# MIT-SPARK/Khronos

Hardware: AMD Instinct MI355X
Metric: active-window frames/sec (+ Mvoxel-updates/sec) at 1280x720 RGB-D+labels, 2 cm voxels (higher is better)
Workload: dtype f32

## Files before the change

### include/khronos_amd.h

```cpp
#ifndef KHRONOS_AMD_H_
#define KHRONOS_AMD_H_

#include <stddef.h>
#include <stdint.h>

#ifdef __cplusplus
extern "C" {
#endif

#define KHR_OK 0
#define KHR_EINVAL (-1)
#define KHR_ENOMEM (-2)
#define KHR_EDEVICE (-3)
#define KHR_ENOTFOUND (-4)
#define KHR_ESTATE (-5)

#define KHR_VOX_ACTIVE 1u
#define KHR_VOX_EVER_FREE 2u
#define KHR_VOX_TO_REMOVE 4u
#define KHR_VOX_SEM_VALID 8u
#define KHR_BLK_UPDATED 1u
#define KHR_BLK_MESH_UPDATED 2u
#define KHR_BLK_TRACKING_UPDATED 4u
#define KHR_BLK_HAS_ACTIVE_DATA 8u

typedef struct khr_config {
  float voxel_size;
  int32_t voxels_per_side;
  float truncation_distance;
  int32_t with_semantics;
  int32_t with_tracking;
  int32_t num_labels;
  int32_t use_weight_dropoff;
  float weight_dropoff_epsilon;
  int32_t use_constant_weight;
  float max_weight;
  int32_t interpolation_method;
  float adaptive_max_range_difference;
  int32_t range_mode;
  int32_t semantic_mode;
  float label_confidence;
  float temporal_buffer;
  float tsdf_occupancy_threshold;
  int32_t neighbor_connectivity;
  float temporal_window;
  int32_t md_neighbor_connectivity;
  int32_t md_min_cluster_size;
  int32_t md_max_cluster_size;
  float md_min_separation_distance;
  float md_max_range;
  float md_min_z_coordinate;
  float mesh_min_weight;
  uint32_t max_blocks;
  uint32_t max_frame_pixels;
  uint32_t num_frame_slots;
  uint64_t max_mesh_vertices;
  uint32_t max_band_records;
  int32_t disable_culling;
  int32_t device;
  int32_t rank;
  int32_t world_size;
  int32_t relaxed_arithmetic;
  uint32_t max_snapshot_blocks;
  int32_t alloc_candidate;
  int32_t color_blend_weight;
  int32_t mesh_attr_source;
  float mesh_degenerate_eps;
  int32_t packed_likelihood_rows;
} khr_config;

typedef struct khr_sensor {
  int32_t width, height;
  float fx, fy, cx, cy;
  float min_range, max_range;
} khr_sensor;

typedef struct khr_frame {
  uint64_t timestamp_ns;
  double world_T_sensor[16];
  const float* depth;
  const uint8_t* color;
  const int32_t* label;
} khr_frame;

typedef struct khr_stats {
  uint64_t n_allocated_blocks;
  uint64_t n_visible_blocks;
  uint64_t n_new_blocks;
  uint64_t n_visited_voxels;
  uint64_t n_updated_voxels;
  uint64_t n_band_voxels;
  uint64_t n_tracking_updated_blocks;
  uint64_t n_seeds;
  uint64_t n_mesh_blocks;
  uint64_t n_mesh_vertices;
  uint64_t pool_exhausted;
  uint64_t cum_updated_voxels;
  uint64_t cum_band_voxels;
  uint64_t cum_visited_voxels;
  uint64_t cum_integrate_calls;
  uint64_t n_tsdf_blocks;
  uint64_t band_overflow;
  uint64_t n_tracking_processed_blocks;
  uint64_t n_fuse_items;
  uint64_t n_seed_waits;
  uint64_t n_seed_waits_late;
  uint64_t seed_wait_max_us;
  uint64_t seed_wait_hist[8];
  uint64_t seed_wait_late_us;
  uint64_t seed_wait_late_frame;
  uint64_t seed_wait_late_state;
  uint64_t n_md_device_merges;
  uint64_t n_md_host_walks;
  uint64_t n_md_prelaunched;
  uint64_t n_md_prelaunch_repeats;
} khr_stats;

typedef struct khr_cluster {
  int32_t id;
  uint64_t num_pixels_listed;
  uint32_t num_pixels_painted;
  float bbox_min[3], bbox_max[3];
  float centroid[3];
  int32_t semantic_id;
} khr_cluster;

typedef struct khr_object_detector_config {
  int32_t use_full_connectivity;
  int32_t min_cluster_size;
  int32_t max_cluster_size;
  int32_t use_3d;
  float grid_size;
  float max_range;
  const int32_t* object_labels;
  int32_t n_object_labels;
} khr_object_detector_config;

typedef struct khr_ctx khr_ctx;

int khr_create(const khr_config* cfg, khr_ctx** out);
void khr_destroy(khr_ctx* ctx);
const char* khr_last_error(void);

void khr_host_trace(const char* tag);
int khr_set_stream(khr_ctx* ctx, void* hip_stream);
int khr_sync(khr_ctx* ctx);
void khr_default_config(khr_config* cfg);
int khr_reset_map(khr_ctx* ctx, float voxel_size, float truncation_distance);
int khr_retain_slot(khr_ctx* ctx, int slot);
int khr_release_slot(khr_ctx* ctx, int slot);
int khr_depend_on(khr_ctx* ctx, khr_ctx* other);
int khr_get_config(khr_ctx* ctx, khr_config* out);

int khr_upload_frame(khr_ctx* ctx, const khr_sensor* sensor, const khr_frame* frame, int on_device);
int khr_set_frame_image(khr_ctx* ctx, int slot, int which, const int32_t* image, int on_device);
int khr_download_frame(khr_ctx* ctx, int slot, float* range, float* vertex_map, int32_t* dynamic_image);
int khr_download_frame_image(khr_ctx* ctx, int slot, int which, int32_t* image);
typedef struct khr_frame_copy khr_frame_copy;
int khr_frame_copy_create(khr_ctx* ctx, int slot, khr_frame_copy** out);
int khr_frame_copy_download(khr_frame_copy* fc, float* depth, float* range, uint8_t* color_rgb, int32_t* labels, float* vertex_map);
void khr_frame_copy_release(khr_frame_copy* fc);
int khr_copy_frame_image(khr_ctx* ctx, int slot, int which, void* device_dst);

int khr_integrate(khr_ctx* ctx, int slot, int allocate_blocks, int use_mask, int object_id);
int khr_integrate_shared(khr_ctx* ctx, khr_ctx* src, int src_slot, int allocate_blocks, int use_mask, int object_id);
int khr_integrate_shared_batch(khr_ctx* ctx, khr_ctx* src, const int* src_slots, const int* object_ids, int n_frames,
                               int allocate_blocks, int use_mask);
int khr_update_tracking(khr_ctx* ctx, uint64_t timestamp_ns);
int khr_update_tracking_phase(khr_ctx* ctx, uint64_t timestamp_ns, int phase);
#define KHR_HALO_RECORD_BYTES 528
int khr_export_halo(khr_ctx* ctx, void* records, int64_t cap_records, int on_device);
int khr_import_halo(khr_ctx* ctx, const void* records, int64_t n_records, int on_device);
int khr_detect_motion(khr_ctx* ctx, int slot);
int khr_motion_keys(khr_ctx* ctx, int slot, void* keys_out, int on_device, uint32_t* n_seed_pixels);
int khr_detect_motion_from_keys(khr_ctx* ctx, int slot, const void* keys, int on_device);
size_t khr_motion_bits_bytes(int64_t n_pixels);
int khr_motion_bits(khr_ctx* ctx, int slot, void* bits_device);
int khr_detect_motion_from_bits(khr_ctx* ctx, int slot, const void* bits_device);
int khr_dynamic_pack_bytes(khr_ctx* ctx, int slot, void* dst_device);
int khr_dynamic_unpack_bytes(khr_ctx* ctx, int slot, const void* src_device);
int khr_mirror_dynamic(khr_ctx* ctx, int src_slot, int dst_slot);
int khr_get_dynamic_clusters(khr_ctx* ctx, int slot, khr_cluster* out, int cap);
int khr_configure_object_detector(khr_ctx* ctx, const khr_object_detector_config* cfg);
int khr_detect_objects(khr_ctx* ctx, int slot);
int khr_detect_objects_launch(khr_ctx* ctx, int slot);
int khr_get_semantic_clusters(khr_ctx* ctx, int slot, khr_cluster* out, int cap);
int64_t khr_cluster_voxels(khr_ctx* ctx, int slot, int which, float voxel_size, int32_t* ids_out, int64_t* voxels_out,
                           int64_t cap);
int khr_cluster_voxels_launch(khr_ctx* ctx, int slot, int which, float voxel_size);
int64_t khr_cluster_voxels_fetch(khr_ctx* ctx, int which, int32_t* ids_out, int64_t* voxels_out, int64_t cap);
int khr_configure_object_voxel_sets(khr_ctx* ctx, float voxel_size);
typedef struct khr_pixel_ref {
  int32_t slot;
  int32_t which;
  int32_t id;
} khr_pixel_ref;
int khr_pixel_iou(khr_ctx* ctx, int slot, const khr_pixel_ref* refs, int n_refs, int max_id, uint32_t* n_points, uint32_t* inter);
int khr_forward_instances(khr_ctx* ctx, int slot, float max_range, const int32_t* background_ids, int n_background, int max_id,
                          khr_cluster* out);
int khr_generate_mesh(khr_ctx* ctx, int only_mesh_updated, int clear_flag);
#define KHR_MESH_HALO_RECORD_BYTES(vps) (4 * (4 + 3 * 6 * (vps) * (vps)))
int khr_mesh_halo_requests(khr_ctx* ctx, void* keys_out, int64_t cap, int only_mesh_updated, int on_device);
int khr_mesh_halo_export(khr_ctx* ctx, const void* requests, int64_t n_requests, void* records, int64_t cap_records,
                         int on_device);
int khr_mesh_halo_import(khr_ctx* ctx, const void* records, int64_t n_records, int on_device);
#define KHR_MESH_HALO_REQ_HEADER_WORDS(world) (8 * (world))
int khr_mesh_halo_requests_sorted(khr_ctx* ctx, void* requests_device, int64_t cap, int only_mesh_updated);
int khr_mesh_halo_plan(int world, int rank, int vps, const uint64_t* headers, uint64_t* sendcounts, uint64_t* sdispls,
                       uint64_t* recvcounts, uint64_t* rdispls);
int khr_mesh_halo_answer(khr_ctx* ctx, const void* all_requests_device, int64_t cap, const uint64_t* headers, void* records_device,
                         int64_t cap_words);
int khr_mesh_halo_adopt(khr_ctx* ctx, const void* own_requests_device, const uint64_t* own_header, const void* records_device,
                        const uint64_t* rdispls);
int khr_reset_inactive(khr_ctx* ctx, int32_t* removed, int64_t cap, int64_t* n_removed);
int khr_last_removed(khr_ctx* ctx, int32_t* removed, int64_t cap, int64_t* n_removed);
int khr_mark_all_inactive(khr_ctx* ctx);
int khr_clear_updated(khr_ctx* ctx);
int khr_allocate_blocks(khr_ctx* ctx, const int32_t* indices, int64_t n);
int khr_object_prune(khr_ctx* ctx, float min_confidence, float min_observations, int64_t* n_pruned);

#define KHR_PF_MOTION 1u
#define KHR_PF_TRACKING 2u
#define KHR_PF_OUTPUT 4u
#define KHR_PF_OBJECTS 8u
#define KHR_PF_SNAPSHOT 32u
#define KHR_PF_INPUT_READY 16u
#define KHR_PF_INPUT_PINNED 128u
#define KHR_PF_INGESTED 64u
int khr_process_frame(khr_ctx* ctx, const khr_sensor* sensor, const khr_frame* frame, int on_device, uint32_t flags,
                      int* n_clusters);
int khr_ingest_ahead(khr_ctx* ctx, const khr_sensor* sensor, const khr_frame* frame);
int khr_ingest_ahead_host(khr_ctx* ctx, const khr_sensor* sensor, const khr_frame* frame);
int khr_ingest_cancel(khr_ctx* ctx);

int64_t khr_pool_exhausted(khr_ctx* ctx);
int khr_get_stats(khr_ctx* ctx, khr_stats* out);
int64_t khr_num_blocks(khr_ctx* ctx);
int64_t khr_block_indices(khr_ctx* ctx, int32_t* out, int64_t cap, int only_updated);
int khr_download_block(khr_ctx* ctx, int32_t bx, int32_t by, int32_t bz, float* distance, float* weight,
                       uint8_t* color_rgba, uint64_t* last_observed, uint64_t* last_occupied,
                       uint8_t* voxel_flags, uint32_t* sem_label, float* likelihoods, uint8_t* block_flags);
int khr_map_slice(khr_ctx* ctx, int64_t voxel_z, int64_t cap, int32_t* block_xy, float* positions, float* distance, float* weight,
                  uint64_t* last_observed, uint8_t* voxel_flags, int64_t* n_voxels);
int khr_slice_voxel_z(float height, float voxel_size, int32_t voxels_per_side, int64_t* voxel_z);
typedef struct khr_render_request {
  khr_sensor sensor;
  double world_T_sensor[16];
  float step_voxels;
  float min_weight;
} khr_render_request;
typedef struct khr_render_stats {
  uint64_t n_hit, n_blocked;
  uint64_t n_samples_total;
  uint64_t n_samples_evaluated;
} khr_render_stats;
int khr_render_view(khr_ctx* ctx, const khr_render_request* request, int on_device, float* depth, float* normal, uint8_t* color_rgba,
                    uint32_t* label, uint8_t* vflags, uint8_t* status, khr_render_stats* stats);
typedef struct khr_query_stats {
  uint64_t n_value, n_gradient, n_voxel;
} khr_query_stats;
#define KHR_QP_VALUE 1
#define KHR_QP_GRADIENT 2
#define KHR_QP_VOXEL 4
int khr_query_points(khr_ctx* ctx, int64_t n, const float* points, float min_weight, int on_device, float* distance, float* gradient,
                     float* weight, uint8_t* color_rgba, uint32_t* label, uint8_t* vflags, uint64_t* last_observed, uint8_t* status,
                     khr_query_stats* stats);
#define KHR_DF_MAX_DIM 512
#define KHR_DF_FAR (1 << 30)
// ... 177 lines not shown
```

### khronos_amd/capi.py

```python
import ctypes as C
import os

import numpy as np

_HERE = os.path.dirname(os.path.abspath(__file__))
LIB_PATH = os.path.join(_HERE, "lib", "libkhronos_amd.so")

KHR_OK, KHR_EINVAL, KHR_ENOMEM, KHR_EDEVICE, KHR_ENOTFOUND, KHR_ESTATE = 0, -1, -2, -3, -4, -5
VOX_ACTIVE, VOX_EVER_FREE, VOX_TO_REMOVE, VOX_SEM_VALID = 1, 2, 4, 8
BLK_UPDATED, BLK_MESH_UPDATED, BLK_TRACKING_UPDATED, BLK_HAS_ACTIVE_DATA = 1, 2, 4, 8


class KhrConfig(C.Structure):
    _fields_ = [
        ("voxel_size", C.c_float), ("voxels_per_side", C.c_int32), ("truncation_distance", C.c_float),
        ("with_semantics", C.c_int32), ("with_tracking", C.c_int32), ("num_labels", C.c_int32),
        ("use_weight_dropoff", C.c_int32), ("weight_dropoff_epsilon", C.c_float),
        ("use_constant_weight", C.c_int32), ("max_weight", C.c_float), ("interpolation_method", C.c_int32),
        ("adaptive_max_range_difference", C.c_float), ("range_mode", C.c_int32), ("semantic_mode", C.c_int32),
        ("label_confidence", C.c_float),
        ("temporal_buffer", C.c_float), ("tsdf_occupancy_threshold", C.c_float),
        ("neighbor_connectivity", C.c_int32), ("temporal_window", C.c_float),
        ("md_neighbor_connectivity", C.c_int32), ("md_min_cluster_size", C.c_int32),
        ("md_max_cluster_size", C.c_int32), ("md_min_separation_distance", C.c_float),
        ("md_max_range", C.c_float), ("md_min_z_coordinate", C.c_float),
        ("mesh_min_weight", C.c_float),
        ("max_blocks", C.c_uint32), ("max_frame_pixels", C.c_uint32), ("num_frame_slots", C.c_uint32),
        ("max_mesh_vertices", C.c_uint64), ("max_band_records", C.c_uint32), ("disable_culling", C.c_int32),
        ("device", C.c_int32), ("rank", C.c_int32), ("world_size", C.c_int32), ("relaxed_arithmetic", C.c_int32), ("max_snapshot_blocks", C.c_uint32),
        ("alloc_candidate", C.c_int32), ("color_blend_weight", C.c_int32), ("mesh_attr_source", C.c_int32), ("mesh_degenerate_eps", C.c_float),
        ("packed_likelihood_rows", C.c_int32),
    ]


class KhrSensor(C.Structure):
    _fields_ = [("width", C.c_int32), ("height", C.c_int32), ("fx", C.c_float), ("fy", C.c_float),
                ("cx", C.c_float), ("cy", C.c_float), ("min_range", C.c_float), ("max_range", C.c_float)]


class KhrRenderRequest(C.Structure):
    _fields_ = [("sensor", KhrSensor), ("world_T_sensor", C.c_double * 16), ("step_voxels", C.c_float), ("min_weight", C.c_float)]


class KhrRenderStats(C.Structure):
    _fields_ = [(n, C.c_uint64) for n in ("n_hit", "n_blocked", "n_samples_total", "n_samples_evaluated")]


class KhrQueryStats(C.Structure):
    _fields_ = [(n, C.c_uint64) for n in ("n_value", "n_gradient", "n_voxel")]


KHR_QP_VALUE, KHR_QP_GRADIENT, KHR_QP_VOXEL = 1, 2, 4


class KhrWeldStats(C.Structure):
    _fields_ = [("n_soup_vertices", C.c_uint64), ("n_vertices", C.c_uint64), ("n_faces", C.c_uint64), ("n_degenerate_faces", C.c_uint64)]


KHR_MERGE_ALIGNED, KHR_MERGE_RESAMPLE = 0, 1


class KhrMergeRequest(C.Structure):
    _fields_ = [("mode", C.c_int32), ("voxel_offset", C.c_int32 * 3), ("dst_T_src", C.c_double * 16), ("min_weight", C.c_float)]


class KhrMergeStats(C.Structure):
    _fields_ = [(n, C.c_uint64) for n in ("n_src_blocks", "n_candidate_blocks", "n_touched_blocks", "n_new_blocks", "n_added_voxels",
                                          "n_merged_voxels")]


class KhrDfRequest(C.Structure):
    _fields_ = [("origin", C.c_int32 * 3), ("dims", C.c_int32 * 3), ("ratio", C.c_int32), ("min_weight", C.c_float),
                ("max_distance", C.c_float), ("surface_distance", C.c_float), ("unknown_is_obstacle", C.c_int32),
                ("positive_only", C.c_int32)]


class KhrDfStats(C.Structure):
    _fields_ = [(n, C.c_uint64) for n in ("n_observed", "n_obstacle", "n_free", "n_in_range")]


KHR_DF_OBSERVED, KHR_DF_OBSTACLE, KHR_DF_IN_RANGE = 1, 2, 4
KHR_DF_MAX_DIM, KHR_DF_FAR = 512, 1 << 30


class KhrAlignRequest(C.Structure):
    _fields_ = [("n", C.c_int64), ("points", C.c_void_p), ("depth", C.c_void_p), ("sensor", KhrSensor), ("stride", C.c_int32),
                ("weights", C.c_void_p), ("world_T_source", C.c_double * 16), ("min_weight", C.c_float), ("gate", C.c_float),
                ("huber_delta", C.c_float)]


class KhrAlignOptions(C.Structure):
    _fields_ = [("max_iterations", C.c_int32), ("min_inliers", C.c_int32), ("lambda_", C.c_double), ("eps_rot", C.c_double),
                ("eps_trans", C.c_double)]


class KhrAlignResult(C.Structure):
    _fields_ = [("iterations", C.c_int32), ("converged", C.c_int32), ("n_inlier_first", C.c_uint64), ("n_inlier_last", C.c_uint64),
                ("rmse_first", C.c_double), ("rmse_last", C.c_double), ("H", C.c_double * 21), ("b", C.c_double * 6)]


KHR_ALIGN_WORDS, KHR_ALIGN_MAX_SOURCES = 32, 1 << 20


class KhrFrame(C.Structure):
    _fields_ = [("timestamp_ns", C.c_uint64), ("world_T_sensor", C.c_double * 16), ("depth", C.c_void_p),
                ("color", C.c_void_p), ("label", C.c_void_p)]


class KhrConvertedFrame(C.Structure):
    _fields_ = [("timestamp_ns", C.c_uint64), ("world_T_sensor", C.c_double * 16), ("range", C.c_void_p), ("depth", C.c_void_p),
                ("rgba", C.c_void_p), ("label", C.c_void_p), ("tile_max", C.c_void_p)]


class KhrCluster(C.Structure):
    _fields_ = [("id", C.c_int32), ("num_pixels_listed", C.c_uint64), ("num_pixels_painted", C.c_uint32),
                ("bbox_min", C.c_float * 3), ("bbox_max", C.c_float * 3), ("centroid", C.c_float * 3),
                ("semantic_id", C.c_int32)]


class KhrObjectDetectorConfig(C.Structure):
    _fields_ = [("use_full_connectivity", C.c_int32), ("min_cluster_size", C.c_int32), ("max_cluster_size", C.c_int32),
                ("use_3d", C.c_int32), ("grid_size", C.c_float), ("max_range", C.c_float),
                ("object_labels", C.POINTER(C.c_int32)), ("n_object_labels", C.c_int32)]


CKPT_SECTIONS = ("indices", "distance", "weight", "color", "last_observed", "last_occupied", "flags", "sem_label", "block_flags",
                 "likelihoods")


class KhrCheckpointHeader(C.Structure):
    _fields_ = [("magic", C.c_uint32), ("version", C.c_uint32), ("voxel_size", C.c_float), ("voxels_per_side", C.c_int32),
                ("truncation_distance", C.c_float), ("with_semantics", C.c_int32), ("with_tracking", C.c_int32),
                ("num_labels", C.c_int32), ("semantic_mode", C.c_int32), ("header_bytes", C.c_uint32),
                ("num_blocks", C.c_uint64), ("total_bytes", C.c_uint64), ("offset", C.c_uint64 * len(CKPT_SECTIONS))]


class KhrStats(C.Structure):
    _fields_ = [(n, C.c_uint64) for n in (
        "n_allocated_blocks", "n_visible_blocks", "n_new_blocks", "n_visited_voxels", "n_updated_voxels",
        "n_band_voxels", "n_tracking_updated_blocks", "n_seeds", "n_mesh_blocks", "n_mesh_vertices",
        "pool_exhausted", "cum_updated_voxels", "cum_band_voxels", "cum_visited_voxels", "cum_integrate_calls", "n_tsdf_blocks", "band_overflow",
        "n_tracking_processed_blocks", "n_fuse_items", "n_seed_waits", "n_seed_waits_late", "seed_wait_max_us")] + [
        ("seed_wait_hist", C.c_uint64 * 8)] + [(n, C.c_uint64) for n in (
        "seed_wait_late_us", "seed_wait_late_frame", "seed_wait_late_state", "n_md_device_merges", "n_md_host_walks",
        "n_md_prelaunched", "n_md_prelaunch_repeats")]


EXPORTS = [
    "khr_create", "khr_destroy", "khr_last_error", "khr_host_trace", "khr_set_stream", "khr_sync", "khr_default_config",
    "khr_upload_frame", "khr_set_frame_image", "khr_download_frame", "khr_frame_copy_create", "khr_frame_copy_download", "khr_frame_copy_release", "khr_integrate", "khr_update_tracking",
    "khr_detect_motion", "khr_generate_mesh", "khr_reset_inactive", "khr_mark_all_inactive", "khr_clear_updated",
    "khr_allocate_blocks", "khr_object_prune", "khr_get_stats", "khr_num_blocks", "khr_block_indices",
    "khr_download_block", "khr_mesh_num_vertices", "khr_download_mesh", "khr_fetch_mesh", "khr_fetch_mesh_into", "khr_timing_enable", "khr_timing_reset",
    "khr_timing_get", "khr_debug_read", "khr_tick_ingest", "khr_tick_integrate", "khr_tick_live_bound", "khr_tick_seed_counts", "khr_converted_bytes", "khr_export_converted",
    "khr_converted_views", "khr_tick_adopt", "khr_copy_frame_image", "khr_rv_detect_changes", "khr_last_removed", "khr_process_frame", "khr_ingest_ahead", "khr_ingest_ahead_host", "khr_ingest_cancel", "khr_integrate_shared", "khr_integrate_shared_batch", "khr_pixel_iou", "khr_forward_instances", "khr_update_tracking_phase",
    "khr_export_halo", "khr_import_halo", "khr_get_dynamic_clusters", "khr_motion_keys", "khr_motion_bits_bytes", "khr_motion_bits", "khr_detect_motion_from_bits",
    "khr_dynamic_pack_bytes", "khr_dynamic_unpack_bytes",
    "khr_detect_motion_from_keys", "khr_download_updated", "khr_mesh_halo_requests", "khr_mesh_halo_export",
    "khr_mesh_halo_requests_sorted", "khr_mesh_halo_plan", "khr_mesh_halo_answer", "khr_mesh_halo_adopt",
    "khr_mesh_halo_import", "khr_configure_object_detector", "khr_detect_objects", "khr_get_semantic_clusters",
    "khr_cluster_voxels", "khr_download_frame_image", "khr_detect_objects_launch", "khr_pool_exhausted", "khr_map_digest",
    "khr_rv_create", "khr_rv_destroy", "khr_rv_clear", "khr_rv_add_rays", "khr_rv_num_rays", "khr_rv_num_pairs", "khr_rv_check",
    "khr_snapshot_updated", "khr_take_snapshot", "khr_snapshot_num_blocks", "khr_snapshot_download", "khr_snapshot_download_extra", "khr_snapshot_download_begin", "khr_snapshot_download_end", "khr_snapshot_poll", "khr_fetch_mesh_launch", "khr_reserve_mesh_staging", "khr_reserve_snapshots", "khr_mirror_dynamic", "khr_snapshot_release",
    "khr_rv_check_stamps", "khr_get_config", "khr_cluster_voxels_launch", "khr_cluster_voxels_fetch", "khr_reset_map", "khr_depend_on", "khr_retain_slot", "khr_release_slot",
    "khr_map_slice", "khr_slice_voxel_z", "khr_render_view", "khr_query_points",
    "khr_align_linearize", "khr_align_frame", "khr_distance_field",
    "khr_checkpoint_size", "khr_checkpoint_save", "khr_checkpoint_load", "khr_checkpoint_inspect",
    "khr_debug_live_resources", "khr_configure_object_voxel_sets",
    "khr_weld_mesh", "khr_weld_mesh_into", "khr_merge_map",
]

_lib = None


class KhronosAmdError(RuntimeError):
    pass


def load_library():
    global _lib
    if _lib is not None:
        return _lib
    if not os.path.exists(LIB_PATH):
        raise KhronosAmdError(
            "HIP extension %s is missing: run `python -c 'import __graft_entry__ as g; g.build()'`. "
            "The khronos_amd fusion path has no CPU fallback." % LIB_PATH)
    lib = C.CDLL(LIB_PATH)
    vp, i32, i64, u64 = C.c_void_p, C.c_int, C.c_int64, C.c_uint64
    lib.khr_create.argtypes = [C.POINTER(KhrConfig), C.POINTER(vp)]
    lib.khr_create.restype = i32
    lib.khr_destroy.argtypes = [vp]
    lib.khr_destroy.restype = None
    lib.khr_last_error.restype = C.c_char_p
    lib.khr_host_trace.argtypes = [C.c_char_p]
    lib.khr_host_trace.restype = None
    lib.khr_set_stream.argtypes = [vp, vp]
    lib.khr_sync.argtypes = [vp]
    lib.khr_default_config.argtypes = [C.POINTER(KhrConfig)]
    lib.khr_default_config.restype = None
    lib.khr_upload_frame.argtypes = [vp, C.POINTER(KhrSensor), C.POINTER(KhrFrame), i32]
    lib.khr_set_frame_image.argtypes = [vp, i32, i32, vp, i32]
    lib.khr_download_frame.argtypes = [vp, i32, vp, vp, vp]
    lib.khr_integrate.argtypes = [vp, i32, i32, i32, i32]
    lib.khr_integrate_shared.argtypes = [vp, vp, i32, i32, i32, i32]
    lib.khr_integrate_shared_batch.argtypes = [vp, vp, vp, vp, i32, i32, i32]
    lib.khr_update_tracking.argtypes = [vp, u64]
    lib.khr_update_tracking_phase.argtypes = [vp, u64, i32]
    lib.khr_export_halo.argtypes = [vp, vp, i64, i32]
    lib.khr_import_halo.argtypes = [vp, vp, i64, i32]
    lib.khr_detect_motion.argtypes = [vp, i32]
    lib.khr_motion_keys.argtypes = [vp, i32, vp, i32, C.POINTER(C.c_uint32)]
    lib.khr_detect_motion_from_keys.argtypes = [vp, i32, vp, i32]
    lib.khr_get_dynamic_clusters.argtypes = [vp, i32, C.POINTER(KhrCluster), i32]
    lib.khr_configure_object_detector.argtypes = [vp, C.POINTER(KhrObjectDetectorConfig)]
    lib.khr_detect_objects.argtypes = [vp, i32]
    lib.khr_pixel_iou.argtypes = [vp, i32, vp, i32, i32, vp, vp]
    lib.khr_forward_instances.argtypes = [vp, i32, C.c_float, vp, i32, i32, C.POINTER(KhrCluster)]
    lib.khr_download_frame_image.argtypes = [vp, i32, i32, vp]
    lib.khr_rv_create.argtypes = [C.c_float, C.c_float, C.c_float, i32, C.POINTER(vp)]
    lib.khr_rv_destroy.argtypes = [vp]
    lib.khr_rv_destroy.restype = None
    lib.khr_rv_clear.argtypes = [vp]
    lib.khr_rv_add_rays.argtypes = [vp, C.c_int64, vp, vp, vp]
    lib.khr_rv_num_rays.argtypes = [vp]
    lib.khr_rv_num_rays.restype = C.c_int64
    lib.khr_rv_num_pairs.argtypes = [vp]
    lib.khr_rv_num_pairs.restype = C.c_int64
    lib.khr_rv_check.argtypes = [vp, C.c_int64, vp, vp, vp, vp, vp, C.POINTER(C.c_uint64), C.POINTER(C.c_uint64)]
    lib.khr_rv_check_stamps.argtypes = [vp, vp, vp]
    lib.khr_rv_detect_changes.argtypes = [vp, C.c_float, C.c_int64, i32, C.c_float, C.c_float, vp, i32, vp, vp, vp]
    lib.khr_get_config.argtypes = [vp, vp]
    lib.khr_reset_map.argtypes = [vp, C.c_float, C.c_float]
    lib.khr_depend_on.argtypes = [vp, vp]
    lib.khr_retain_slot.argtypes = [vp, i32]
    lib.khr_release_slot.argtypes = [vp, i32]
    lib.khr_cluster_voxels_launch.argtypes = [vp, i32, i32, C.c_float]
    lib.khr_cluster_voxels_fetch.argtypes = [vp, i32, vp, vp, C.c_int64]
    lib.khr_cluster_voxels_fetch.restype = C.c_int64
    lib.khr_configure_object_voxel_sets.argtypes = [vp, C.c_float]
    lib.khr_get_semantic_clusters.argtypes = [vp, i32, C.POINTER(KhrCluster), i32]
    lib.khr_cluster_voxels.argtypes = [vp, i32, i32, C.c_float, vp, vp, C.c_int64]
    lib.khr_cluster_voxels.restype = C.c_int64
    lib.khr_generate_mesh.argtypes = [vp, i32, i32]
    lib.khr_reset_inactive.argtypes = [vp, vp, i64, C.POINTER(i64)]
    lib.khr_mark_all_inactive.argtypes = [vp]
    lib.khr_clear_updated.argtypes = [vp]
    lib.khr_allocate_blocks.argtypes = [vp, vp, i64]
    lib.khr_object_prune.argtypes = [vp, C.c_float, C.c_float, C.POINTER(i64)]
    lib.khr_get_stats.argtypes = [vp, C.POINTER(KhrStats)]
    lib.khr_num_blocks.argtypes = [vp]
    lib.khr_num_blocks.restype = i64
    lib.khr_block_indices.argtypes = [vp, vp, i64, i32]
    lib.khr_block_indices.restype = i64
    lib.khr_download_block.argtypes = [vp, C.c_int32, C.c_int32, C.c_int32] + [vp] * 9
    lib.khr_map_slice.argtypes = [vp, i64, i64] + [vp] * 7
    lib.khr_slice_voxel_z.argtypes = [C.c_float, C.c_float, C.c_int32, vp]
    lib.khr_render_view.argtypes = [vp, C.POINTER(KhrRenderRequest), i32] + [vp] * 6 + [C.POINTER(KhrRenderStats)]
    lib.khr_query_points.argtypes = [vp, i64, vp, C.c_float, i32] + [vp] * 8 + [C.POINTER(KhrQueryStats)]
    lib.khr_distance_field.argtypes = [vp, C.POINTER(KhrDfRequest), i32, vp, vp, vp, C.POINTER(KhrDfStats)]
    lib.khr_align_linearize.argtypes = [vp, C.POINTER(KhrAlignRequest), i32, vp]
    lib.khr_align_frame.argtypes = [vp, C.POINTER(KhrAlignRequest), i32, C.POINTER(KhrAlignOptions), vp, C.POINTER(KhrAlignResult)]
    lib.khr_checkpoint_size.argtypes = [vp, C.POINTER(u64), C.POINTER(i64)]
    lib.khr_checkpoint_save.argtypes = [vp, vp, u64, C.POINTER(u64)]
    lib.khr_checkpoint_load.argtypes = [vp, vp, u64, C.POINTER(i64)]
    lib.khr_checkpoint_inspect.argtypes = [vp, u64, C.POINTER(KhrCheckpointHeader)]
    lib.khr_mesh_halo_requests.argtypes = [vp, vp, i64, i32, i32]
    lib.khr_mesh_halo_export.argtypes = [vp, vp, i64, vp, i64, i32]
    lib.khr_mesh_halo_import.argtypes = [vp, vp, i64, i32]
    lib.khr_mesh_halo_requests_sorted.argtypes = [vp, vp, i64, i32]
    lib.khr_mesh_halo_plan.argtypes = [i32, i32, i32, vp, vp, vp, vp, vp]
    lib.khr_mesh_halo_answer.argtypes = [vp, vp, i64, vp, vp, i64]
    lib.khr_mesh_halo_adopt.argtypes = [vp, vp, vp, vp, vp]
    lib.khr_download_updated.argtypes = [vp] + [vp] * 7 + [i64]
    lib.khr_download_updated.restype = i64
    lib.khr_snapshot_updated.argtypes = [vp, C.c_uint32, i64, C.POINTER(vp)]
    lib.khr_take_snapshot.argtypes = [vp, C.POINTER(vp)]
    lib.khr_snapshot_num_blocks.argtypes = [vp]
    lib.khr_snapshot_num_blocks.restype = i64
    lib.khr_snapshot_download.argtypes = [vp] + [vp] * 7 + [i64]
    lib.khr_snapshot_download.restype = i64
    lib.khr_snapshot_download_begin.argtypes = [vp] + [vp] * 7 + [i64]
    lib.khr_snapshot_download_end.argtypes = [vp]
    lib.khr_snapshot_download_end.restype = i64
    lib.khr_snapshot_download_extra.argtypes = [vp, vp, vp, vp, i64]
    lib.khr_snapshot_download_extra.restype = i64
    lib.khr_snapshot_release.argtypes = [vp]
    lib.khr_snapshot_release.restype = None
    lib.khr_mesh_num_vertices.argtypes = [vp]
    lib.khr_mesh_num_vertices.restype = i64
    lib.khr_download_mesh.argtypes = [vp, vp, vp, vp, vp, vp, i64]
    lib.khr_download_mesh.restype = i64
    lib.khr_fetch_mesh.argtypes = [vp, vp]
    lib.khr_fetch_mesh.restype = i64
    lib.khr_fetch_mesh_into.argtypes = [vp, vp, vp, vp, vp, vp]
    lib.khr_weld_mesh.argtypes = [vp, C.c_float, C.POINTER(KhrWeldStats)]
    lib.khr_weld_mesh_into.argtypes = [vp, i32] + [vp] * 7
    lib.khr_merge_map.argtypes = [vp, vp, C.POINTER(KhrMergeRequest), C.POINTER(KhrMergeStats)]
    lib.khr_debug_read.argtypes = [vp, vp, i64]
# ... 1028 lines not shown
```

### khronos_amd/csrc/khr_kernels_aux.h

```cpp
#pragma once
#include <cstring>
#include "khr_md_host.h"
#include "khr_device.h"

namespace khr {

#include "mc_table.inc"
__device__ int8_t g_mc_tri[256][16];
__device__ uint8_t g_mc_ntri[256];

constexpr uint64_t kSeedBit = kSeedFlag;

__global__ __launch_bounds__(256) void k_motion_pixels(DevMap m, DevParams p, DevFrame f, float md_max_range,
                                                      float min_z_world, uint64_t* __restrict__ keys, int ignore_epoch,
                                                      uint32_t* __restrict__ begin_band_count) {
  if (begin_band_count && blockIdx.x == 0) beginIntegrate(m, p.nvox, begin_band_count);
  const int i = blockIdx.x * blockDim.x + threadIdx.x;
  const bool in = i < f.W * f.H;
  uint64_t key = ~0ull;
  if (in)
    key = motionPixelKey(m, p, f.range[i], f.depth[i], i % f.W, i / f.W, f.fx, f.fy, f.cx, f.cy, f.Rw, f.tw, md_max_range,
                         min_z_world, ignore_epoch);
  if (in) keys[i] = key;
  const bool seed = (key != ~0ull) && (key & kSeedBit);
  const int any = __syncthreads_count(seed ? 1 : 0);
  if (any && threadIdx.x == 0) atomicAdd(&m.counters[C_N_SEEDS], static_cast<uint32_t>(any));
}

__global__ __launch_bounds__(1024) void k_publish(const uint32_t* __restrict__ src, volatile uint32_t* __restrict__ dst_host,
                                                 uint32_t rec_words, uint32_t max_recs, volatile uint32_t* __restrict__ ticket_host,
                                                 uint32_t ticket, uint32_t* __restrict__ counters_to_zero) {
  const uint32_t n_words = 4u + min(src[0], max_recs) * rec_words;
  for (uint32_t i = threadIdx.x; i < n_words; i += blockDim.x) dst_host[i] = src[i];
  __threadfence_system();
  __syncthreads();
  if (threadIdx.x < 4) counters_to_zero[threadIdx.x] = 0u;
  if (threadIdx.x == 0) {
    *ticket_host = ticket;
    __threadfence_system();
  }
}

__global__ void k_publish_seed(DevMap m, volatile uint32_t* host_seed, uint32_t ticket) {
  if (blockIdx.x == 0 && threadIdx.x == 0) publishSeedCount(m, host_seed, ticket);
}

__global__ __launch_bounds__(256) void k_md_keys_export(const uint64_t* __restrict__ keys, int n, uint64_t* __restrict__ out) {
  const int i = blockIdx.x * blockDim.x + threadIdx.x;
  if (i < n) out[i] = keys[i] == ~0ull ? 0ull : keys[i];
}
__global__ __launch_bounds__(256) void k_md_keys_import(const uint64_t* __restrict__ in, int n, uint64_t* __restrict__ keys,
                                                       uint32_t* __restrict__ n_seed_px) {
  const int i = blockIdx.x * blockDim.x + threadIdx.x;
  uint64_t k = ~0ull;
  if (i < n) {
    k = in[i] == 0ull ? ~0ull : in[i];
    keys[i] = k;
  }
  const unsigned long long b = __ballot(k != ~0ull && (k & kSeedBit));
  if (b && laneId() == static_cast<uint32_t>(__ffsll(static_cast<long long>(b)) - 1))
    atomicAdd(n_seed_px, static_cast<uint32_t>(__popcll(b)));
}

__global__ __launch_bounds__(256) void k_md_bits_export(const uint64_t* __restrict__ keys, int n, unsigned long long* __restrict__ bits) {
  const int i = blockIdx.x * blockDim.x + threadIdx.x;
  const uint64_t k = i < n ? keys[i] : ~0ull;
  const unsigned long long ex = __ballot(k != ~0ull), sd = __ballot(k != ~0ull && (k & kSeedBit));
  if (laneId() == 0 && (i & ~63) < n) {
    bits[2 * (i >> 6)] = ex;
    bits[2 * (i >> 6) + 1] = sd;
  }
}
__global__ __launch_bounds__(256) void k_md_keys_from_bits(DevParams p, DevFrame f, float md_max_range, float min_z_world,
                                                          const unsigned long long* __restrict__ bits, uint64_t* __restrict__ keys,
                                                          uint32_t* __restrict__ n_seed_px) {
  const int i = blockIdx.x * blockDim.x + threadIdx.x;
  const int n = f.W * f.H;
  uint64_t k = ~0ull;
  if (i < n) {
    const unsigned long long ex = bits[2 * (i >> 6)], sd = bits[2 * (i >> 6) + 1];
    if ((ex >> (i & 63)) & 1ull) {
      uint64_t bkey;
      int lin;
      k = motionPixelVoxel(p, f.range[i], f.depth[i], i % f.W, i / f.W, f.fx, f.fy, f.cx, f.cy, f.Rw, f.tw, md_max_range, min_z_world, &bkey, &lin);
      if (k != ~0ull && ((sd >> (i & 63)) & 1ull)) k |= kSeedBit;
    }
    keys[i] = k;
  }
  const unsigned long long b = __ballot(k != ~0ull && (k & kSeedBit));
  if (b && laneId() == static_cast<uint32_t>(__ffsll(static_cast<long long>(b)) - 1))
    atomicAdd(n_seed_px, static_cast<uint32_t>(__popcll(b)));
}
__global__ __launch_bounds__(256) void k_dyn_pack_u8(const int32_t* __restrict__ img, int n4, uint32_t* __restrict__ out) {
  const int i = blockIdx.x * blockDim.x + threadIdx.x;
  if (i >= n4) return;
  const int4 v = reinterpret_cast<const int4*>(img)[i];
  out[i] = (static_cast<uint32_t>(v.x) & 0xffu) | ((static_cast<uint32_t>(v.y) & 0xffu) << 8) | ((static_cast<uint32_t>(v.z) & 0xffu) << 16) |
           ((static_cast<uint32_t>(v.w) & 0xffu) << 24);
}
__global__ __launch_bounds__(256) void k_dyn_unpack_u8(const uint32_t* __restrict__ in, int n4, int32_t* __restrict__ img) {
  const int i = blockIdx.x * blockDim.x + threadIdx.x;
  if (i >= n4) return;
  const uint32_t w = in[i];
  reinterpret_cast<int4*>(img)[i] = make_int4(static_cast<int>(w & 0xffu), static_cast<int>((w >> 8) & 0xffu), static_cast<int>((w >> 16) & 0xffu),
                                              static_cast<int>(w >> 24));
}

struct VoxTable {
  uint64_t* keys;
  uint32_t* counts;
  uint32_t* ids;
  uint32_t mask;
};

__device__ inline int voxFind(const VoxTable& t, uint64_t key) {
  uint32_t h = hashKey(key) & t.mask;
  for (uint32_t probes = 0; probes <= t.mask; ++probes) {
    const uint64_t k = t.keys[h];
    if (k == key) return static_cast<int>(h);
    if (k == kEmptyKey) return -1;
    h = (h + 1) & t.mask;
  }
  return -1;
}

__device__ inline uint32_t voxInsert(const VoxTable& t, uint64_t key) {
  uint32_t h = hashKey(key) & t.mask;
  for (uint32_t probes = 0; probes <= t.mask; ++probes) {
    const unsigned long long prev = atomicCAS(reinterpret_cast<unsigned long long*>(&t.keys[h]),
                                              static_cast<unsigned long long>(kEmptyKey), static_cast<unsigned long long>(key));
    if (prev == kEmptyKey || prev == key) return h;
    h = (h + 1) & t.mask;
  }
  return kInvalidSlot;
}

__constant__ int8_t c_md_nbr26[26][3] = {
    {-1, 0, 0}, {1, 0, 0}, {0, -1, 0}, {0, 1, 0}, {0, 0, -1}, {0, 0, 1},
    {-1, -1, 0}, {-1, 1, 0}, {1, -1, 0}, {1, 1, 0}, {-1, 0, -1}, {-1, 0, 1}, {1, 0, -1}, {1, 0, 1},
    {0, -1, -1}, {0, -1, 1}, {0, 1, -1}, {0, 1, 1},
    {-1, -1, -1}, {-1, -1, 1}, {-1, 1, -1}, {-1, 1, 1}, {1, -1, -1}, {1, -1, 1}, {1, 1, -1}, {1, 1, 1}};

__device__ inline uint64_t neighbourKey(uint64_t key, int k) {
  int x, y, z;
  unpackKey(key, &x, &y, &z);
  return packKey(x + c_md_nbr26[k][0], y + c_md_nbr26[k][1], z + c_md_nbr26[k][2]);
}

__device__ inline void voxInsertCounted(const VoxTable& t, bool has, uint64_t key, uint32_t* overflow = nullptr) {
  const uint32_t lane = laneId();
  const uint32_t klo = static_cast<uint32_t>(key), khi = static_cast<uint32_t>(key >> 32);
  const uint32_t plo = __shfl_up(klo, 1), phi = __shfl_up(khi, 1);
  const unsigned long long hm = __ballot(has);
  const bool prev_has = lane > 0u && ((hm >> (lane - 1u)) & 1ull);
  const bool start = has && !(prev_has && plo == klo && phi == khi);
  const unsigned long long cont = hm & ~__ballot(start);
  if (start) {
    const unsigned long long above = lane == 63u ? 0ull : (~cont >> (lane + 1u));
    const uint32_t len = 1u + (lane == 63u ? 0u : static_cast<uint32_t>(__ffsll(static_cast<long long>(above | (1ull << (63u - lane)))) - 1));
    const uint32_t h = voxInsert(t, key);
    if (h != kInvalidSlot) atomicAdd(&t.counts[h], len);
    else if (overflow) atomicOr(overflow, 1u);
  }
}

__global__ __launch_bounds__(256) void k_md_clear(uint64_t* __restrict__ keys, uint32_t* __restrict__ counts, uint32_t tsize,
                                                 uint32_t* __restrict__ n4, int32_t* __restrict__ aabb) {
  const uint32_t stride = gridDim.x * blockDim.x;
  const uint32_t t0 = blockIdx.x * blockDim.x + threadIdx.x;
  ulonglong2* k2 = reinterpret_cast<ulonglong2*>(keys);
  for (uint32_t i = t0; i < 3u * (tsize / 2); i += stride) k2[i] = make_ulonglong2(~0ull, ~0ull);
  uint4* c4 = reinterpret_cast<uint4*>(counts);
  for (uint32_t i = t0; i < 2u * (tsize / 4); i += stride) c4[i] = make_uint4(0u, 0u, 0u, 0u);
  if (t0 < 4) n4[t0] = 0u;
  if (t0 < 6) aabb[t0] = t0 < 3 ? INT32_MAX : INT32_MIN;
  if (t0 == 7) aabb[7] = 0;
}

__global__ __launch_bounds__(256) void k_md_seed_insert(const uint64_t* __restrict__ keys, int n, VoxTable seeds,
                                                       uint32_t* __restrict__ overflow) {
  const int i = blockIdx.x * blockDim.x + threadIdx.x;
  const uint64_t k = i < n ? keys[i] : ~0ull;
  voxInsertCounted(seeds, k != ~0ull && (k & kSeedBit), k & ~kSeedBit, overflow);
}

__global__ __launch_bounds__(256) void k_md_near_insert(const uint64_t* __restrict__ seed_keys,
                                                       const uint32_t* __restrict__ n_seeds, uint32_t cap, int nn,
                                                       VoxTable near, uint32_t* __restrict__ overflow, int32_t* __restrict__ aabb) {
  const uint32_t ns = min(*n_seeds, cap);
  const bool direct = static_cast<float>(nn) * static_cast<float>(ns) > 0.7f * (static_cast<float>(near.mask) + 1.f);
  if (blockIdx.x == 0 && threadIdx.x == 0) aabb[6] = direct ? 1 : 0;
  int lo[3] = {INT32_MAX, INT32_MAX, INT32_MAX}, hi[3] = {INT32_MIN, INT32_MIN, INT32_MIN};
  for (uint32_t i = blockIdx.x * blockDim.x + threadIdx.x; i < ns * nn; i += gridDim.x * blockDim.x) {
    const uint64_t sk = seed_keys[i / nn];
    if (!direct && voxInsert(near, neighbourKey(sk, static_cast<int>(i % nn))) == kInvalidSlot) atomicOr(overflow, 1u);
    if (i % nn == 0) {
      int v[3];
      unpackKey(sk, &v[0], &v[1], &v[2]);
#pragma unroll
      for (int d = 0; d < 3; ++d) { lo[d] = min(lo[d], v[d]); hi[d] = max(hi[d], v[d]); }
    }
  }
  __shared__ int s_box[6][4];
#pragma unroll
  for (int d = 0; d < 3; ++d) {
#pragma unroll
    for (int o = 32; o > 0; o >>= 1) {
      lo[d] = min(lo[d], __shfl_xor(lo[d], o));
      hi[d] = max(hi[d], __shfl_xor(hi[d], o));
    }
  }
  if ((threadIdx.x & 63) == 0) {
#pragma unroll
    for (int d = 0; d < 3; ++d) { s_box[d][threadIdx.x >> 6] = lo[d]; s_box[3 + d][threadIdx.x >> 6] = hi[d]; }
  }
  __syncthreads();
  if (threadIdx.x < 6) {
    const int d = threadIdx.x;
    int v = s_box[d][0];
    for (int w = 1; w < 4; ++w) v = d < 3 ? min(v, s_box[d][w]) : max(v, s_box[d][w]);
    if (d < 3) { if (v != INT32_MAX) atomicMin(&aabb[d], v); }
    else if (v != INT32_MIN) atomicMax(&aabb[d], v);
  }
}

__global__ __launch_bounds__(256) void k_md_boundary_insert(const uint64_t* __restrict__ keys, int n, VoxTable near,
                                                           VoxTable bnd, VoxTable seeds, int nn, int direct,
                                                           const int32_t* __restrict__ aabb, uint32_t* __restrict__ overflow) {
  const int i = blockIdx.x * blockDim.x + threadIdx.x;
  const uint64_t k = i < n ? keys[i] : ~0ull;
  bool cand = k != ~0ull && !(k & kSeedBit);
  direct = direct || aabb[6];
  if (cand) {
    int x, y, z;
    unpackKey(k, &x, &y, &z);
    cand = x >= aabb[0] - 1 && y >= aabb[1] - 1 && z >= aabb[2] - 1 && x <= aabb[3] + 1 && y <= aabb[4] + 1 && z <= aabb[5] + 1;
  }
  if (cand) {
    if (!direct) {
      cand = voxFind(near, k) >= 0;
    } else {
      cand = false;
      for (int j = 0; j < nn && !cand; ++j) cand = voxFind(seeds, neighbourKey(k, j)) >= 0;
    }
  }
  voxInsertCounted(bnd, cand, k, overflow);
}

__global__ __launch_bounds__(256) void k_md_compact(VoxTable t, uint64_t* __restrict__ list_keys,
                                                   uint32_t* __restrict__ list_counts, uint32_t* __restrict__ n_out,
                                                   uint32_t cap, int32_t* __restrict__ zero_per_entry,
                                                   int32_t* __restrict__ zero_per_entry2 = nullptr,
                                                   unsigned long long* __restrict__ zero64 = nullptr) {
  __shared__ uint32_t s_cnt[4], s_base;
  const uint32_t h = blockIdx.x * blockDim.x + threadIdx.x;
  const bool used = h <= t.mask && t.keys[h] != kEmptyKey;
  const unsigned long long b = __ballot(used);
  if ((threadIdx.x & 63) == 0) s_cnt[threadIdx.x >> 6] = static_cast<uint32_t>(__popcll(b));
  __syncthreads();
  if (threadIdx.x == 0) {
    const uint32_t tot = s_cnt[0] + s_cnt[1] + s_cnt[2] + s_cnt[3];
    s_base = tot ? atomicAdd(n_out, tot) : 0u;
  }
  __syncthreads();
  if (used) {
    uint32_t id = s_base + static_cast<uint32_t>(__popcll(b & ((1ull << laneId()) - 1ull)));
    for (uint32_t w = 0; w < (threadIdx.x >> 6); ++w) id += s_cnt[w];
    if (id < cap) {
      list_keys[id] = t.keys[h];
      list_counts[id] = t.counts[h];
      t.ids[h] = id;
      if (zero_per_entry) zero_per_entry[id] = 0;
      if (zero_per_entry2) zero_per_entry2[id] = 0;
      if (zero64) zero64[id] = 0ull;
    }
  }
}

__global__ __launch_bounds__(256) void k_md_adjacency(const uint64_t* __restrict__ seed_keys,
                                                     const uint32_t* __restrict__ n_seeds, VoxTable seeds, VoxTable bnd,
                                                     int nn, uint32_t cap, uint32_t* __restrict__ adj,
                                                     uint32_t* __restrict__ edges, uint32_t edge_cap, uint32_t* __restrict__ n_edges) {
  __shared__ uint32_t s_cnt[4], s_base;
  const uint32_t ns = min(*n_seeds, cap);
  const uint32_t total = ns * nn;
  const uint32_t rounds = (total + gridDim.x * blockDim.x - 1) / (gridDim.x * blockDim.x);
  for (uint32_t r = 0; r < rounds; ++r) {
    const uint32_t i = (r * gridDim.x + blockIdx.x) * blockDim.x + threadIdx.x;
    uint32_t out = 0xffffffffu, s = 0;
    if (i < total) {
      s = i / nn;
      const uint32_t j = i % nn;
      const uint64_t nk = neighbourKey(seed_keys[s], static_cast<int>(j));
      const int hs = voxFind(seeds, nk);
      if (hs >= 0) {
        out = 0x80000000u | seeds.ids[hs];
      } else {
        const int hb = voxFind(bnd, nk);
        if (hb >= 0) out = bnd.ids[hb];
      }
      adj[i] = out;
    }
    const bool is_edge = out != 0xffffffffu && (out & 0x80000000u) && (out & 0x7fffffffu) < s && s < 65536u;
    const unsigned long long b = __ballot(is_edge);
    if ((threadIdx.x & 63) == 0) s_cnt[threadIdx.x >> 6] = static_cast<uint32_t>(__popcll(b));
    __syncthreads();
    if (threadIdx.x == 0) {
      const uint32_t tot = s_cnt[0] + s_cnt[1] + s_cnt[2] + s_cnt[3];
      s_base = tot ? atomicAdd(n_edges, tot) : 0u;
    }
    __syncthreads();
    if (is_edge) {
      uint32_t pos = s_base + static_cast<uint32_t>(__popcll(b & ((1ull << laneId()) - 1ull)));
      for (uint32_t w = 0; w < (threadIdx.x >> 6); ++w) pos += s_cnt[w];
      if (pos < edge_cap) edges[pos] = (s << 16) | (out & 0x7fffffffu);
    }
    __syncthreads();
  }
}

static_assert(sizeof(CompAcc) == 48, "CompAcc travels to the host as 12 words (k_publish)");
__device__ inline unsigned long long canonKey(uint64_t packed) {
  int x, y, z;
  unpackKey(packed, &x, &y, &z);
  return (static_cast<unsigned long long>(x + (1 << 20)) << 42) | (static_cast<unsigned long long>(y + (1 << 20)) << 21) |
         static_cast<unsigned long long>(z + (1 << 20));
}

constexpr uint32_t kCompLds = 12288;
// ... 136 lines not shown
    uint64_t bk[26];
#pragma unroll
    for (int j = 0; j < 26; ++j) {
      const bool is_b = av[j] != 0xffffffffu && !(av[j] & 0x80000000u);
      bc[j] = is_b ? bnd_counts[av[j]] : 0u;
      bk[j] = is_b ? bnd_keys[av[j]] : k;
    }
#pragma unroll
    for (int j = 0; j < 26; ++j) {
      px += bc[j];
      unpackKey(bk[j], &v[0], &v[1], &v[2]);
#pragma unroll
      for (int d = 0; d < 3; ++d) { lo[d] = min(lo[d], v[d]); hi[d] = max(hi[d], v[d]); }
    }
  }
  unsigned long long todo = __ballot(on);
  while (todo) {
    const int leader = __ffsll(static_cast<long long>(todo)) - 1;
    const uint32_t lr = __shfl(r, leader);
    const bool mine = on && r == lr;
    const unsigned long long grp = __ballot(mine);
    todo &= ~grp;
    unsigned long long p2 = mine ? px : 0ull, k2 = mine ? key : ~0ull;
    int l2[3], h2[3];
#pragma unroll
    for (int d = 0; d < 3; ++d) { l2[d] = mine ? lo[d] : INT32_MAX; h2[d] = mine ? hi[d] : INT32_MIN; }
#pragma unroll
    for (int o = 32; o > 0; o >>= 1) {
      const unsigned long long po = (static_cast<unsigned long long>(__shfl_xor(static_cast<uint32_t>(p2 >> 32), o)) << 32) |
                                    __shfl_xor(static_cast<uint32_t>(p2), o);
      const unsigned long long ko = (static_cast<unsigned long long>(__shfl_xor(static_cast<uint32_t>(k2 >> 32), o)) << 32) |
                                    __shfl_xor(static_cast<uint32_t>(k2), o);
      p2 += po;
      k2 = ko < k2 ? ko : k2;
#pragma unroll
      for (int d = 0; d < 3; ++d) { l2[d] = min(l2[d], __shfl_xor(l2[d], o)); h2[d] = max(h2[d], __shfl_xor(h2[d], o)); }
    }
    if (static_cast<int>(laneId()) == leader) {
      CompAcc* a = acc + lr;
      atomicAdd(&a->n_pixels, p2);
      atomicMin(&a->min_key, k2);
#pragma unroll
      for (int d = 0; d < 3; ++d) { atomicMin(&a->lo[d], l2[d]); atomicMax(&a->hi[d], h2[d]); }
    }
  }
}

__global__ __launch_bounds__(256) void k_md_comp_roots(const uint32_t* __restrict__ n_seeds, uint32_t cap, const uint32_t* __restrict__ parent,
                                                      const CompAcc* __restrict__ acc, uint32_t* __restrict__ root_idx,
                                                      uint32_t* __restrict__ n_roots, CompAcc* __restrict__ out, uint32_t out_cap) {
  const uint32_t ns = min(*n_seeds, cap);
  const uint32_t s = blockIdx.x * blockDim.x + threadIdx.x;
  const bool is_root = s < ns && parent[s] == s;
  const uint32_t idx = waveAggInc(n_roots, is_root);
  if (is_root) {
    root_idx[s] = idx;
    if (idx < out_cap) {
      CompAcc a = acc[s];
      a.root = 0u;
      a.pad = 0u;
      out[idx] = a;
    }
  }
}

__device__ inline unsigned long long compBit(const uint32_t* __restrict__ parent, const uint32_t* __restrict__ root_idx, uint32_t seed_id) {
  const uint32_t ri = root_idx[parent[seed_id]];
  return ri < 64u ? (1ull << ri) : 0ull;
}
__device__ inline unsigned long long segmentedOr(unsigned long long bits, uint32_t seg, bool* head) {
  const uint32_t lane = laneId();
  const uint32_t prev = __shfl_up(seg, 1);
  *head = lane == 0u || prev != seg;
#pragma unroll
  for (int o = 1; o < 32; o <<= 1) {
    const unsigned long long ob = (static_cast<unsigned long long>(__shfl_down(static_cast<uint32_t>(bits >> 32), o)) << 32) |
                                  __shfl_down(static_cast<uint32_t>(bits), o);
    const uint32_t os = __shfl_down(seg, o);
    if (lane + static_cast<uint32_t>(o) < 64u && os == seg) bits |= ob;
  }
  return bits;
}
__global__ __launch_bounds__(256) void k_md_bnd_comps(const uint64_t* __restrict__ bnd_keys, const uint32_t* __restrict__ n4, uint32_t cap, int nn,
                                                     VoxTable seeds, const uint32_t* __restrict__ parent, const uint32_t* __restrict__ root_idx,
                                                     unsigned long long* __restrict__ bnd_mask) {
  const uint32_t nb = min(n4[1], cap), R = n4[2];
  if (R < 2u || R > 64u) return;
  const uint32_t total = nb * static_cast<uint32_t>(nn), step = gridDim.x * blockDim.x;
  for (uint32_t i0 = blockIdx.x * blockDim.x; i0 < total; i0 += step) {
    const uint32_t i = i0 + threadIdx.x;
    const bool valid = i < total;
    const uint32_t b = valid ? i / nn : 0xffffffffu, j = valid ? i % nn : 0u;
    unsigned long long bit = 0ull;
    if (valid) {
      const int hs = voxFind(seeds, neighbourKey(bnd_keys[b], static_cast<int>(j)));
      if (hs >= 0) bit = compBit(parent, root_idx, seeds.ids[hs]);
    }
    bool head;
    bit = segmentedOr(bit, b, &head);
    if (valid && head && bit) atomicOr(&bnd_mask[b], bit);
  }
}
__global__ __launch_bounds__(256) void k_md_comp_overlap(const uint64_t* __restrict__ seed_keys, const uint64_t* __restrict__ bnd_keys,
                                                        const uint32_t* __restrict__ n4, uint32_t cap, int radius, VoxTable seeds, VoxTable bnd,
                                                        const uint32_t* __restrict__ parent, const uint32_t* __restrict__ root_idx,
                                                        const unsigned long long* __restrict__ bnd_mask, CompAcc* __restrict__ out) {
  const uint32_t ns = min(n4[0], cap), nb = min(n4[1], cap), R = n4[2];
  if (R < 2u || R > 64u) return;
  const uint32_t per = radius > 0 ? 27u : 1u;
  const uint32_t total = (ns + nb) * per, step = gridDim.x * blockDim.x;
  for (uint32_t i0 = blockIdx.x * blockDim.x; i0 < total; i0 += step) {
    const uint32_t i = i0 + threadIdx.x;
    const bool valid = i < total;
    const uint32_t v = valid ? i / per : 0xffffffffu, k = valid ? (per == 1u ? 26u : i % per) : 0u;
    unsigned long long bits = 0ull, mine = 0ull;
    if (valid) {
      const bool is_seed = v < ns;
      const uint64_t key = is_seed ? seed_keys[v] : bnd_keys[v - ns];
      mine = is_seed ? compBit(parent, root_idx, v) : bnd_mask[v - ns];
      if (k == 26u) {
        bits = mine;
      } else {
        const uint64_t nk = neighbourKey(key, static_cast<int>(k));
        const int hs = voxFind(seeds, nk);
        if (hs >= 0) {
          bits = compBit(parent, root_idx, seeds.ids[hs]);
        } else {
          const int hb = voxFind(bnd, nk);
          if (hb >= 0 && bnd.ids[hb] < cap) bits = bnd_mask[bnd.ids[hb]];
        }
      }
    }
    bool head;
    const unsigned long long acc = segmentedOr(bits, v, &head);
    if (valid && head && (acc & ~mine)) {
      unsigned long long todo = mine;
      while (todo) {
        const int c = __ffsll(static_cast<long long>(todo)) - 1;
        todo &= todo - 1ull;
        atomicOr(reinterpret_cast<unsigned long long*>(&out[c].root), acc | mine);
      }
    }
    if (valid && head && (mine & (mine - 1ull))) {
      unsigned long long todo = mine;
      while (todo) {
        const int c = __ffsll(static_cast<long long>(todo)) - 1;
        todo &= todo - 1ull;
        atomicOr(reinterpret_cast<unsigned long long*>(&out[c].root), mine);
      }
    }
  }
}

constexpr int kCompInline = 64;
struct CompFinals {
  int32_t id[kCompInline];
};
__global__ __launch_bounds__(256) void k_md_comp_finals(const uint32_t* __restrict__ adj, const uint32_t* __restrict__ n_seeds, uint32_t cap,
                                                       int nn, const uint32_t* __restrict__ parent, const uint32_t* __restrict__ root_idx,
                                                       const int32_t* __restrict__ comp_final, CompFinals inl, int32_t* __restrict__ seed_final,
                                                       int32_t* __restrict__ bnd_final, int32_t* __restrict__ bnd_deg) {
  const uint32_t ns = min(*n_seeds, cap);
  for (uint32_t i = blockIdx.x * blockDim.x + threadIdx.x; i < ns * nn; i += gridDim.x * blockDim.x) {
    const uint32_t s = i / nn, j = i % nn;
    const uint32_t ri = root_idx[parent[s]];
    const int32_t f = comp_final ? comp_final[ri] : inl.id[ri];
    if (j == 0) seed_final[s] = f;
    const uint32_t a = adj[i];
    if (f && a != 0xffffffffu && !(a & 0x80000000u)) {
      atomicMax(&bnd_final[a], f);
      atomicAdd(&bnd_deg[a], 1);
    }
  }
}

struct ClusterAcc {
  uint32_t n_pixels;
  int32_t bmin[3], bmax[3];
  float sum[3];
  uint32_t n_listed;
  float wsum[3];
};
__host__ __device__ inline void clusterAccReset(ClusterAcc& a) {
  a.n_pixels = 0;
  a.n_listed = 0;
  for (int d = 0; d < 3; ++d) { a.bmin[d] = INT32_MAX; a.bmax[d] = INT32_MIN; a.sum[d] = 0.f; a.wsum[d] = 0.f; }
}
__device__ inline int32_t floatToOrdered(float f) {
  const int32_t i = __float_as_int(f);
  return i >= 0 ? i : i ^ 0x7fffffff;
}
__host__ __device__ inline float orderedToFloat(int32_t i) {
  const int32_t j = i >= 0 ? i : i ^ 0x7fffffff;
  float f;
#if defined(__HIP_DEVICE_COMPILE__)
  f = __int_as_float(j);
#else
  std::memcpy(&f, &j, sizeof(f));
#endif
  return f;
}

__global__ __launch_bounds__(256) void k_md_paint(const uint64_t* __restrict__ keys, int n, VoxTable seeds, VoxTable bnd,
                                                 const int32_t* __restrict__ seed_final,
                                                 const int32_t* __restrict__ bnd_final, int32_t* __restrict__ dyn,
                                                 const int32_t* __restrict__ bnd_deg, uint8_t* __restrict__ dyn_weight) {
  const int i = blockIdx.x * blockDim.x + threadIdx.x;
  if (i >= n) return;
  const uint64_t k = keys[i];
  if (k == ~0ull) return;
  int id = 0, w = 1;
  if (k & kSeedBit) {
    const int h = voxFind(seeds, k & ~kSeedBit);
    if (h >= 0) id = seed_final[seeds.ids[h]];
  } else {
    const int h = voxFind(bnd, k);
    if (h >= 0) {
      id = bnd_final[bnd.ids[h]];
      w = bnd_deg[bnd.ids[h]];
    }
  }
  if (id) {
    dyn[i] = id;
    dyn_weight[i] = static_cast<uint8_t>(min(max(w, 1), 255));
  }
}

constexpr int kAccTile = 32, kAccSlots = 8;
__global__ __launch_bounds__(1024) void k_cluster_summary(DevFrame f, const int32_t* __restrict__ img,
                                                         ClusterAcc* __restrict__ acc, const uint8_t* __restrict__ weight) {
  __shared__ int s_id[kAccSlots];
  __shared__ ClusterAcc s_acc[kAccSlots];
  if (threadIdx.x < kAccSlots) {
    s_id[threadIdx.x] = 0;
    ClusterAcc a;
    clusterAccReset(a);
    s_acc[threadIdx.x] = a;
  }
  __syncthreads();
  const int tiles_x = (f.W + kAccTile - 1) / kAccTile;
  const int u = (blockIdx.x % tiles_x) * kAccTile + (threadIdx.x & 31), v = (blockIdx.x / tiles_x) * kAccTile + (threadIdx.x >> 5);
  int id = 0;
  float pw[3] = {0.f, 0.f, 0.f};
  float wt = 1.f;
  if (u < f.W && v < f.H) {
    const int i = v * f.W + u;
    id = img[i];
    if (id) {
      if (weight) wt = static_cast<float>(weight[i]);
      const float d = f.depth[i];
      xform(f.Rw, f.tw, ((static_cast<float>(u) - f.cx) / f.fx) * d, ((static_cast<float>(v) - f.cy) / f.fy) * d, d, pw);
    }
  }
  unsigned long long todo = __ballot(id != 0);
  while (todo) {
    const int leader = __ffsll(static_cast<long long>(todo)) - 1;
    const int cid = __shfl(id, leader);
    const bool mine = id == cid;
    const unsigned long long grp = __ballot(mine);
    todo &= ~grp;
    float mn[3], mx[3], sm[3], ws[3];
    float wn = mine ? wt : 0.f;
#pragma unroll
    for (int c = 0; c < 3; ++c) {
      mn[c] = mine ? pw[c] : 3.0e38f;
      mx[c] = mine ? pw[c] : -3.0e38f;
      sm[c] = mine ? pw[c] : 0.f;
      ws[c] = mine ? wt * pw[c] : 0.f;
    }
#pragma unroll
    for (int o = 32; o > 0; o >>= 1) {
      wn += __shfl_xor(wn, o);
#pragma unroll
      for (int c = 0; c < 3; ++c) {
        mn[c] = fminf(mn[c], __shfl_xor(mn[c], o));
        mx[c] = fmaxf(mx[c], __shfl_xor(mx[c], o));
        sm[c] += __shfl_xor(sm[c], o);
        ws[c] += __shfl_xor(ws[c], o);
      }
    }
    if (static_cast<int>(laneId()) == leader) {
      ClusterAcc* a = acc + cid;
      for (int k = 0; k < kAccSlots; ++k) {
        const int h = (cid + k) & (kAccSlots - 1);
        const int prev = atomicCAS(&s_id[h], 0, cid);
        if (prev == 0 || prev == cid) {
          a = &s_acc[h];
          break;
        }
      }
      atomicAdd(&a->n_pixels, static_cast<uint32_t>(__popcll(grp)));
      atomicAdd(&a->n_listed, static_cast<uint32_t>(wn));
#pragma unroll
      for (int c = 0; c < 3; ++c) {
        atomicMin(&a->bmin[c], floatToOrdered(mn[c]));
        atomicMax(&a->bmax[c], floatToOrdered(mx[c]));
        atomicAdd(&a->sum[c], sm[c]);
        atomicAdd(&a->wsum[c], ws[c]);
      }
    }
  }
  __syncthreads();
  if (threadIdx.x < kAccSlots && s_id[threadIdx.x]) {
    const ClusterAcc& l = s_acc[threadIdx.x];
    ClusterAcc* a = acc + s_id[threadIdx.x];
    atomicAdd(&a->n_pixels, l.n_pixels);
    atomicAdd(&a->n_listed, l.n_listed);
#pragma unroll
    for (int c = 0; c < 3; ++c) {
      atomicMin(&a->bmin[c], l.bmin[c]);
      atomicMax(&a->bmax[c], l.bmax[c]);
      atomicAdd(&a->sum[c], l.sum[c]);
      atomicAdd(&a->wsum[c], l.wsum[c]);
    }
  }
}

__global__ __launch_bounds__(256) void k_publish_cluster_acc(ClusterAcc* __restrict__ acc, volatile uint32_t* __restrict__ dst_host,
                                                            uint32_t n_ids, volatile uint32_t* __restrict__ ticket_host, uint32_t ticket) {
  constexpr uint32_t W = sizeof(ClusterAcc) / 4;
  const uint32_t* src = reinterpret_cast<const uint32_t*>(acc);
  for (uint32_t i = threadIdx.x; i < n_ids * W; i += blockDim.x) dst_host[i] = src[i];
  __threadfence_system();
  __syncthreads();
  for (uint32_t k = threadIdx.x; k < n_ids; k += blockDim.x) {
    ClusterAcc a;
    clusterAccReset(a);
    acc[k] = a;
  }
  if (threadIdx.x == 0) {
    *ticket_host = ticket;
    __threadfence_system();
  }
}

template <int VPS>
struct MeshHalo {
  static constexpr int PL = VPS * VPS;
  static constexpr int kPlaneWords = PL * 6;
  static constexpr int kWords = 4 + 3 * kPlaneWords;
  __host__ __device__ static int planeOf(int sel) { return (sel & 1) ? 0 : ((sel & 2) ? 1 : 2); }
  __host__ __device__ static int indexOf(int sel, int x, int y, int z) {
    return (sel & 1) ? (y + VPS * z) : ((sel & 2) ? (x + VPS * z) : (x + VPS * y));
  }
  __host__ __device__ static const uint32_t* plane(const uint32_t* rec, int pl) { return rec + 4 + pl * kPlaneWords; }
  __host__ __device__ static float dist(const uint32_t* rec, int pl, int i) {
    const uint32_t v = plane(rec, pl)[i];
    float f;
#if defined(__HIP_DEVICE_COMPILE__)
    f = __uint_as_float(v);
#else
    std::memcpy(&f, &v, 4);
#endif
    return f;
  }
  __host__ __device__ static float weight(const uint32_t* rec, int pl, int i) {
    const uint32_t v = plane(rec, pl)[PL + i];
    float f;
#if defined(__HIP_DEVICE_COMPILE__)
// ... 965 lines not shown
```

### khronos_amd/csrc/khr_md_host.h

```cpp
#pragma once
#include <algorithm>
#include <cmath>
#include <cstdint>
#include <numeric>
#include <utility>
#include <vector>

namespace khr {

struct CompAcc {
  unsigned long long n_pixels;
  unsigned long long min_key;
  int32_t lo[3], hi[3];
  uint32_t root, pad;
};

namespace mdh {

struct Vox { int64_t v[3]; };
inline Vox voxelOf(uint64_t key) {
  return Vox{{static_cast<int64_t>(key & 0x1fffffu) - (1 << 20), static_cast<int64_t>((key >> 21) & 0x1fffffu) - (1 << 20),
              static_cast<int64_t>((key >> 42) & 0x1fffffu) - (1 << 20)}};
}
inline bool closerThan(int64_t n2, float sep) { return static_cast<float>(static_cast<int64_t>(std::sqrt(static_cast<double>(n2)))) < sep; }
template <class A, class B>
inline bool boxesCloserThan(const A& a, const B& b, float sep) {
  int64_t gap2 = 0;
  for (int d = 0; d < 3; ++d) {
    const int64_t gp = std::max<int64_t>(0, std::max(static_cast<int64_t>(a.lo[d]) - b.hi[d], static_cast<int64_t>(b.lo[d]) - a.hi[d]));
    gap2 += gp * gp;
  }
  return closerThan(gap2, sep);
}

inline std::vector<uint32_t> clusterOrder(const CompAcc* comp, uint32_t R) {
  std::vector<uint32_t> order(R);
  std::iota(order.begin(), order.end(), 0u);
  std::sort(order.begin(), order.end(), [&](uint32_t a, uint32_t b) { return comp[a].min_key < comp[b].min_key; });
  return order;
}

inline bool mayMerge(const CompAcc* comp, uint32_t R, float sep) {
  for (uint32_t i = 0; i < R; ++i)
    for (uint32_t j = i + 1; j < R; ++j)
      if (boxesCloserThan(comp[i], comp[j], sep)) return true;
  return false;
}

struct Groups {
  std::vector<uint32_t> rep;
  explicit Groups(uint32_t n) : rep(n) { std::iota(rep.begin(), rep.end(), 0u); }
  uint32_t find(uint32_t x) {
    while (rep[x] != x) x = rep[x] = rep[rep[x]];
    return x;
  }
  void unite(uint32_t a, uint32_t b) {
    a = find(a), b = find(b);
    if (a != b) rep[std::max(a, b)] = std::min(a, b);
  }
  std::vector<uint32_t> labels() {
    for (uint32_t i = 0; i < rep.size(); ++i) rep[i] = find(i);
    return rep;
  }
};

inline std::vector<uint32_t> groupsFromRows(const CompAcc* comp, uint32_t R) {
  Groups g(R);
  for (uint32_t i = 0; i < R && i < 64; ++i) {
    unsigned long long row = ((static_cast<unsigned long long>(comp[i].pad) << 32) | comp[i].root) & ~(1ull << i);
    for (; row; row &= row - 1ull) {
      const uint32_t j = static_cast<uint32_t>(__builtin_ctzll(row));
      if (j < R) g.unite(i, j);
    }
  }
  return g.labels();
}

using Kept = std::vector<std::pair<int, uint64_t>>;
template <class Px>
inline Kept numberClusters(const uint32_t* order, const uint32_t* group, uint32_t R, Px px, int min_size, int max_size, std::vector<int32_t>* id_out) {
  Kept kept;
  id_out->assign(R, 0);
  std::vector<uint64_t> gpx(R, 0);
  std::vector<int32_t> gid(R, -1);
  for (uint32_t r = 0; r < R; ++r) gpx[group[r]] += px(r);
  int id = 1;
  for (uint32_t k = 0; k < R; ++k) {
    const uint32_t r = order[k], g = group[r];
    if (gid[g] < 0) {
      const int size = static_cast<int>(gpx[g]);
      gid[g] = size < min_size || size > max_size ? 0 : id;
      if (gid[g]) kept.emplace_back(id, gpx[g]);
      if (gid[g] && id < 255) ++id;
    }
    (*id_out)[r] = gid[g];
  }
  return kept;
}

struct WalkLists {
  const uint64_t *seed_keys, *bnd_keys;
  const uint32_t *seed_counts, *bnd_counts, *adj;
  uint32_t S, B;
  int nn;
};

inline Kept walkClusters(const WalkLists& l, float sep, int min_size, int max_size, int32_t* seed_final, int32_t* bnd_final, int32_t* bnd_deg) {
  const uint32_t S = l.S, B = l.B;
  const int nn = l.nn;
  std::vector<uint32_t> order(S);
  std::vector<Vox> sg(S);
  std::iota(order.begin(), order.end(), 0u);
  for (uint32_t i = 0; i < S; ++i) sg[i] = voxelOf(l.seed_keys[i]);
  std::sort(order.begin(), order.end(),
            [&](uint32_t a, uint32_t b) { return std::lexicographical_compare(sg[a].v, sg[a].v + 3, sg[b].v, sg[b].v + 3); });
  struct Cluster {
    uint64_t n_pixels = 0;
    std::vector<uint32_t> seeds, bnds;
    std::vector<Vox> vox;
    int64_t lo[3], hi[3];
  };
  std::vector<Cluster> clusters;
  std::vector<uint8_t> closed(S, 0);
  std::vector<uint32_t> stack;
  for (uint32_t s0 : order) {
    if (closed[s0]) continue;
    stack.assign(1, s0);
    Cluster cl;
    while (!stack.empty()) {
      const uint32_t r = stack.back();
      stack.pop_back();
      if (closed[r]) continue;
      closed[r] = 1;
      cl.n_pixels += l.seed_counts[r];
      cl.seeds.push_back(r);
      for (int k = 0; k < nn; ++k) {
        const uint32_t a = l.adj[static_cast<size_t>(r) * nn + k];
        if (a == 0xffffffffu) continue;
        if (a & 0x80000000u) {
          stack.push_back(a & 0x7fffffffu);
        } else {
          cl.n_pixels += l.bnd_counts[a];
          cl.bnds.push_back(a);
        }
      }
    }
    std::sort(cl.bnds.begin(), cl.bnds.end());
    cl.bnds.erase(std::unique(cl.bnds.begin(), cl.bnds.end()), cl.bnds.end());
    for (int d = 0; d < 3; ++d) { cl.lo[d] = INT64_MAX; cl.hi[d] = INT64_MIN; }
    for (uint32_t r : cl.seeds) cl.vox.push_back(sg[r]);
    for (uint32_t r : cl.bnds) cl.vox.push_back(voxelOf(l.bnd_keys[r]));
    for (const Vox& g : cl.vox)
      for (int d = 0; d < 3; ++d) { cl.lo[d] = std::min(cl.lo[d], g.v[d]); cl.hi[d] = std::max(cl.hi[d], g.v[d]); }
    clusters.push_back(std::move(cl));
  }
  const uint32_t nc = static_cast<uint32_t>(clusters.size());
  auto overlap = [&](const Cluster& a, const Cluster& b) {
    if (!boxesCloserThan(a, b, sep)) return false;
    for (const Vox& p : a.vox)
      for (const Vox& q : b.vox) {
        const int64_t dx = p.v[0] - q.v[0], dy = p.v[1] - q.v[1], dz = p.v[2] - q.v[2];
        if (closerThan(dx * dx + dy * dy + dz * dz, sep)) return true;
      }
    return false;
  };
  Groups groups(nc);
  for (uint32_t i = 0; i < nc; ++i)
    for (uint32_t j = i + 1; j < nc; ++j)
      if (overlap(clusters[i], clusters[j])) groups.unite(i, j);
  const std::vector<uint32_t> group = groups.labels();
  std::vector<uint32_t> identity(nc);
  std::vector<int32_t> ids;
  std::iota(identity.begin(), identity.end(), 0u);
  Kept kept = numberClusters(identity.data(), group.data(), nc, [&](uint32_t i) { return clusters[i].n_pixels; }, min_size, max_size, &ids);
  std::fill(seed_final, seed_final + S, 0);
  std::fill(bnd_final, bnd_final + B, 0);
  std::fill(bnd_deg, bnd_deg + B, 0);
  for (uint32_t ci = 0; ci < nc; ++ci) {
    const int32_t id = ids[ci];
    if (!id) continue;
    for (uint32_t r : clusters[ci].seeds) {
      seed_final[r] = id;
      for (int k = 0; k < nn; ++k) {
        const uint32_t a = l.adj[static_cast<size_t>(r) * nn + k];
        if (a != 0xffffffffu && !(a & 0x80000000u)) ++bnd_deg[a];
      }
    }
    for (uint32_t r : clusters[ci].bnds) bnd_final[r] = std::max(bnd_final[r], id);
  }
  return kept;
}

}
}
```

### khronos_amd/csrc/khronos_amd.hip

```cpp
#include <hip/hip_runtime.h>
#include <hip/hip_ext.h>
#include <hipcub/hipcub.hpp>

#include <algorithm>
#include <array>
#include <atomic>
#include <chrono>
#include <memory>
#include <mutex>
#include <cmath>
#include <cstdarg>
#include <cstdio>
#include <climits>
#include <cstring>
#include <cstdlib>
#include <functional>
#include <map>
#include <string>
#include <thread>
#include <tuple>
#include <unordered_map>
#include <vector>

#include "../../include/khronos_amd.h"
// ... 100 lines not shown
  Stream mc_stream;
  Stream h2d_stream;
  Event ev_aux, ev_aux_done;
  uint64_t aux_seq_issued = 0, aux_seq_done = 0, obj_seq = 0, cv_seq[3] = {0, 0, 0};
  std::vector<DevBuf<uint8_t>> allocs;
  std::vector<FrameSlot> slots;
  int next_slot = 0;
  std::unique_ptr<std::atomic<int>[]> slot_leases;
  uint32_t* d_work = nullptr;
  uint32_t* d_new = nullptr;
  uint32_t* d_ef = nullptr;
  uint32_t* d_trk_proc = nullptr;
  uint32_t* d_tick_work = nullptr;
  uint32_t* d_tick_counts = nullptr;
  uint32_t* d_tick_seeds = nullptr;
  PinnedBuf<uint32_t> h_tick;
  uint32_t tick_ticket = 0;
  std::vector<uint32_t> tick_seed_host;
  int tick_seed_n = 0, tick_seed_collected = 0;
  int tick_epoch = 0, motion_ignore_epoch = 0;
  unsigned long long* d_dbg = nullptr;
  unsigned long long* d_digest = nullptr;
  uint32_t* d_wg_stats = nullptr;
  bool fold_pending = false;
  int stream_priority = 0;
  unsigned char* d_fuse_sink = nullptr;
  DevBuf<uint32_t> d_pix_scratch;
  DevBuf<uint8_t> d_inst;
  uint4* d_work4 = nullptr;
  uint4* d_tick_work4 = nullptr;
  FuseFrame* d_tick_frames = nullptr;
  uint32_t* d_tick_mask = nullptr;
  bool tick_mask_dirty = false;
  uint32_t item_cap = 0;
  struct SnapArena {
    DevBuf<uint8_t> buf;
    PinnedBuf<uint32_t> count;
    volatile uint32_t* h_count() const { return count.get(); }
    int alloc(size_t bytes) {
      if (buf.alloc(bytes)) return fail(KHR_ENOMEM, "snapshot arena of %zu bytes", bytes);
      if (count.alloc(16)) {
        buf.reset();
        return fail(KHR_ENOMEM, "snapshot pinned words");
      }
      count[0] = count[1] = 0;
      return KHR_OK;
    }
  };
  struct SnapPool {
    std::mutex mu;
    std::vector<SnapArena> free;
    bool dead = false;
  };
  std::shared_ptr<SnapPool> snap_pool = std::make_shared<SnapPool>();
  struct FramePool {
    std::mutex mu;
    std::vector<DevBuf<uint8_t>> free;
    bool dead = false;
  };
  std::shared_ptr<FramePool> frame_pool = std::make_shared<FramePool>();
  khr_snapshot* pending_snapshot = nullptr;
  Event ev_snap_fork, ev_snap_join;
  Event ev_mc_fork, ev_mc_join;
  uint64_t explicit_blocks = 0;
  DevBuf<uint4> d_multi_list;
  DevBuf<uint32_t> d_frame_bits;
  PinnedBuf<FuseFrame> h_frames;
  DevBuf<FuseFrame> d_frames;
  Event ev_frames;
  uint32_t snap_ticket = 0;
  uint32_t wpb = 0;
  int fuse_zsplit = 2;
  DevBuf<uint64_t> d_halo_recs;
  const uint64_t* halo_view = nullptr;
  DevBuf<uint64_t> d_halo_keys;
  DevBuf<uint32_t> d_halo_vals;
  uint32_t halo_cap_total = 0, halo_mask = 0, halo_n = 0;
  DevBuf<uint32_t> d_mh_recs;
  const uint32_t* mh_view = nullptr;
  DevBuf<uint64_t> d_mh_keys;
  DevBuf<uint32_t> d_mh_vals;
  uint32_t mh_cap_total = 0, mh_mask = 0, mh_n = 0;
  uint8_t* d_mh_flag = nullptr;
  DevBuf<uint32_t> d_mh2_scratch;
  DevBuf<uint64_t> d_mh2_keys;
  DevBuf<uint32_t> d_mh2_offs;
  uint32_t mh2_ht = 0;
  bool mh_compact = false;
  PinnedBuf<uint32_t> h_pinned;
  uint32_t seed_ticket = 0;
  bool seed_publish_pending = false;
  bool seed_by_ticket = false;
  bool begun = false;
  uint32_t fetch_ticket = 0;
  bool fetch_pending = false;
  uint32_t* d_fetch_done = nullptr;
  std::vector<uint32_t> fm_order;
  size_t fm_total = 0;
  uint64_t map_gen = 1, counters_gen = 0;
  int last_frame_slot = -1;
  PinnedBuf<void> h_stage;
  PinnedBuf<uint32_t> h_totals;
  PinnedBuf<void> h_up;
  Event ev_ingest;
  Event ev_up;
  struct AheadEntry { int slot; int ev; bool host; };
  std::vector<AheadEntry> ahead_q;
  Event ev_ahead[2];
  Event ev_ahead_h2d[2];
  int ahead_ev_next = 0;
  Event ev_h2d;
  bool h2d_pending = false;
  uint64_t h2d_bytes = 0;
  int ef_parity = 0, ef_cur = 0;
  Event ev_seed;
  uint32_t last_removed = 0;
  khr_ctx* dep_src = nullptr;
  Event ev_dep, ev_dep_aux;
  uint64_t last_track_stamp = 0;
  bool removed_pending = false;
  int4* d_removed = nullptr;
  PinnedBuf<int4> h_removed_early;
  uint32_t* d_removed_early_n = nullptr;
  uint32_t removed_early_ticket = 0;
  bool removed_early = false;
  int* d_idx_staging = nullptr;
  uint64_t* d_keys = nullptr;
  uint32_t* d_pix = nullptr;
  void* d_cub_temp = nullptr;
  uint64_t* d_md_keys = nullptr;
  uint32_t *d_md_counts = nullptr, *d_md_ids = nullptr, *d_md_adj = nullptr;
  uint32_t* d_md_n = nullptr;
  uint64_t *d_md_seed_keys = nullptr, *d_md_bnd_keys = nullptr;
  uint32_t *d_md_seed_counts = nullptr, *d_md_bnd_counts = nullptr;
  int32_t *d_md_seed_final = nullptr, *d_md_bnd_final = nullptr;
  int32_t* d_md_bnd_deg = nullptr;
  unsigned long long* d_md_bnd_mask = nullptr;
  uint64_t n_seed_waits = 0, n_seed_waits_late = 0, seed_wait_max_us = 0, seed_wait_hist[8] = {0, 0, 0, 0, 0, 0, 0, 0};
  uint64_t seed_wait_late_us = 0, seed_wait_late_frame = 0, seed_wait_late_state = 0;
  bool last_ingest_on_aux = false;
  uint64_t n_md_device_merges = 0, n_md_host_walks = 0;
  ClusterAcc* d_md_acc = nullptr;
  uint32_t *d_md_parent = nullptr, *d_md_rootidx = nullptr;
  CompAcc* d_md_comp_acc = nullptr;
  int32_t* d_md_comp_final = nullptr;
  PinnedBuf<uint8_t> h_md_head;
  bool md_host_walk = false;
  uint32_t md_lds_max = kCompLds;
  uint32_t md_mask = 0, md_list_cap = 0;
  uint32_t md_head_ticket = 0;
  bool md_seed_run = false;
  uint32_t md_prev_seed_px = 0;
  uint64_t n_md_prelaunched = 0, n_md_prelaunch_repeats = 0;
  uint32_t md_last_seeds = 0;
  uint32_t* d_md_edges = nullptr;
  uint32_t* d_md_scratch4 = nullptr;
  PinnedBuf<uint32_t> h_md_walk;
  Event ev_md_walk_up;
  PinnedBuf<ClusterAcc> h_md_acc_pinned;
  uint32_t md_acc_ticket = 0;
  int md_acc_slot = -1;
  size_t cub_temp_bytes = 0;
  bool obj_configured = false;
  khr_object_detector_config obj_cfg{};
  std::vector<int32_t> obj_labels;
  DevBuf<int32_t> d_obj_labels;
  uint64_t* d_gv_keys = nullptr;
  uint32_t gv_mask = 0;
  uint32_t *d_gv_parent = nullptr, *d_gv_rootidx = nullptr, *d_gv_node = nullptr;
  uint32_t* d_gv_n = nullptr;
  ObjAcc* d_obj_acc = nullptr;
  int32_t* d_obj_final = nullptr;
  uint64_t* d_cv_list = nullptr;
  uint32_t obj_root_cap = 0;
  uint32_t* d_gv_owners = nullptr;
  uint32_t* d_gv_done = nullptr;
  bool gv_clean = false;
  bool gv_counters_clean[4] = {false, false, false, false};
  PinnedBuf<uint8_t> h_obj_head;
  Event ev_obj;
  int obj_pending_slot = -1;
  uint32_t* d_cv_n[3] = {nullptr, nullptr, nullptr};
  uint64_t* d_cv_keys[3] = {nullptr, nullptr, nullptr};
  PinnedBuf<uint8_t> h_cv[3];
  Event ev_cv[3];
  int cv_pending_slot[2] = {-1, -1};
  uint32_t obj_ticket = 0, cv_ticket[3] = {0, 0, 0};
  int3 cv_origin[3]{};
  int cv_set_obj = 1;
  float obj_cv_size = 0.f;
  int obj_cv_slot = -1;
  MeshBuffers mesh[2]{};
  int mesh_cur = 0;
  uint32_t *d_mesh_count = nullptr, *d_mesh_offset = nullptr;
  uint8_t* d_regen = nullptr;
  uint32_t* d_mesh_old_off = nullptr;
  uint32_t* d_mesh_nwork = nullptr;
  uint64_t mesh_total = 0;
  bool mesh_stale = false;
  std::vector<uint32_t> h_counters;
  khr_stats stats{};
  bool host_index_valid = false;
  std::map<std::array<int32_t, 3>, uint32_t> host_index;
  std::vector<uint32_t> host_flags;
  DevBuf<uint64_t> d_slice_keys;
  DevBuf<uint32_t> d_slice_count;
  DevBuf<uint8_t> d_slice_stage;
  PinnedBuf<uint8_t> h_slice_stage;
  uint32_t slice_cap = 0, slice_hint = 0;
  DevBuf<unsigned long long> d_render_stats;
  DevBuf<uint8_t> d_render_stage;
  PinnedBuf<uint8_t> h_render_stage;
  DevBuf<unsigned long long> d_query_stats;
  DevBuf<uint8_t> d_query_stage;
  PinnedBuf<uint8_t> h_query_stage;
  DevBuf<int32_t> d_df_outer, d_df_inner;
  DevBuf<unsigned long long> d_df_stats;
  DevBuf<uint8_t> d_df_stage;
  PinnedBuf<uint8_t> h_df_stage;
  DevBuf<unsigned long long> d_align_acc;
  PinnedBuf<unsigned long long> h_align_acc;
  DevBuf<uint8_t> d_align_stage;
  PinnedBuf<uint8_t> h_align_stage;
  DevBuf<uint8_t> d_ckpt[2];
  PinnedBuf<uint8_t> h_ckpt[2];
  DevBuf<uint32_t> d_ckpt_slots[2];
  DevBuf<uint32_t> d_ckpt_err;
  Event ev_ckpt_filled[2], ev_ckpt_drained[2];
  DevBuf<uint8_t> d_weld_work, d_weld_cub, d_weld_out;
  PinnedBuf<uint32_t> h_weld;
  WeldOut weld_out{};
  khr_weld_stats weld_stats{};
  bool weld_valid = false;
  DevBuf<uint64_t> d_merge_set;
  DevBuf<int4> d_merge_cand;
  DevBuf<uint32_t> d_merge_words;
  DevBuf<uint32_t> d_merge_ctr;
  PinnedBuf<uint32_t> h_merge;
  Event ev_merge;
  uint32_t timing = 0;
  std::vector<TimingRec> pending;
  std::vector<Event> event_pool;
  double t_ms[kNumTimers] = {0};
  uint64_t t_n[kNumTimers] = {0};
};

namespace {

Event takeEvent(khr_ctx* c) {
  Event e;
  if (!c->event_pool.empty()) {
    e = std::move(c->event_pool.back());
    c->event_pool.pop_back();
  } else {
    e.ensure(hipEventDefault);
  }
  return e;
}

struct ScopedTimer {
  khr_ctx* c;
  int which;
  Event a, b;
  hipStream_t st;
  bool on = false;
  ScopedTimer(khr_ctx* ctx, int w, hipStream_t stream = nullptr)
      : c(ctx), which(w), st(stream ? stream : static_cast<hipStream_t>(ctx->stream)) {
    on = w >= 0 && ((c->timing >> w) & 1u);
    if (on) {
      a = takeEvent(c);
      b = takeEvent(c);
      hipEventRecord(a, st);
    }
  }
  ~ScopedTimer() {
    if (on) {
      hipEventRecord(b, st);
      c->pending.push_back({which, std::move(a), std::move(b)});
    }
  }
};

#define KHR_LAUNCH_TIMED_ON(which, strm, kernel, grid, block, ...)                                     \
  do {                                                                                                 \
    if ((c->timing >> (which)) & 1u) {                                                                 \
      Event ev_a = takeEvent(c), ev_b = takeEvent(c);                                                  \
      hipExtLaunchKernelGGL(kernel, grid, block, 0, strm, ev_a, ev_b, 0, __VA_ARGS__);                 \
      c->pending.push_back({(which), std::move(ev_a), std::move(ev_b)});                               \
    } else {                                                                                           \
      hipLaunchKernelGGL(kernel, grid, block, 0, strm, __VA_ARGS__);                                   \
    }                                                                                                  \
  } while (0)
#define KHR_LAUNCH_TIMED(which, kernel, grid, block, ...) KHR_LAUNCH_TIMED_ON(which, c->stream, kernel, grid, block, __VA_ARGS__)

void resolveTimers(khr_ctx* c) {
  for (auto& r : c->pending) {
    hipEventSynchronize(r.b);
    float ms = 0.f;
    hipEventElapsedTime(&ms, r.a, r.b);
    if (r.which >= 0) {
      c->t_ms[r.which] += ms;
      c->t_n[r.which] += 1;
    }
    c->event_pool.push_back(std::move(r.a));
    c->event_pool.push_back(std::move(r.b));
  }
// ... 336 lines not shown
  *out = nullptr;
  if (!(cfg->voxel_size > 0.f) || !(cfg->truncation_distance > 0.f)) return fail(KHR_EINVAL, "voxel_size / truncation_distance must be > 0");
  if (cfg->voxels_per_side != 16 && cfg->voxels_per_side != 8) return fail(KHR_EINVAL, "voxels_per_side must be 8 or 16");
  auto conn_ok = [](int c) { return c == 6 || c == 18 || c == 26; };
  if (!conn_ok(cfg->neighbor_connectivity) || !conn_ok(cfg->md_neighbor_connectivity)) return fail(KHR_EINVAL, "neighbor_connectivity must be one of {6, 18, 26}");
  if (!(cfg->temporal_buffer > 0.f) || !(cfg->temporal_window > 0.f)) return fail(KHR_EINVAL, "temporal_buffer / temporal_window must be > 0");
  if (cfg->tsdf_occupancy_threshold == 0.f) return fail(KHR_EINVAL, "tsdf_occupancy_threshold must be != 0");
  if (cfg->md_max_cluster_size < cfg->md_min_cluster_size) return fail(KHR_EINVAL, "param 'max_cluster_size' must be >= 'min_cluster_size'");
  if (!(cfg->md_max_range > 0.f)) return fail(KHR_EINVAL, "md_max_range must be > 0");
  if (cfg->with_semantics && cfg->num_labels < 1) return fail(KHR_EINVAL, "num_labels must be >= 1 with semantics");
  if (cfg->semantic_mode == 1 && cfg->with_semantics && cfg->num_labels != 2) return fail(KHR_EINVAL, "binary semantic integrator needs num_labels == 2");
  if (cfg->max_blocks < 1 || cfg->max_frame_pixels < 1 || cfg->num_frame_slots < 1) return fail(KHR_EINVAL, "capacities must be >= 1");
  if (cfg->world_size < 1 || cfg->rank < 0 || cfg->rank >= cfg->world_size) return fail(KHR_EINVAL, "bad rank / world_size");

  int ndev = 0;
  if (hipGetDeviceCount(&ndev) != hipSuccess || ndev == 0)
    return fail(KHR_EDEVICE, "no HIP device available: the khronos_amd fusion path has no CPU fallback");
  if (cfg->device < 0 || cfg->device >= ndev) return fail(KHR_EINVAL, "device %d out of range (%d devices)", cfg->device, ndev);
  HIP_TRY(hipSetDevice(cfg->device));

  std::unique_ptr<khr_ctx, void (*)(khr_ctx*)> owner(new khr_ctx(), khr_destroy);
  khr_ctx* c = owner.get();
  c->cfg = *cfg;
  c->device = cfg->device;
  {
    static const bool prio_off = std::getenv("KHR_STREAM_PRIORITY") && std::atoi(std::getenv("KHR_STREAM_PRIORITY")) == 0;
    static const int prio_window = std::getenv("KHR_WINDOW_PRIORITY") ? std::atoi(std::getenv("KHR_WINDOW_PRIORITY")) : 0;
    c->stream_priority = prio_off ? 0 : (cfg->voxels_per_side == 8 ? -1 : prio_window);
  }
  if (createStream(c, c->stream)) return fail(KHR_EDEVICE, "hipStreamCreate failed");
  if (createStream(c, c->aux_stream) || c->ev_aux.ensure() || c->ev_aux_done.ensure())
    return fail(KHR_EDEVICE, "auxiliary stream / event creation failed");
  if (c->h_pinned.alloc(16) || c->ev_seed.ensure()) return fail(KHR_EDEVICE, "pinned scratch / event creation failed");
  std::memset(c->h_pinned, 0, 64);
  if (ensureStage(c, 1u << 20) != KHR_OK ||
      c->h_up.alloc(std::max<size_t>(1u << 16, cfg->voxels_per_side == 8 ? sizeof(int32_t) * 3 * static_cast<size_t>(cfg->max_blocks) : 0)))
    return fail(KHR_ENOMEM, "pinned staging buffers");

  DevParams& p = c->p;
  deriveMetricParams(*cfg, p);
  p.vps = cfg->voxels_per_side;
  p.nvox = p.vps * p.vps * p.vps;
  p.K = cfg->with_semantics ? cfg->num_labels : 1;
  p.KS = cfg->packed_likelihood_rows ? p.K : likStride(p.K);
  p.with_semantics = cfg->with_semantics;
  p.with_tracking = cfg->with_tracking;
  p.use_dropoff = cfg->use_weight_dropoff;
  p.const_weight = cfg->use_constant_weight;
  p.interp = cfg->interpolation_method;
  p.range_mode = cfg->range_mode;
  p.sem_mode = cfg->semantic_mode;
  p.max_weight = cfg->max_weight;
  p.adaptive_diff = cfg->adaptive_max_range_difference;
  p.log_match = std::log(cfg->label_confidence);
  p.log_nomatch = cfg->num_labels > 1 ? std::log((1.f - cfg->label_confidence) / static_cast<float>(cfg->num_labels - 1)) : 0.f;
  p.temporal_buffer = static_cast<double>(cfg->temporal_buffer);
  p.temporal_window = static_cast<double>(cfg->temporal_window);
  p.nn = cfg->neighbor_connectivity;
  p.mesh_min_weight = cfg->mesh_min_weight;
  p.mesh_eps = cfg->mesh_degenerate_eps > 0.f ? cfg->mesh_degenerate_eps : 1e-6f;
  p.mesh_attr_source = cfg->mesh_attr_source;
  p.alloc_candidate = cfg->alloc_candidate;
  p.rank = cfg->rank;
  p.world = cfg->world_size;
  p.dbg = std::getenv("KHR_DEBUG") ? std::atoi(std::getenv("KHR_DEBUG")) : 0;

  DevMap& m = c->m;
  const size_t cap = cfg->max_blocks, nv = p.nvox;
  uint32_t ht = 1;
  while (ht < cap * 4) ht <<= 1;
  m.ht_mask = ht - 1;
  m.capacity = static_cast<uint32_t>(cap);
  int rc = KHR_OK;
  KHR_CHAIN(devAlloc(c, &m.ht_keys, ht, false));
  KHR_CHAIN(devAlloc(c, &m.ht_vals, ht));
  KHR_CHAIN(devAlloc(c, &m.blk_index, cap));
  KHR_CHAIN(devAlloc(c, &m.blk_flags, cap));
  KHR_CHAIN(devAlloc(c, &m.dist, cap * nv, false));
  KHR_CHAIN(devAlloc(c, &m.weight, cap * nv, false));
  KHR_CHAIN(devAlloc(c, &m.color, cap * nv, false));
  KHR_CHAIN(devAlloc(c, &m.vflags, cap * nv, false));
  KHR_CHAIN(devAlloc(c, &m.sem_label, cfg->with_semantics ? cap * nv : 1, false));
  if (rc == KHR_OK && devAlloc(c, &m.lik, cfg->with_semantics ? cap * nv * p.KS : 1, false) != KHR_OK) {
    fail(KHR_ENOMEM, "the label-likelihood layer of %zu blocks needs %.2f GB (%d floats per voxel%s); khr_config.packed_likelihood_rows = 1 "
                     "stores %d per voxel, a smaller max_blocks less of everything", static_cast<size_t>(cap),
         1e-9 * static_cast<double>(cap) * nv * p.KS * 4, p.KS, p.KS != p.K ? ": rows padded to 128-byte lines" : "", p.K);
    KHR_CHAIN(KHR_ENOMEM);
  }
  KHR_CHAIN(devAlloc(c, &m.last_obs, cfg->with_tracking ? cap * nv : 1, false));
  KHR_CHAIN(devAlloc(c, &m.last_occ, cfg->with_tracking ? cap * nv : 1, false));
  KHR_CHAIN(devAlloc(c, &m.trk_lim, cfg->with_tracking ? cap * 2 : 2));
  KHR_CHAIN(devAlloc(c, &m.freebits, cfg->with_tracking ? cap * (nv / 64) : 1, false));
  KHR_CHAIN(devAlloc(c, &m.obs, cfg->with_tracking ? cap * (nv / 64) : 1, false));
  KHR_CHAIN(devAlloc(c, &m.free_slots, cap, false));
  KHR_CHAIN(devAlloc(c, &m.counters, C_COUNT));
  KHR_CHAIN(devAlloc(c, &m.stats, S_COUNT));
  KHR_CHAIN(devAlloc(c, &m.mesh_desc, cap));
  KHR_CHAIN(devAlloc(c, &c->d_work, cap));
  KHR_CHAIN(devAlloc(c, &c->d_new, cap));
  KHR_CHAIN(devAlloc(c, &c->d_ef, cap));
  KHR_CHAIN(devAlloc(c, &c->d_trk_proc, cap));
  KHR_CHAIN(devAlloc(c, &c->d_dbg, 4096 * 4 * 12));
  KHR_CHAIN(devAlloc(c, &c->d_digest, kDigestWords));
  KHR_CHAIN(devAlloc(c, &c->d_wg_stats, 2 * kUpdateStatSlots));
  KHR_CHAIN(devAlloc(c, &c->d_fuse_sink, static_cast<size_t>(kUpdateStatSlots) * 16 * 256, false));
  KHR_CHAIN(devAlloc(c, &c->d_fetch_done, 4));
  {
    const int zs = (cfg->voxels_per_side != 8 && (cfg->world_size >= 4 || cfg->max_frame_pixels <= 640u * 480u)) ? 8 : 4;
    c->fuse_zsplit = zs;
    c->wpb = static_cast<uint32_t>((cfg->voxels_per_side * cfg->voxels_per_side / 64) * zs);
    c->item_cap = static_cast<uint32_t>(cap) * c->wpb;
  }
  KHR_CHAIN(devAlloc(c, &c->d_work4, 2 * static_cast<size_t>(c->item_cap), false));
  if (cfg->voxels_per_side == 8 && rc == KHR_OK) {
    const size_t bits_words = static_cast<size_t>(c->item_cap) * 4;
    if (c->h_frames.alloc(kMaxMultiFrames) || c->d_frames.alloc(kMaxMultiFrames) || c->ev_frames.ensure() ||
        hipEventRecord(c->ev_frames, c->stream) != hipSuccess || c->d_frame_bits.alloc(bits_words) ||
        c->d_multi_list.alloc(2 * static_cast<size_t>(c->item_cap) + 1))
      rc = fail(KHR_ENOMEM, "buffers of the multi-frame update");
    if (rc == KHR_OK && (c->h_totals.alloc(C_COUNT + 2) || c->ev_up.ensure() || hipEventRecord(c->ev_up, c->stream) != hipSuccess ||
                         c->ev_dep.ensure() || c->ev_dep_aux.ensure()))
      rc = fail(KHR_ENOMEM, "page-locked words / events of an object mini-map");
  }
  KHR_CHAIN(devAlloc(c, &m.blk_band, cap * kBandSlots));
  KHR_CHAIN(devAlloc(c, &c->d_removed, cap));
  KHR_CHAIN(devAlloc(c, &c->d_mesh_count, cap + 1));
  KHR_CHAIN(devAlloc(c, &c->d_mesh_offset, cap + 1));
  KHR_CHAIN(devAlloc(c, &c->d_regen, cap));
  KHR_CHAIN(devAlloc(c, &c->d_mesh_old_off, cap + 1));
  KHR_CHAIN(devAlloc(c, &c->d_mh_flag, cap));
  KHR_CHAIN(devAlloc(c, &c->d_mesh_nwork, 8));
  const size_t npx = cfg->max_frame_pixels;
  KHR_CHAIN(devAlloc(c, &c->d_keys, npx, false));
  KHR_CHAIN(devAlloc(c, &c->d_pix, npx, false));
  {
    uint32_t ts = 1;
    while (ts < 2 * npx) ts <<= 1;
    c->md_mask = ts - 1;
    c->md_list_cap = static_cast<uint32_t>(std::min<size_t>(npx, 1u << 20));
    KHR_CHAIN(devAlloc(c, &c->d_md_keys, 3 * static_cast<size_t>(ts), false));
    KHR_CHAIN(devAlloc(c, &c->d_md_counts, 3 * static_cast<size_t>(ts), false));
    KHR_CHAIN(devAlloc(c, &c->d_md_ids, 3 * static_cast<size_t>(ts), false));
    {
      uint8_t* head = nullptr;
      KHR_CHAIN(devAlloc(c, &head, 16 + sizeof(CompAcc) * kCompCap));
      c->d_md_n = reinterpret_cast<uint32_t*>(head);
    }
    KHR_CHAIN(devAlloc(c, &c->d_md_parent, c->md_list_cap, false));
    KHR_CHAIN(devAlloc(c, &c->d_md_rootidx, c->md_list_cap, false));
    KHR_CHAIN(devAlloc(c, &c->d_md_edges, c->md_list_cap, false));
    KHR_CHAIN(devAlloc(c, &c->d_md_comp_acc, c->md_list_cap, false));
    KHR_CHAIN(devAlloc(c, &c->d_md_comp_final, kCompCap));
    KHR_CHAIN(c->h_md_head.alloc(16 + sizeof(CompAcc) * kCompCap));
    KHR_CHAIN(devAlloc(c, &c->d_md_scratch4, 16));
    c->md_host_walk = std::getenv("KHR_MD_HOST_WALK") != nullptr;
    if (const char* e = std::getenv("KHR_MD_LDS_MAX")) c->md_lds_max = std::min<uint32_t>(kCompLds, static_cast<uint32_t>(std::atoi(e)));
    KHR_CHAIN(devAlloc(c, &c->d_md_seed_keys, c->md_list_cap, false));
    KHR_CHAIN(devAlloc(c, &c->d_md_bnd_keys, c->md_list_cap, false));
    KHR_CHAIN(devAlloc(c, &c->d_md_seed_counts, c->md_list_cap, false));
    KHR_CHAIN(devAlloc(c, &c->d_md_bnd_counts, c->md_list_cap, false));
    KHR_CHAIN(devAlloc(c, &c->d_md_seed_final, c->md_list_cap, false));
    KHR_CHAIN(devAlloc(c, &c->d_md_bnd_final, c->md_list_cap, false));
    KHR_CHAIN(devAlloc(c, &c->d_md_bnd_deg, c->md_list_cap, false));
    KHR_CHAIN(devAlloc(c, &c->d_md_bnd_mask, c->md_list_cap, false));
    KHR_CHAIN(devAlloc(c, &c->d_md_adj, static_cast<size_t>(c->md_list_cap) * 26, false));
    KHR_CHAIN(c->h_md_walk.alloc(std::min<size_t>(c->md_list_cap, 16384) * (3 + 26 + 3 + 3) + 16));
    KHR_CHAIN(devAlloc(c, &c->d_md_acc, 256, false));
    KHR_CHAIN(c->h_md_acc_pinned.alloc(256));
    {
      std::vector<ClusterAcc> init(256);
      for (auto& a : init) clusterAccReset(a);
      KHR_CHAIN(hipMemcpy(c->d_md_acc, init.data(), sizeof(ClusterAcc) * 256, hipMemcpyHostToDevice) != hipSuccess ? KHR_EDEVICE : KHR_OK);
    }
  }
  if (rc == KHR_OK) {
    size_t t3 = 0;
    hipcub::DeviceScan::ExclusiveSum(nullptr, t3, c->d_mesh_count, c->d_mesh_offset, static_cast<int>(cap + 1), c->stream);
    c->cub_temp_bytes = t3 + 256;
    uint8_t* tmp = nullptr;
    KHR_CHAIN(devAlloc(c, &tmp, c->cub_temp_bytes, false));
    c->d_cub_temp = tmp;
  }
  for (int b = 0; b < 2 && rc == KHR_OK; ++b) {
    KHR_CHAIN(devAlloc(c, &c->mesh[b].points, cfg->max_mesh_vertices * 3, false));
    KHR_CHAIN(devAlloc(c, &c->mesh[b].colors, cfg->max_mesh_vertices, false));
    KHR_CHAIN(devAlloc(c, &c->mesh[b].labels, cfg->max_mesh_vertices, false));
    KHR_CHAIN(devAlloc(c, &c->mesh[b].stamps, cfg->max_mesh_vertices, false));
  }
  c->slots.resize(cfg->num_frame_slots);
  c->slot_leases.reset(new std::atomic<int>[cfg->num_frame_slots]);
  for (uint32_t i = 0; i < cfg->num_frame_slots; ++i) c->slot_leases[i].store(0);
  for (auto& s : c->slots) {
    if (rc != KHR_OK) break;
    KHR_CHAIN(devAlloc(c, &s.depth, npx, false));
    KHR_CHAIN(devAlloc(c, &s.range, npx + 4, false));
    KHR_CHAIN(devAlloc(c, &s.rgba, npx + 4, false));
    KHR_CHAIN(devAlloc(c, &s.label, npx, false));
    KHR_CHAIN(devAlloc(c, &s.dyn, npx));
    KHR_CHAIN(devAlloc(c, &s.dynw, npx, false));
    KHR_CHAIN(devAlloc(c, &s.obj, npx));
    KHR_CHAIN(devAlloc(c, &s.rgb_staging, npx * 3, false));
    KHR_CHAIN(devAlloc(c, &s.tile_max, npx / 16 + 64, false));
  }
  if (rc != KHR_OK) return rc;
  hipError_t e = hipMemsetAsync(m.ht_keys, 0xff, sizeof(uint64_t) * ht, c->stream);
  if (e == hipSuccess) {
    std::vector<uint32_t> ident(cap);
    for (size_t i = 0; i < cap; ++i) ident[i] = static_cast<uint32_t>(i);
    e = hipMemcpyAsync(m.free_slots, ident.data(), sizeof(uint32_t) * cap, hipMemcpyHostToDevice, c->stream);
    uint32_t ctr[C_COUNT] = {0};
    ctr[C_N_FREE] = static_cast<uint32_t>(cap);
    if (e == hipSuccess) e = hipMemcpyAsync(m.counters, ctr, sizeof(ctr), hipMemcpyHostToDevice, c->stream);
    if (e == hipSuccess) e = hipMemcpyToSymbol(HIP_SYMBOL(g_mc_tri), kMcTriTable, sizeof(kMcTriTable));
    if (e == hipSuccess) e = hipMemcpyToSymbol(HIP_SYMBOL(g_mc_ntri), kMcNumTris, sizeof(kMcNumTris));
    if (e == hipSuccess) e = hipStreamSynchronize(c->stream);
  }
  if (e != hipSuccess) return fail(KHR_EDEVICE, "context initialisation failed: %s", hipGetErrorString(e));
  {
    std::lock_guard<std::mutex> lock(g_live_mu);
    g_live_ctx.push_back(c);
  }
  *out = owner.release();
  return KHR_OK;
}

void khr_destroy(khr_ctx* c) {
  if (!c) return;
  {
    std::lock_guard<std::mutex> lock(g_live_mu);
    g_live_ctx.erase(std::remove(g_live_ctx.begin(), g_live_ctx.end(), c), g_live_ctx.end());
  }
  hipSetDevice(c->device);
  for (Stream* st : {&c->stream, &c->aux_stream, &c->h2d_stream, &c->snap_stream, &c->mc_stream, &c->copy_stream})
    if (*st) hipStreamSynchronize(*st);
  resolveTimers(c);
  if (c->pending_snapshot) khr_snapshot_release(c->pending_snapshot);
  {
    std::lock_guard<std::mutex> lock(c->snap_pool->mu);
    c->snap_pool->dead = true;
    c->snap_pool->free.clear();
  }
  {
    std::lock_guard<std::mutex> lock(c->frame_pool->mu);
    c->frame_pool->dead = true;
    c->frame_pool->free.clear();
  }
  delete c;
}

int khr_set_stream(khr_ctx* c, void* hip_stream) {
  if (!c) return fail(KHR_EINVAL, "null ctx");
  HIP_TRY(hipStreamSynchronize(c->stream));
  HIP_TRY(hipStreamSynchronize(c->aux_stream));
  if (hip_stream) {
    c->stream.refer(static_cast<hipStream_t>(hip_stream));
    return KHR_OK;
  }
  return createStream(c, c->stream);
}

int khr_sync(khr_ctx* c) {
  if (!c) return fail(KHR_EINVAL, "null ctx");
  HIP_TRY(hipStreamSynchronize(c->stream));
  HIP_TRY(hipStreamSynchronize(c->aux_stream));
  return KHR_OK;
}

static int auxAfterMain(khr_ctx* c) {
  HIP_TRY(hipEventRecord(c->ev_aux, c->stream));
  HIP_TRY(hipStreamWaitEvent(c->aux_stream, c->ev_aux, 0));
  return KHR_OK;
}

static int peekSlot(const khr_ctx* c) {
  const int n_slots = static_cast<int>(c->slots.size());
  for (int k = 0; k < n_slots; ++k) {
    const int cand = (c->next_slot + k) % n_slots;
    if (c->slot_leases[cand].load(std::memory_order_acquire) == 0) return cand;
  }
  return -1;
}

static int acquireSlot(khr_ctx* c) {
  const int n_slots = static_cast<int>(c->slots.size());
  int slot = -1;
  for (int k = 0; k < n_slots && slot < 0; ++k) {
    const int cand = (c->next_slot + k) % n_slots;
    if (c->slot_leases[cand].load(std::memory_order_acquire) == 0) slot = cand;
  }
  if (slot < 0) return fail(KHR_ENOMEM, "all %d frame slots are retained (raise num_frame_slots)", n_slots);
  c->next_slot = (slot + 1) % n_slots;
  if (c->slots[slot].aux_seq > c->aux_seq_done) {
    const uint64_t upto = c->aux_seq_issued;
    if (hipStreamQuery(c->aux_stream) != hipSuccess) HIP_TRY(hipStreamSynchronize(c->aux_stream));
    c->aux_seq_done = upto;
  }
  c->slots[slot].aux_seq = 0;
  FrameSlot& fs = c->slots[slot];
  fs.x_depth = fs.x_range = nullptr, fs.x_rgba = nullptr, fs.x_label = nullptr, fs.x_tile_max = nullptr;
  return slot;
}

static bool validSlot(const khr_ctx* c, int slot) {
  return slot >= 0 && slot < static_cast<int>(c->slots.size()) && c->slots[slot].valid;
}

// ... 920 lines not shown
    if (phases & 8) {
      ScopedTimer tm(c, 3);
      hipLaunchKernelGGL(k_init_blocks, dim3(2048), dim3(256), 0, c->stream, m, c->p, c->d_new);
      const FrameSlot& s0 = c->slots[slots[base]];
      if (one_launch && c->tick_mask_dirty)
        HIP_TRY(hipMemsetAsync(c->d_tick_mask, 0, sizeof(uint32_t) * (c->item_cap / 4 + 1), c->stream));
      c->tick_mask_dirty = one_launch;
      hipLaunchKernelGGL(k_tick_cull, dim3(256, nb), dim3(256), 0, c->stream, m, c->p, t, c->d_tick_work, cap, c->d_tick_work4, c->item_cap, c->wpb,
                         c->d_tick_counts, c->cfg.disable_culling ? 0 : 1, s0.tw, s0.th, one_launch ? c->d_tick_mask : nullptr);
      c->host_index_valid = false, ++c->map_gen;
      HIP_TRY(hipGetLastError());
    }
    if ((phases & 2) && one_launch) {
      rc = tickUpdateUnion(c, slots + base, t.f, nb, use_mask, object_id);
      if (rc) return rc;
    }
    for (int k = 0; k < nb && (phases & 2) && !one_launch; ++k) {
      FrameSlot& s = c->slots[slots[base + k]];
      UpdateLists lists;
      lists.list = FuseList{c->d_tick_work4 + static_cast<size_t>(2 * k) * c->item_cap, c->d_tick_work4 + static_cast<size_t>(2 * k + 1) * c->item_cap,
                            c->item_cap, &c->d_tick_counts[2 * kMaxTick + 4 * k]};
      rc = integrateUpdate(c, s, t.f[k], 1, use_mask, object_id, false, &lists);
      if (rc) return rc;
    }
    if (phases & 2) c->motion_ignore_epoch = 0;
  }
  return KHR_OK;
}

int khr_tick_live_bound(khr_ctx* c, int64_t* out_device, int n_out, int index) {
  if (!c || !out_device || n_out < 1 || index < 0 || index >= n_out) return fail(KHR_EINVAL, "bad argument");
  HIP_TRY(hipSetDevice(c->device));
  hipLaunchKernelGGL(k_live_bound, dim3(1), dim3(64), 0, c->stream, c->m, out_device, n_out, index);
  HIP_TRY(hipGetLastError());
  return KHR_OK;
}

int khr_export_halo(khr_ctx* c, void* records, int64_t cap_records, int on_device) {
  if (!c || !records || cap_records < 1) return fail(KHR_EINVAL, "bad argument");
  if (!c->cfg.with_tracking) return fail(KHR_ESTATE, "halo records need the tracking layer");
  HIP_TRY(hipSetDevice(c->device));
  DevMap& m = c->m;
  const size_t bytes = static_cast<size_t>(cap_records) * kHaloRecWords * sizeof(uint64_t);
  uint64_t* dst = static_cast<uint64_t*>(records);
  DevTemp holder;
  uint64_t* tmp = nullptr;
  if (!on_device) {
    KHR_TRY(holder.alloc(bytes));
    dst = tmp = holder.as<uint64_t>();
  }
  HIP_TRY(hipMemsetAsync(c->d_mesh_nwork + 1, 0, sizeof(uint32_t), c->stream));
  hipLaunchKernelGGL(k_list_live, dim3(gridFor(m.capacity)), dim3(256), 0, c->stream, m, c->d_work, c->d_mesh_nwork + 1, 0u);
  int rc = dispatchVps(c, [&](auto vps) {
    hipLaunchKernelGGL((k_export_halo<decltype(vps)::value>), dim3(1024), dim3(256), 0, c->stream, m, c->d_work,
                       c->d_mesh_nwork + 1, dst, static_cast<uint32_t>(cap_records));
    return KHR_OK;
  });
  if (rc == KHR_OK && !on_device) {
    hipError_t e = hipMemcpyAsync(records, tmp, bytes, hipMemcpyDeviceToHost, c->stream);
    if (e == hipSuccess) e = hipStreamSynchronize(c->stream);
    if (e != hipSuccess) rc = fail(KHR_EDEVICE, "halo export copy failed: %s", hipGetErrorString(e));
  }
  return rc;
}

int khr_import_halo(khr_ctx* c, const void* records, int64_t n_records, int on_device) {
  if (!c || (!records && n_records > 0) || n_records < 0) return fail(KHR_EINVAL, "bad argument");
  HIP_TRY(hipSetDevice(c->device));
  if (n_records == 0) {
    c->halo_n = 0;
    return KHR_OK;
  }
  uint32_t ht = 1;
  while (ht < static_cast<uint64_t>(n_records) * 4) ht <<= 1;
  if (static_cast<uint64_t>(n_records) > c->halo_cap_total) {
    HIP_TRY(hipStreamSynchronize(c->stream));
    c->halo_cap_total = 0;
    c->d_halo_keys.reset(), c->d_halo_vals.reset();
    KHR_TRY(c->d_halo_keys.alloc(ht));
    KHR_TRY(c->d_halo_vals.alloc(ht));
    c->halo_cap_total = static_cast<uint32_t>(n_records);
  }
  if (!on_device && static_cast<size_t>(n_records) * kHaloRecWords > c->d_halo_recs.count()) {
    HIP_TRY(hipStreamSynchronize(c->stream));
    KHR_TRY(c->d_halo_recs.reserve(static_cast<size_t>(n_records) * kHaloRecWords));
  }
  c->halo_mask = ht - 1;
  if (on_device) {
    c->halo_view = static_cast<const uint64_t*>(records);
  } else {
    HIP_TRY(hipMemcpyAsync(c->d_halo_recs, records, static_cast<size_t>(n_records) * kHaloRecWords * sizeof(uint64_t),
                           hipMemcpyHostToDevice, c->stream));
    c->halo_view = c->d_halo_recs;
  }
  HIP_TRY(hipMemsetAsync(c->d_halo_keys, 0xff, sizeof(uint64_t) * (static_cast<size_t>(c->halo_mask) + 1), c->stream));
  hipLaunchKernelGGL(k_import_halo, dim3(gridFor(n_records)), dim3(256), 0, c->stream, c->halo_view,
                     static_cast<uint32_t>(n_records), c->cfg.rank, c->cfg.world_size, c->d_halo_keys, c->d_halo_vals, c->halo_mask);
  HIP_TRY(hipGetLastError());
  if (!on_device) HIP_TRY(hipStreamSynchronize(c->stream));
  c->halo_n = static_cast<uint32_t>(n_records);
  return KHR_OK;
}

static int motionLaunch(khr_ctx* c, FrameSlot& s, bool fresh_slot, bool do_begin = false) {
  const size_t n = static_cast<size_t>(s.sensor.width) * s.sensor.height;
  if (!fresh_slot) {
    if (!s.dyn_clean) HIP_TRY(hipMemsetAsync(s.dyn, 0, n * sizeof(int32_t), c->stream));
    HIP_TRY(hipMemsetAsync(&c->m.counters[C_N_SEEDS], 0, sizeof(uint32_t), c->stream));
  }
  c->stats.n_seeds = 0;
  c->h_pinned[0] = 0;
  c->seed_by_ticket = false;
  if (!c->cfg.with_tracking) return KHR_OK;
  DevMap& m = c->m;
  const DevFrame f = makeDevFrame(c, s);
  const float min_z_world = static_cast<float>(s.meta.world_T_sensor[11] + static_cast<double>(c->cfg.md_min_z_coordinate));
  {
    ScopedTimer tm(c, 4);
    ++c->seed_ticket;
    if (c->seed_ticket == 0) ++c->seed_ticket;
    hipLaunchKernelGGL(k_motion_pixels, dim3(gridFor(n)), dim3(256), 0, c->stream, m, c->p, f, c->cfg.md_max_range,
                       min_z_world, c->d_keys, c->motion_ignore_epoch, do_begin ? c->d_wg_stats : nullptr);
    if (do_begin) c->begun = true;
  }
  HIP_TRY(hipGetLastError());
  c->seed_by_ticket = true;
  c->seed_publish_pending = true;
  return KHR_OK;
}

static void seedWaitDone(khr_ctx* c, std::chrono::steady_clock::time_point t0, bool event_path) {
  const uint64_t us = static_cast<uint64_t>(std::chrono::duration_cast<std::chrono::microseconds>(std::chrono::steady_clock::now() - t0).count());
  ++c->n_seed_waits;
  c->seed_wait_max_us = std::max(c->seed_wait_max_us, us);
  static const uint64_t edge[7] = {50, 100, 200, 500, 1000, 2000, 5000};
  int b = 0;
  while (b < 7 && us >= edge[b]) ++b;
  ++c->seed_wait_hist[b];
  if (us > 500) {
    ++c->n_seed_waits_late;
    c->seed_wait_late_us = us;
    c->seed_wait_late_frame = c->n_seed_waits;
    uint64_t st = 0;
    if (hipStreamQuery(c->stream) == hipErrorNotReady) st |= 1u;
    if (c->aux_stream && hipStreamQuery(c->aux_stream) == hipErrorNotReady) st |= 2u;
    if (c->h2d_stream && hipStreamQuery(c->h2d_stream) == hipErrorNotReady) st |= 4u;
    if (c->last_ingest_on_aux) st |= 8u;
    if (event_path) st |= 16u;
    st |= static_cast<uint64_t>(c->ahead_q.size()) << 8;
    c->seed_wait_late_state = st;
  }
}

static int waitSeedCount(khr_ctx* c) {
  const auto t_wait0 = std::chrono::steady_clock::now();
  if (!c->seed_by_ticket) {
    HIP_TRY(hipEventSynchronize(c->ev_seed));
    seedWaitDone(c, t_wait0, true);
    return KHR_OK;
  }
  if (c->seed_publish_pending) {
    hipLaunchKernelGGL(k_publish_seed, dim3(1), dim3(1), 0, c->stream, c->m, c->h_pinned.dev() + 2, c->seed_ticket);
    HIP_TRY(hipGetLastError());
    c->seed_publish_pending = false;
  }
  volatile uint32_t* hp = c->h_pinned;
  uint64_t spins = 0;
  while (hp[3] != c->seed_ticket) {
    __builtin_ia32_pause();
    if ((++spins & 0xffffu) == 0) {
      const hipError_t q = hipStreamQuery(c->stream);
      if (q != hipSuccess && q != hipErrorNotReady) return fail(KHR_EDEVICE, "stream failed while waiting for the seed count: %s", hipGetErrorString(q));
      if (q == hipSuccess && hp[3] != c->seed_ticket) return fail(KHR_EDEVICE, "seed count was never published");
    }
  }
  c->h_pinned[0] = hp[2];
  seedWaitDone(c, t_wait0, false);
  return KHR_OK;
}

static int waitTicket(khr_ctx* c, int word, uint32_t ticket, const char* what, hipStream_t stream = nullptr) {
  volatile uint32_t* hp = c->h_pinned;
  uint64_t spins = 0;
  if (!stream) stream = c->stream;
  while (hp[word] != ticket) {
    __builtin_ia32_pause();
    if ((++spins & 0xffffu) == 0) {
      const hipError_t q = hipStreamQuery(stream);
      if (q != hipSuccess && q != hipErrorNotReady) return fail(KHR_EDEVICE, "stream failed while waiting for %s: %s", what, hipGetErrorString(q));
      if (q == hipSuccess && hp[word] != ticket) return fail(KHR_EDEVICE, "%s was never published", what);
    }
  }
  return KHR_OK;
}

static int clusterSummaryLaunch(khr_ctx* c, FrameSlot& s, int max_id) {
  const int tiles = ((s.sensor.width + kAccTile - 1) / kAccTile) * ((s.sensor.height + kAccTile - 1) / kAccTile);
  hipLaunchKernelGGL(k_cluster_summary, dim3(tiles), dim3(1024), 0, c->stream, makeDevFrame(c, s), s.dyn, c->d_md_acc,
                     s.dynw_valid ? static_cast<const uint8_t*>(s.dynw) : nullptr);
  if (++c->md_acc_ticket == 0) ++c->md_acc_ticket;
  hipLaunchKernelGGL(k_publish_cluster_acc, dim3(1), dim3(256), 0, c->stream, c->d_md_acc, reinterpret_cast<uint32_t*>(c->h_md_acc_pinned.dev()),
                     static_cast<uint32_t>(std::min(max_id + 1, 256)), c->h_pinned.dev() + 7, c->md_acc_ticket);
  HIP_TRY(hipGetLastError());
  c->md_acc_slot = static_cast<int>(&s - c->slots.data());
  return KHR_OK;
}

struct MdHooks {
  bool no_device_merge, no_predict, no_prelaunch;
  uint32_t table_log2, prelaunch_px;
};
static MdHooks mdHooks() {
  static const bool no_device_merge = std::getenv("KHR_MD_NO_DEVICE_MERGE") != nullptr;
  MdHooks h{};
  h.no_device_merge = no_device_merge;
  h.no_predict = std::getenv("KHR_MD_NO_PREDICT") != nullptr;
  h.no_prelaunch = std::getenv("KHR_MD_NO_PRELAUNCH") != nullptr;
  if (const char* e = std::getenv("KHR_MD_TABLE_LOG2")) h.table_log2 = static_cast<uint32_t>(std::min(30, std::max(4, std::atoi(e))));
  if (const char* e = std::getenv("KHR_MD_PRELAUNCH_PX")) h.prelaunch_px = static_cast<uint32_t>(std::max(1, std::atoi(e)));
  return h;
}

static bool mdQueuesAhead(const khr_ctx* c, const MdHooks& hooks) { return c->md_seed_run && c->seed_by_ticket && !hooks.no_prelaunch; }

static uint32_t mdMaskFor(const khr_ctx* c, const MdHooks& hooks, uint32_t seed_pixels) {
  uint32_t ts = 1u << 14;
  while (ts < 2ull * std::max<uint32_t>(seed_pixels, 1u) && ts - 1 < c->md_mask) ts <<= 1;
  if (hooks.table_log2) ts = 1u << hooks.table_log2;
  return std::min(ts - 1, c->md_mask);
}

struct MdTables { VoxTable seeds, bnd, near; };
struct MdHead { uint32_t S, B, R, overflow; };
static int mdLaunchChain(khr_ctx* c, int n, uint32_t seed_pixels, uint32_t mask, bool global_components, bool device_merge, MdTables* t) {
  const uint32_t cap = c->md_list_cap;
  const int nn = c->cfg.md_neighbor_connectivity;
  CompAcc* d_comp_out = reinterpret_cast<CompAcc*>(reinterpret_cast<uint8_t*>(c->d_md_n) + 16);
  const uint32_t seed_px = std::min<uint32_t>(seed_pixels, cap);
  const size_t tsize = static_cast<size_t>(mask) + 1;
  const VoxTable seeds = t->seeds = VoxTable{c->d_md_keys, c->d_md_counts, c->d_md_ids, mask};
  const VoxTable bnd = t->bnd = VoxTable{c->d_md_keys + tsize, c->d_md_counts + tsize, c->d_md_ids + tsize, mask};
  const VoxTable near = t->near = VoxTable{c->d_md_keys + 2 * tsize, c->d_md_counts + 2 * tsize, c->d_md_ids + 2 * tsize, mask};
  int32_t* const d_box = reinterpret_cast<int32_t*>(c->d_md_scratch4) + 8;
  hipLaunchKernelGGL(k_md_clear, dim3(1024), dim3(256), 0, c->stream, c->d_md_keys, c->d_md_counts, static_cast<uint32_t>(tsize), c->d_md_n, d_box);
  hipLaunchKernelGGL(k_md_seed_insert, dim3(gridFor(n)), dim3(256), 0, c->stream, c->d_keys, n, seeds, c->d_md_n + 3);
  hipLaunchKernelGGL(k_md_compact, dim3(gridFor(tsize)), dim3(256), 0, c->stream, seeds, c->d_md_seed_keys, c->d_md_seed_counts, c->d_md_n, cap, nullptr);
  hipLaunchKernelGGL(k_md_near_insert, dim3(256), dim3(256), 0, c->stream, c->d_md_seed_keys, c->d_md_n, cap, nn, near, c->d_md_n + 3, d_box);
  hipLaunchKernelGGL(k_md_boundary_insert, dim3(gridFor(n)), dim3(256), 0, c->stream, c->d_keys, n, near, bnd, seeds, nn, 0, d_box, c->d_md_n + 3);
  hipLaunchKernelGGL(k_md_compact, dim3(gridFor(tsize)), dim3(256), 0, c->stream, bnd, c->d_md_bnd_keys, c->d_md_bnd_counts,
                     c->d_md_n + 1, cap, c->d_md_bnd_final, c->d_md_bnd_deg, c->d_md_bnd_mask);
  uint32_t* const d_n_edges = c->d_md_scratch4 + 15;
  hipLaunchKernelGGL(k_md_adjacency, dim3(1024), dim3(256), 0, c->stream, c->d_md_seed_keys, c->d_md_n, seeds, bnd, nn, cap,
                     c->d_md_adj, c->d_md_edges, cap, d_n_edges);
  hipLaunchKernelGGL(k_md_comp_lds, dim3(1), dim3(1024), 0, c->stream, c->d_md_adj, c->d_md_n, cap, nn, c->d_md_parent, c->d_md_comp_acc,
                     c->md_lds_max, c->d_md_edges, cap, d_n_edges, (c->p.dbg & 16) ? c->d_dbg : nullptr);
  if (global_components) {
    hipLaunchKernelGGL(k_md_comp_init, dim3(64), dim3(256), 0, c->stream, c->d_md_adj, c->d_md_n, cap, nn, c->d_md_parent, c->d_md_comp_acc,
                       c->md_lds_max);
    hipLaunchKernelGGL(k_md_comp_jump, dim3(64), dim3(256), 0, c->stream, c->d_md_n, cap, c->d_md_parent, c->md_lds_max);
    hipLaunchKernelGGL(k_md_comp_union, dim3(1024), dim3(256), 0, c->stream, c->d_md_adj, c->d_md_n, cap, nn, c->d_md_parent, c->md_lds_max);
  }
  hipLaunchKernelGGL(k_md_comp_reduce, dim3(gridFor(seed_px)), dim3(256), 0, c->stream, c->d_md_seed_keys, c->d_md_seed_counts,
                     c->d_md_bnd_keys, c->d_md_bnd_counts, c->d_md_adj, c->d_md_n, cap, nn, c->d_md_parent, c->d_md_comp_acc);
  hipLaunchKernelGGL(k_md_comp_roots, dim3(gridFor(seed_px)), dim3(256), 0, c->stream, c->d_md_n, cap, c->d_md_parent, c->d_md_comp_acc,
                     c->d_md_rootidx, c->d_md_n + 2, d_comp_out, kCompCap);
  if (device_merge) {
    hipLaunchKernelGGL(k_md_bnd_comps, dim3(256), dim3(256), 0, c->stream, c->d_md_bnd_keys, c->d_md_n, cap, nn, seeds, c->d_md_parent,
                       c->d_md_rootidx, c->d_md_bnd_mask);
    hipLaunchKernelGGL(k_md_comp_overlap, dim3(512), dim3(256), 0, c->stream, c->d_md_seed_keys, c->d_md_bnd_keys, c->d_md_n, cap,
                       c->cfg.md_min_separation_distance > 1.f ? 1 : 0, seeds, bnd, c->d_md_parent, c->d_md_rootidx, c->d_md_bnd_mask, d_comp_out);
  }
  HIP_TRY(hipGetLastError());
  if (++c->md_head_ticket == 0) ++c->md_head_ticket;
  hipLaunchKernelGGL(k_publish, dim3(1), dim3(1024), 0, c->stream, c->d_md_n, reinterpret_cast<uint32_t*>(c->h_md_head.dev()),
                     static_cast<uint32_t>(sizeof(CompAcc) / 4), kCompHead, c->h_pinned.dev() + 8, c->md_head_ticket, c->d_md_scratch4);
  HIP_TRY(hipGetLastError());
  return KHR_OK;
}

static int mdRunChain(khr_ctx* c, FrameSlot& s, const MdHooks& hooks, bool device_merge, MdTables* t, MdHead* head) {
  const int n = s.sensor.width * s.sensor.height;
  bool with_global = c->md_host_walk || 2u * c->md_last_seeds > c->md_lds_max || c->md_lds_max < kCompLds;
  if (hooks.no_predict) with_global = false;
  uint32_t pre_px = 0, pre_mask = 0;
  if (mdQueuesAhead(c, hooks)) {
    pre_px = hooks.prelaunch_px ? hooks.prelaunch_px : std::min<uint32_t>(c->md_list_cap, std::max<uint32_t>(4096u, 2u * c->md_prev_seed_px));
    pre_mask = mdMaskFor(c, hooks, pre_px);
    KHR_TRY(mdLaunchChain(c, n, pre_px, pre_mask, with_global, device_merge, t));
    ++c->n_md_prelaunched;
  }
  KHR_TRY(waitSeedCount(c));
  s.clusters.clear();
  c->md_seed_run = c->h_pinned[0] != 0;
  if (c->h_pinned[0] == 0) return 0;
  c->md_prev_seed_px = c->h_pinned[0];
  s.dyn_clean = false;
  bool chain_queued = pre_px != 0 && c->h_pinned[0] <= pre_px;
  if (pre_px != 0 && !chain_queued) ++c->n_md_prelaunch_repeats;
  uint32_t mask = chain_queued ? pre_mask : mdMaskFor(c, hooks, c->h_pinned[0]);
  const uint32_t* cnt = reinterpret_cast<const uint32_t*>(c->h_md_head.get());
  for (int attempt = 0;; ++attempt) {
    if (!chain_queued) KHR_TRY(mdLaunchChain(c, n, c->h_pinned[0], mask, with_global, device_merge, t));
    chain_queued = false;
    KHR_TRY(waitTicket(c, 8, c->md_head_ticket, "the motion detector's component records"));
    const bool table_full = cnt[3] && mask < c->md_mask;
    const bool lds_short = !table_full && cnt[0] > c->md_lds_max && !with_global;
    if (attempt == 2 || !(table_full || lds_short)) break;
    if (table_full) mask = c->md_mask;
    else with_global = true;
  }
  *head = MdHead{cnt[0], cnt[1], cnt[2], cnt[3]};
  c->md_last_seeds = head->S;
  if (head->overflow) return fail(KHR_ENOMEM, "motion detector: neighbour table overflow (%u seed voxels)", head->S);
  if (head->S > c->md_list_cap || head->B > c->md_list_cap)
    return fail(KHR_ENOMEM, "motion detector: %u seed / %u boundary voxels exceed the list capacity %u", head->S, head->B, c->md_list_cap);
  return 1;
}

static int mdPaintAndList(khr_ctx* c, FrameSlot& s, const MdTables& t, const mdh::Kept& kept, int* deferred_summary) {
  const int n = s.sensor.width * s.sensor.height;
  hipLaunchKernelGGL(k_md_paint, dim3(gridFor(n)), dim3(256), 0, c->stream, c->d_keys, n, t.seeds, t.bnd, c->d_md_seed_final,
                     c->d_md_bnd_final, s.dyn, c->d_md_bnd_deg, s.dynw);
  s.dyn_clean = false, s.dynw_valid = true;
  HIP_TRY(hipGetLastError());
  if (deferred_summary) *deferred_summary = kept.back().first;
  else KHR_TRY(clusterSummaryLaunch(c, s, kept.back().first));
  s.clusters.assign(kept.size(), khr_cluster{});
  for (size_t i = 0; i < kept.size(); ++i) {
    s.clusters[i].id = kept[i].first;
    s.clusters[i].num_pixels_listed = kept[i].second;
    s.clusters[i].semantic_id = -1;
  }
  return static_cast<int>(kept.size());
}

static int mdFinishFromRecords(khr_ctx* c, FrameSlot& s, const MdTables& t, const CompAcc* comp, uint32_t R, bool merge_here, int* deferred_summary) {
  const std::vector<uint32_t> order = mdh::clusterOrder(comp, R);
  const std::vector<uint32_t> group = merge_here ? mdh::groupsFromRows(comp, R) : mdh::Groups(R).labels();
  std::vector<int32_t> ids;
  const mdh::Kept kept = mdh::numberClusters(order.data(), group.data(), R, [&](uint32_t r) { return comp[r].n_pixels; },
                                             c->cfg.md_min_cluster_size, c->cfg.md_max_cluster_size, &ids);
  if (kept.empty()) return 0;
  CompFinals inl{};
  const int32_t* fin_dev = nullptr;
  if (R <= static_cast<uint32_t>(kCompInline)) {
    std::copy(ids.begin(), ids.end(), inl.id);
  } else {
    int32_t* fin = reinterpret_cast<int32_t*>(c->h_md_head.get());
    std::copy(ids.begin(), ids.end(), fin);
    HIP_TRY(hipMemcpyAsync(c->d_md_comp_final, fin, sizeof(int32_t) * R, hipMemcpyHostToDevice, c->stream));
    fin_dev = c->d_md_comp_final;
  }
  hipLaunchKernelGGL(k_md_comp_finals, dim3(1024), dim3(256), 0, c->stream, c->d_md_adj, c->d_md_n, c->md_list_cap, c->cfg.md_neighbor_connectivity,
                     c->d_md_parent, c->d_md_rootidx, fin_dev, inl, c->d_md_seed_final, c->d_md_bnd_final, c->d_md_bnd_deg);
  return mdPaintAndList(c, s, t, kept, deferred_summary);
}

static void mdCopyWords(khr_ctx* c, const void* src, void* dst, size_t words) {
  if (words) hipLaunchKernelGGL(k_copy_words, dim3(static_cast<unsigned>((words + 255) / 256)), dim3(256), 0, c->stream,
                                static_cast<const uint32_t*>(src), static_cast<uint32_t*>(dst), static_cast<uint32_t>(words));
}

static int mdFinishByWalk(khr_ctx* c, FrameSlot& s, const MdTables& t, const MdHead& head, int* deferred_summary) {
  const size_t S = head.S, B = head.B, nn = static_cast<size_t>(c->cfg.md_neighbor_connectivity);
  const size_t o_sk = 0, o_bk = o_sk + 2 * S, o_sc = o_bk + 2 * B, o_adj = o_sc + S, o_bc = o_adj + S * nn;
  const size_t o_sf = o_bc + B, o_bf = o_sf + S, o_bd = o_bf + B, walk_words = o_bd + B + 16;
  if (c->ev_md_walk_up) HIP_TRY(hipEventSynchronize(c->ev_md_walk_up));
  if (walk_words > c->h_md_walk.count()) {
    const size_t want = std::max<size_t>(2 * walk_words, 1u << 18);
    if (c->h_md_walk.reserve(want)) return fail(KHR_ENOMEM, "page-locked block of the motion detector's host walk (%zu bytes)", want * 4);
  }
  KHR_TRY(c->ev_md_walk_up.ensure());
  uint32_t *const w = c->h_md_walk, *const w_dev = c->h_md_walk.dev();
  mdCopyWords(c, c->d_md_seed_keys, w_dev + o_sk, 2 * S);
  mdCopyWords(c, c->d_md_bnd_keys, w_dev + o_bk, 2 * B);
  mdCopyWords(c, c->d_md_seed_counts, w_dev + o_sc, S);
  mdCopyWords(c, c->d_md_adj, w_dev + o_adj, S * nn);
  mdCopyWords(c, c->d_md_bnd_counts, w_dev + o_bc, B);
  HIP_TRY(hipGetLastError());
  HIP_TRY(hipStreamSynchronize(c->stream));
  const mdh::WalkLists lists{reinterpret_cast<const uint64_t*>(w + o_sk), reinterpret_cast<const uint64_t*>(w + o_bk), w + o_sc, w + o_bc, w + o_adj,
                             head.S, head.B, static_cast<int>(nn)};
  const mdh::Kept kept = mdh::walkClusters(lists, c->cfg.md_min_separation_distance, c->cfg.md_min_cluster_size, c->cfg.md_max_cluster_size,
                                        reinterpret_cast<int32_t*>(w + o_sf), reinterpret_cast<int32_t*>(w + o_bf), reinterpret_cast<int32_t*>(w + o_bd));
  if (kept.empty()) return 0;
  mdCopyWords(c, w_dev + o_sf, c->d_md_seed_final, S);
  mdCopyWords(c, w_dev + o_bf, c->d_md_bnd_final, B);
  mdCopyWords(c, w_dev + o_bd, c->d_md_bnd_deg, B);
  HIP_TRY(hipEventRecord(c->ev_md_walk_up, c->stream));
  return mdPaintAndList(c, s, t, kept, deferred_summary);
}

static int motionFinish(khr_ctx* c, FrameSlot& s, int* deferred_summary = nullptr) {
  if (deferred_summary) *deferred_summary = -1;
  if (!c->cfg.with_tracking) return 0;
  const MdHooks hooks = mdHooks();
  const float sep = c->cfg.md_min_separation_distance;
  const bool device_merge = !hooks.no_device_merge && !c->md_host_walk && sep > 0.f && sep <= 2.f;
  MdTables t{};
  MdHead head{};
  const int rc = mdRunChain(c, s, hooks, device_merge, &t, &head);
  if (rc <= 0) return rc;
  c->stats.n_seeds = head.S;
  if (head.R <= kCompCap && !c->md_host_walk) {
    if (head.R > kCompHead) {
      HIP_TRY(hipMemcpyAsync(c->h_md_head, c->d_md_n, 16 + sizeof(CompAcc) * head.R, hipMemcpyDeviceToHost, c->stream));
      HIP_TRY(hipStreamSynchronize(c->stream));
    }
    const CompAcc* comp = reinterpret_cast<const CompAcc*>(c->h_md_head + 16);
    const bool may_merge = mdh::mayMerge(comp, head.R, sep);
    const bool merge_here = may_merge && device_merge && head.R <= 64;
    if (merge_here) ++c->n_md_device_merges;
    if (!may_merge || merge_here) return mdFinishFromRecords(c, s, t, comp, head.R, merge_here, deferred_summary);
  }
  ++c->n_md_host_walks;
  return mdFinishByWalk(c, s, t, head, deferred_summary);
}

int khr_detect_motion(khr_ctx* c, int slot) {
  if (!c || !validSlot(c, slot)) return fail(KHR_EINVAL, "bad slot");
  HIP_TRY(hipSetDevice(c->device));
  FrameSlot& s = c->slots[slot];
  int rc = motionLaunch(c, s, false);
  if (rc) return rc;
  return motionFinish(c, s);
}

int khr_motion_keys(khr_ctx* c, int slot, void* keys_out, int on_device, uint32_t* n_seed_pixels) {
  if (!c || !keys_out || !validSlot(c, slot)) return fail(KHR_EINVAL, "bad argument");
  HIP_TRY(hipSetDevice(c->device));
  FrameSlot& s = c->slots[slot];
  const int n = s.sensor.width * s.sensor.height;
  int rc = motionLaunch(c, s, false);
  if (rc) return rc;
  uint64_t* dst = static_cast<uint64_t*>(keys_out);
  DevTemp holder;
  if (!on_device) {
    KHR_TRY(holder.alloc(sizeof(uint64_t) * n));
    dst = holder.as<uint64_t>();
  }
  hipLaunchKernelGGL(k_md_keys_export, dim3(gridFor(n)), dim3(256), 0, c->stream, c->d_keys, n, dst);
  if (!on_device) {
    HIP_TRY(hipMemcpyAsync(keys_out, dst, sizeof(uint64_t) * n, hipMemcpyDeviceToHost, c->stream));
    HIP_TRY(hipStreamSynchronize(c->stream));
  }
  if (!n_seed_pixels && on_device) {
    c->seed_publish_pending = false;
    c->seed_by_ticket = false;
    return KHR_OK;
  }
  { const int rcw = waitSeedCount(c); if (rcw) return rcw; }
  if (n_seed_pixels) *n_seed_pixels = c->h_pinned[0];
  return KHR_OK;
}

int khr_detect_motion_from_keys(khr_ctx* c, int slot, const void* keys, int on_device) {
  if (!c || !keys || !validSlot(c, slot)) return fail(KHR_EINVAL, "bad argument");
  HIP_TRY(hipSetDevice(c->device));
  FrameSlot& s = c->slots[slot];
  const int n = s.sensor.width * s.sensor.height;
  const uint64_t* src = static_cast<const uint64_t*>(keys);
  DevTemp holder;
  if (!on_device) {
    KHR_TRY(holder.alloc(sizeof(uint64_t) * n));
    HIP_TRY(hipMemcpyAsync(holder.get(), keys, sizeof(uint64_t) * n, hipMemcpyHostToDevice, c->stream));
    src = holder.as<uint64_t>();
  }
  if (!s.dyn_clean) HIP_TRY(hipMemsetAsync(s.dyn, 0, sizeof(int32_t) * n, c->stream));
  s.dyn_clean = true, s.dynw_valid = false;
  HIP_TRY(hipMemsetAsync(&c->m.counters[C_N_SEEDS], 0, sizeof(uint32_t), c->stream));
  hipLaunchKernelGGL(k_md_keys_import, dim3(gridFor(n)), dim3(256), 0, c->stream, src, n, c->d_keys, &c->m.counters[C_N_SEEDS]);
  HIP_TRY(hipMemcpyAsync(&c->h_pinned[0], &c->m.counters[C_N_SEEDS], sizeof(uint32_t), hipMemcpyDeviceToHost, c->stream));
  HIP_TRY(hipEventRecord(c->ev_seed, c->stream));
  c->seed_by_ticket = false;
  return motionFinish(c, s);
}

size_t khr_motion_bits_bytes(int64_t n_pixels) { return n_pixels > 0 ? 16u * static_cast<size_t>((n_pixels + 63) / 64) : 0u; }

int khr_motion_bits(khr_ctx* c, int slot, void* bits_device) {
  if (!c || !bits_device || !validSlot(c, slot)) return fail(KHR_EINVAL, "bad argument");
  HIP_TRY(hipSetDevice(c->device));
  FrameSlot& s = c->slots[slot];
  const int n = s.sensor.width * s.sensor.height;
  int rc = motionLaunch(c, s, false);
  if (rc) return rc;
  hipLaunchKernelGGL(k_md_bits_export, dim3(gridFor((static_cast<size_t>(n) + 63) / 64 * 64)), dim3(256), 0, c->stream, c->d_keys, n,
                     static_cast<unsigned long long*>(bits_device));
  HIP_TRY(hipGetLastError());
  c->seed_publish_pending = false;
  c->seed_by_ticket = false;
  return KHR_OK;
}

int khr_detect_motion_from_bits(khr_ctx* c, int slot, const void* bits_device) {
  if (!c || !bits_device || !validSlot(c, slot)) return fail(KHR_EINVAL, "bad argument");
  HIP_TRY(hipSetDevice(c->device));
  FrameSlot& s = c->slots[slot];
  const int n = s.sensor.width * s.sensor.height;
  if (!s.dyn_clean) HIP_TRY(hipMemsetAsync(s.dyn, 0, sizeof(int32_t) * n, c->stream));
  s.dyn_clean = true, s.dynw_valid = false;
  HIP_TRY(hipMemsetAsync(&c->m.counters[C_N_SEEDS], 0, sizeof(uint32_t), c->stream));
  const float min_z_world = static_cast<float>(s.meta.world_T_sensor[11] + static_cast<double>(c->cfg.md_min_z_coordinate));
  hipLaunchKernelGGL(k_md_keys_from_bits, dim3(gridFor(n)), dim3(256), 0, c->stream, c->p, makeDevFrame(c, s), c->cfg.md_max_range, min_z_world,
                     static_cast<const unsigned long long*>(bits_device), c->d_keys, &c->m.counters[C_N_SEEDS]);
  HIP_TRY(hipMemcpyAsync(&c->h_pinned[0], &c->m.counters[C_N_SEEDS], sizeof(uint32_t), hipMemcpyDeviceToHost, c->stream));
  HIP_TRY(hipEventRecord(c->ev_seed, c->stream));
  c->seed_by_ticket = false;
  return motionFinish(c, s);
}

int khr_dynamic_pack_bytes(khr_ctx* c, int slot, void* dst_device) {
  if (!c || !dst_device || !validSlot(c, slot)) return fail(KHR_EINVAL, "bad argument");
  HIP_TRY(hipSetDevice(c->device));
  FrameSlot& s = c->slots[slot];
  const int n4 = (s.sensor.width * s.sensor.height + 3) / 4;
  hipLaunchKernelGGL(k_dyn_pack_u8, dim3(gridFor(n4)), dim3(256), 0, c->stream, s.dyn, n4, static_cast<uint32_t*>(dst_device));
  HIP_TRY(hipGetLastError());
  return KHR_OK;
}

int khr_dynamic_unpack_bytes(khr_ctx* c, int slot, const void* src_device) {
  if (!c || !src_device || !validSlot(c, slot)) return fail(KHR_EINVAL, "bad argument");
  HIP_TRY(hipSetDevice(c->device));
  FrameSlot& s = c->slots[slot];
  const int n4 = (s.sensor.width * s.sensor.height + 3) / 4;
  hipLaunchKernelGGL(k_dyn_unpack_u8, dim3(gridFor(n4)), dim3(256), 0, c->stream, static_cast<const uint32_t*>(src_device), n4, s.dyn);
  HIP_TRY(hipGetLastError());
  s.dyn_clean = false;
  s.dynw_valid = false;
  return KHR_OK;
}

int khr_mirror_dynamic(khr_ctx* c, int src, int dst) {
  if (!c) return fail(KHR_EINVAL, "null ctx");
  if (!validSlot(c, src) || !validSlot(c, dst)) return fail(KHR_EINVAL, "bad slot");
  if (src == dst) return KHR_OK;
  FrameSlot& a = c->slots[src];
  FrameSlot& b = c->slots[dst];
  if (a.sensor.width != b.sensor.width || a.sensor.height != b.sensor.height) return fail(KHR_EINVAL, "the slots hold frames of different sizes");
  HIP_TRY(hipSetDevice(c->device));
  if (!(a.dyn_clean && b.dyn_clean)) {
    HIP_TRY(hipMemcpyAsync(b.dyn, a.dyn, sizeof(int32_t) * static_cast<size_t>(a.sensor.width) * a.sensor.height, hipMemcpyDeviceToDevice, c->stream));
    if (a.dynw_valid)
      HIP_TRY(hipMemcpyAsync(b.dynw, a.dynw, static_cast<size_t>(a.sensor.width) * a.sensor.height, hipMemcpyDeviceToDevice, c->stream));
  }
  b.dyn_clean = a.dyn_clean;
  b.dynw_valid = a.dynw_valid;
  b.clusters = a.clusters;
  return KHR_OK;
}

int khr_get_dynamic_clusters(khr_ctx* c, int slot, khr_cluster* out, int cap) {
  if (!c || cap < 0 || (!out && cap > 0)) return fail(KHR_EINVAL, "bad argument");
  if (!validSlot(c, slot)) return fail(KHR_EINVAL, "bad slot");
  const int n = static_cast<int>(c->slots[slot].clusters.size());
// ... 918 lines not shown

static int ingestAhead(khr_ctx* c, const khr_sensor* sensor, const khr_frame* frame, int on_device) {
  if (!c || !sensor || !frame) return fail(KHR_EINVAL, "null argument");
  if (c->ahead_q.size() >= kMaxAhead)
    return fail(KHR_ESTATE, "%zu frames handed over by khr_ingest_ahead are still waiting for khr_process_frame (khr_ingest_cancel drops them)", c->ahead_q.size());
  const int next = peekSlot(c);
  if (!c->cfg.with_tracking || c->slots.size() < 3 + c->ahead_q.size() || next < 0 || next == c->last_frame_slot) return KHR_ENOTFOUND;
  HIP_TRY(hipSetDevice(c->device));
  if (!pointerIs(frame->depth, on_device) || !pointerIs(frame->color, on_device) || !pointerIs(frame->label, on_device))
    return fail(KHR_EINVAL, on_device ? "khr_ingest_ahead: the frame's buffers must be device memory" : "khr_ingest_ahead_host: the frame's buffers must be page-locked host memory (hipHostMalloc / hipHostRegister)");
  const int evi = c->ahead_ev_next;
  for (const auto& e : c->ahead_q)
    if (e.ev == evi) return fail(KHR_ESTATE, "look-ahead event ring out of step");
  hipStream_t conv_stream = c->aux_stream;
  if (!on_device) {
    if (!c->h2d_stream) KHR_TRY(createStream(c, c->h2d_stream));
    conv_stream = c->h2d_stream;
  }
  IngestOpts opts;
  opts.stream = conv_stream;
  opts.pinned = !on_device;
  opts.h2d_event = &c->ev_ahead_h2d[evi];
  const int slot = uploadFrame(c, sensor, frame, on_device, opts);
  if (slot < 0) return slot;
  auto undo = [&](int rc) {
    c->slots[slot].valid = false;
    if (!on_device && c->ev_ahead_h2d[evi]) hipEventSynchronize(c->ev_ahead_h2d[evi]);
    return rc;
  };
  if (c->ev_ahead[evi].ensure()) return undo(fail(KHR_EDEVICE, "hipEventCreate failed"));
  if (hipEventRecord(c->ev_ahead[evi], conv_stream) != hipSuccess) return undo(fail(KHR_EDEVICE, "hipEventRecord failed"));
  if (on_device) c->slots[slot].aux_seq = ++c->aux_seq_issued;
  if (on_device && c->obj_configured && c->obj_pending_slot < 0 && c->ahead_q.empty()) {
    const int rco = objectsLaunch(c, slot);
    if (rco) {
      if (c->obj_pending_slot == slot) c->obj_pending_slot = -1;
      return undo(rco);
    }
  }
  c->slot_leases[slot].fetch_add(1, std::memory_order_acq_rel);
  c->ahead_q.push_back({slot, evi, !on_device});
  c->ahead_ev_next ^= 1;
  return slot;
}

int khr_ingest_ahead(khr_ctx* c, const khr_sensor* sensor, const khr_frame* frame) { return ingestAhead(c, sensor, frame, 1); }
int khr_ingest_ahead_host(khr_ctx* c, const khr_sensor* sensor, const khr_frame* frame) { return ingestAhead(c, sensor, frame, 0); }
int khr_ingest_cancel(khr_ctx* c) {
  if (!c) return fail(KHR_EINVAL, "null ctx");
  if (c->ahead_q.empty()) return KHR_ENOTFOUND;
  cancelAhead(c);
  return KHR_OK;
}

static int snapshotUpdated(khr_ctx* c, hipStream_t st, uint32_t fields, int64_t cap_blocks, khr_snapshot** out);

int khr_process_frame(khr_ctx* c, const khr_sensor* sensor, const khr_frame* frame, int on_device, uint32_t flags,
                      int* n_clusters) {
  if (!c) return fail(KHR_EINVAL, "null ctx");
  HT("pf_enter");
  if (n_clusters) *n_clusters = 0;
  const bool motion = (flags & KHR_PF_MOTION) != 0;
  const bool objects = (flags & KHR_PF_OBJECTS) != 0;
  const bool ahead = (flags & KHR_PF_INGESTED) != 0;
  if (ahead && (c->ahead_q.empty() || !frame || !motion || !(flags & KHR_PF_INPUT_READY) ||
                c->slots[c->ahead_q.front().slot].meta.timestamp_ns != frame->timestamp_ns)) {
    cancelAhead(c);
    return fail(KHR_ESTATE, "KHR_PF_INGESTED: the oldest frame handed over by khr_ingest_ahead does not carry this stamp (or flags are missing); the handed-over frames were dropped");
  }
  if (!ahead && !c->ahead_q.empty()) return fail(KHR_ESTATE, "the frames handed over by khr_ingest_ahead have to be processed first (khr_ingest_cancel drops them)");
  const bool pinned_in = !on_device && (flags & KHR_PF_INPUT_PINNED) != 0;
  if (pinned_in && !ahead && frame && (!pointerIs(frame->depth, 0) || !pointerIs(frame->color, 0) || !pointerIs(frame->label, 0)))
    return fail(KHR_EINVAL, "KHR_PF_INPUT_PINNED: the frame's buffers must be page-locked host memory (hipHostMalloc / hipHostRegister)");
  struct Leave {
    khr_ctx* c;
    bool ok = false;
    ~Leave() {
      if (!ok && c->fold_pending) {
        hipLaunchKernelGGL(k_fuse_fold, dim3((c->m.capacity + 255) / 256), dim3(256), 0, c->stream, c->m.blk_flags, c->m.blk_band,
                           &c->m.counters[C_MAX_SLOT], static_cast<const uint32_t*>(nullptr));
        c->fold_pending = false;
      }
      if (c->h2d_pending) {
        hipEventSynchronize(c->ev_h2d);
        c->h2d_pending = false;
      }
      if (own_h2d) hipEventSynchronize(own_h2d);
    }
    hipEvent_t own_h2d = nullptr;
  } leave{c};
  const bool early = ahead || ((flags & KHR_PF_INPUT_READY) && (on_device || pinned_in) && motion && c->cfg.with_tracking &&
                               c->slots.size() >= (pinned_in ? 3u : 2u) && peekSlot(c) != c->last_frame_slot);
  int slot;
  int ahead_ev = 0;
  if (ahead) {
    const khr_ctx::AheadEntry e = c->ahead_q.front();
    c->ahead_q.erase(c->ahead_q.begin());
    slot = e.slot;
    ahead_ev = e.ev;
    if (e.host) leave.own_h2d = c->ev_ahead_h2d[e.ev];
    c->slot_leases[slot].fetch_sub(1, std::memory_order_acq_rel);
  } else {
    c->last_ingest_on_aux = early;
    IngestOpts opts;
    opts.stream = early ? static_cast<hipStream_t>(c->aux_stream) : nullptr;
    opts.pinned = pinned_in;
    opts.begin = !early;
    slot = uploadFrame(c, sensor, frame, on_device, opts);
    if (slot < 0) return slot;
  }
  c->last_frame_slot = slot;
  FrameSlot& s = c->slots[slot];
  const DevFrame f = makeDevFrame(c, s);
  int rc = KHR_OK;
  if (ahead) {
    c->begun = false;
    HIP_TRY(hipStreamWaitEvent(c->stream, c->ev_ahead[ahead_ev], 0));
  } else if (early) {
    c->begun = false;
    s.aux_seq = ++c->aux_seq_issued;
    HIP_TRY(hipEventRecord(c->ev_aux_done, c->aux_stream));
    HIP_TRY(hipStreamWaitEvent(c->stream, c->ev_aux_done, 0));
  }
  if (objects && !c->obj_configured) return fail(KHR_ESTATE, "KHR_PF_OBJECTS needs khr_configure_object_detector");
  if (objects && !early) {
    KHR_TRY(c->ev_ingest.ensure());
    HIP_TRY(hipEventRecord(c->ev_ingest, c->stream));
  }
  if (motion && (rc = motionLaunch(c, s, true, early))) return rc;
  if ((rc = integrateAlloc(c, s, f, 1))) return rc;
  HT("pf_alloc_launched");
  if (objects) {
    if (!(ahead && c->obj_pending_slot == slot)) {
      if (!early) HIP_TRY(hipStreamWaitEvent(c->aux_stream, c->ev_ingest, 0));
      if (ahead) HIP_TRY(hipStreamWaitEvent(c->aux_stream, c->ev_ahead[ahead_ev], 0));
      if ((rc = objectsLaunch(c, slot))) return rc;
    }
    HT("pf_objects_launched");
  }
  bool speculated = false;
  size_t spec_timer = static_cast<size_t>(-1), spec_end = 0;
  const bool tracking = (flags & KHR_PF_TRACKING) && c->cfg.with_tracking;
  const bool defer_fold = tracking;
  if (motion && c->cfg.with_tracking && !mdQueuesAhead(c, mdHooks())) {
    const size_t n_pending = c->pending.size();
    rc = integrateUpdate(c, s, f, 1, 0, -1, defer_fold, nullptr, &c->m.counters[C_N_SEEDS]);
    if (rc) return rc;
    if (c->pending.size() > n_pending) spec_timer = n_pending;
    spec_end = c->pending.size();
    speculated = true;
  }
  bool have_seeds = false;
  int summary_pending = -1;
  if (motion) {
    const int nc = motionFinish(c, s, &summary_pending);
    if (nc < 0) return nc;
    if (n_clusters) *n_clusters = nc;
    have_seeds = c->cfg.with_tracking && c->h_pinned[0] != 0;
  }
  HT("pf_motion_done");
  if (speculated && have_seeds && spec_timer != static_cast<size_t>(-1))
    for (size_t i = spec_timer; i < spec_end && i < c->pending.size(); ++i) c->pending[i].which = -1;
  if (!speculated || have_seeds) {
    rc = integrateUpdate(c, s, f, 1, motion ? 1 : 0, -1, defer_fold);
    if (rc) return rc;
  }
  if (summary_pending >= 0 && (rc = clusterSummaryLaunch(c, s, summary_pending))) return rc;
  const bool mc_fork = (flags & KHR_PF_OUTPUT) && tracking;
  if (mc_fork) {
    if (!c->mc_stream) KHR_TRY(createStream(c, c->mc_stream));
    KHR_TRY(c->ev_mc_fork.ensure());
    KHR_TRY(c->ev_mc_join.ensure());
  }
  if (tracking) {
    HIP_TRY(hipSetDevice(c->device));
    if ((rc = trackingPhase(c, frame->timestamp_ns, 3, mc_fork ? static_cast<hipEvent_t>(c->ev_mc_fork) : nullptr))) return rc;
  }
  const bool early_list = (flags & KHR_PF_OUTPUT) && c->cfg.with_tracking;
  if (mc_fork) {
    HIP_TRY(hipStreamWaitEvent(c->mc_stream, c->ev_mc_fork, 0));
    if ((rc = generateMesh(c, c->mc_stream, 1, 1))) return rc;
    HIP_TRY(hipEventRecord(c->ev_mc_join, c->mc_stream));
  }
  HT("pf_update_launched");
  if (flags & KHR_PF_OUTPUT) {
    const bool snap = (flags & KHR_PF_SNAPSHOT) != 0;
    if (snap) {
      if (c->pending_snapshot) khr_snapshot_release(c->pending_snapshot);
      c->pending_snapshot = nullptr;
      if (!c->snap_stream) KHR_TRY(createStream(c, c->snap_stream));
      KHR_TRY(c->ev_snap_fork.ensure());
      KHR_TRY(c->ev_snap_join.ensure());
      HIP_TRY(hipEventRecord(c->ev_snap_fork, c->stream));
      HIP_TRY(hipStreamWaitEvent(c->snap_stream, c->ev_snap_fork, 0));
      const int64_t snap_cap = c->cfg.max_snapshot_blocks ? c->cfg.max_snapshot_blocks : 8192;
      if ((rc = snapshotUpdated(c, c->snap_stream, KHR_SNAP_ALL, snap_cap, &c->pending_snapshot))) return rc;
      HIP_TRY(hipEventRecord(c->ev_snap_join, c->snap_stream));
    }
    if (early_list && (rc = removedPublishLaunch(c))) return rc;
    if (mc_fork) HIP_TRY(hipStreamWaitEvent(c->stream, c->ev_mc_join, 0));
    else if ((rc = generateMesh(c, c->stream, 1, 1))) return rc;
    if (snap) HIP_TRY(hipStreamWaitEvent(c->stream, c->ev_snap_join, 0));
    if (c->cfg.with_tracking) {
      if ((rc = resetInactiveLaunch(c, early_list, BLK_UPDATED))) return rc;
    } else if ((rc = khr_clear_updated(c))) {
      return rc;
    }
    c->removed_early = early_list;
    HT("pf_output_launched");
  }
  if (objects) {
    const int ns = objectsFinish(c, slot);
    if (ns < 0) return ns;
  }
  HT("pf_exit");
  leave.ok = true;
  return slot;
}

int khr_mark_all_inactive(khr_ctx* c) {
  if (!c) return fail(KHR_EINVAL, "null ctx");
  hipLaunchKernelGGL(k_block_flag_op, dim3(gridFor(c->m.capacity)), dim3(256), 0, c->stream, c->m, ~BLK_HAS_ACTIVE, BLK_TRACK_DIRTY);
  HIP_TRY(hipGetLastError());
  c->host_index_valid = false, ++c->map_gen;
  return KHR_OK;
}

int khr_clear_updated(khr_ctx* c) {
  if (!c) return fail(KHR_EINVAL, "null ctx");
  hipLaunchKernelGGL(k_block_flag_op, dim3(gridFor(c->m.capacity)), dim3(256), 0, c->stream, c->m, ~BLK_UPDATED, 0u);
  HIP_TRY(hipGetLastError());
  c->host_index_valid = false, ++c->map_gen;
  return KHR_OK;
}

int khr_allocate_blocks(khr_ctx* c, const int32_t* indices, int64_t n) {
  if (!c || (!indices && n > 0)) return fail(KHR_EINVAL, "null argument");
  if (n <= 0) return KHR_OK;
  HIP_TRY(hipSetDevice(c->device));
  std::vector<std::array<int32_t, 3>> v(n);
  for (int64_t i = 0; i < n; ++i) v[i] = {indices[3 * i], indices[3 * i + 1], indices[3 * i + 2]};
  std::sort(v.begin(), v.end());
  v.erase(std::unique(v.begin(), v.end()), v.end());
  const size_t bytes = sizeof(int32_t) * 3 * v.size();
  HT("ab_enter");
  if (c->ev_up) HIP_TRY(hipEventSynchronize(c->ev_up));
  KHR_TRY(c->ev_up.ensure());
  HT("ab_prev_upload_consumed");
  if (bytes > c->h_up.count()) {
    HIP_TRY(hipStreamSynchronize(c->stream));
    const size_t want = std::max<size_t>(2 * bytes, 1u << 16);
    if (c->h_up.reserve(want)) return fail(KHR_ENOMEM, "block index staging of %zu bytes", want);
  }
  std::memcpy(c->h_up, v.data(), bytes);
  HIP_TRY(hipMemsetAsync(&c->m.counters[C_N_NEW], 0, sizeof(uint32_t), c->stream));
  c->explicit_blocks += v.size();
  hipLaunchKernelGGL(k_alloc_list, dim3(gridFor(v.size())), dim3(256), 0, c->stream, c->m, static_cast<const int*>(c->h_up.dev()),
                     static_cast<int>(v.size()), c->d_new);
  HIP_TRY(hipEventRecord(c->ev_up, c->stream));
  hipLaunchKernelGGL(k_init_blocks, dim3(2048), dim3(256), 0, c->stream, c->m, c->p, c->d_new);
  HIP_TRY(hipGetLastError());
  c->host_index_valid = false, ++c->map_gen;
  return KHR_OK;
}

int khr_object_prune(khr_ctx* c, float min_confidence, float min_observations, int64_t* n_pruned) {
  if (!c) return fail(KHR_EINVAL, "null ctx");
  if (!c->cfg.with_semantics || c->p.K < 2) return fail(KHR_ESTATE, "object pruning needs a binary semantic layer");
  HIP_TRY(hipMemsetAsync(&c->m.stats[S_PRUNED], 0, sizeof(unsigned long long), c->stream));
  int rc = dispatchVps(c, [&](auto vps) {
    hipLaunchKernelGGL((k_object_prune<decltype(vps)::value>), dim3(kStreamGrid), dim3(256), 0, c->stream, c->m, c->p,
                       min_confidence, min_observations);
    return KHR_OK;
  });
  if (rc) return rc;
  if (n_pruned) {
    unsigned long long np = 0;
    HIP_TRY(hipMemcpyAsync(&np, &c->m.stats[S_PRUNED], sizeof(np), hipMemcpyDeviceToHost, c->stream));
    HIP_TRY(hipStreamSynchronize(c->stream));
    *n_pruned = static_cast<int64_t>(np);
  }
  return KHR_OK;
}

static int refreshMeshTotals(khr_ctx* c);

int64_t khr_pool_exhausted(khr_ctx* c) {
  if (!c) return fail(KHR_EINVAL, "null ctx");
  const int rc = readCounters(c);
  if (rc) return rc;
  return static_cast<int64_t>(c->h_counters[C_POOL_EXHAUSTED]);
}

int khr_get_stats(khr_ctx* c, khr_stats* out) {
  if (!c || !out) return fail(KHR_EINVAL, "null argument");
  int rc = readCounters(c);
  if (rc) return rc;
  unsigned long long st[S_COUNT];
  HIP_TRY(hipMemcpy(st, c->m.stats, sizeof(st), hipMemcpyDeviceToHost));
  rc = ensureHostIndex(c);
  if (rc) return rc;
  rc = refreshMeshTotals(c);
  if (rc) return rc;
  khr_stats s = c->stats;
  s.n_allocated_blocks = c->host_index.size();
  s.n_visible_blocks = c->h_counters[C_N_VISIBLE];
  s.n_new_blocks = c->h_counters[C_N_NEW];
  s.n_visited_voxels = static_cast<uint64_t>(c->h_counters[C_N_VISIBLE]) * c->p.nvox;
  std::vector<uint32_t> wgs(2 * kUpdateStatSlots);
  HIP_TRY(hipMemcpy(wgs.data(), c->d_wg_stats, sizeof(uint32_t) * wgs.size(), hipMemcpyDeviceToHost));
  uint64_t cur_upd = 0, cur_band = 0;
  for (int i = 0; i < kUpdateStatSlots; ++i) {
    cur_upd += wgs[2 * i];
    cur_band += wgs[2 * i + 1];
  }
  s.n_updated_voxels = cur_upd;
  s.n_band_voxels = cur_band;
  s.n_tracking_updated_blocks = c->h_counters[c->ef_cur ? C_N_EF2 : C_N_EF_A];
  s.pool_exhausted = c->h_counters[C_POOL_EXHAUSTED];
  s.n_tsdf_blocks = c->h_counters[C_N_TSDF];
  s.n_fuse_items = static_cast<uint64_t>(c->h_counters[C_N_ITEMS0]) + c->h_counters[C_N_ITEMS1] + c->h_counters[C_N_ITEMS2] +
                   c->h_counters[C_N_ITEMS3];
  s.n_seed_waits = c->n_seed_waits;
  s.n_seed_waits_late = c->n_seed_waits_late;
  s.seed_wait_max_us = c->seed_wait_max_us;
  for (int i = 0; i < 8; ++i) s.seed_wait_hist[i] = c->seed_wait_hist[i];
  s.seed_wait_late_us = c->seed_wait_late_us;
  s.seed_wait_late_frame = c->seed_wait_late_frame;
  s.seed_wait_late_state = c->seed_wait_late_state;
  s.n_md_device_merges = c->n_md_device_merges;
  s.n_md_host_walks = c->n_md_host_walks;
  s.n_md_prelaunched = c->n_md_prelaunched;
  s.n_md_prelaunch_repeats = c->n_md_prelaunch_repeats;
  s.band_overflow = 0;
  s.n_tracking_processed_blocks = c->h_counters[c->ef_cur ? C_N_PROC2 : C_N_PROC];
  s.cum_updated_voxels = st[S_CUM_UPD] + cur_upd;
  s.cum_band_voxels = st[S_CUM_BAND] + cur_band;
  s.cum_visited_voxels = st[S_CUM_VISITED] + s.n_visited_voxels;
  s.cum_integrate_calls = st[S_CUM_CALLS];
  *out = s;
  return KHR_OK;
}

int64_t khr_num_blocks(khr_ctx* c) {
  if (!c) return fail(KHR_EINVAL, "null ctx");
  int rc = ensureHostIndex(c);
  if (rc) return rc;
  return static_cast<int64_t>(c->host_index.size());
}

int64_t khr_block_indices(khr_ctx* c, int32_t* out, int64_t cap, int only_updated) {
  if (!c) return fail(KHR_EINVAL, "null ctx");
  int rc = ensureHostIndex(c);
  if (rc) return rc;
  int64_t n = 0;
  for (auto& kv : c->host_index) {
    if (only_updated && !(c->host_flags[kv.second] & BLK_UPDATED)) continue;
    if (out && n < cap) {
      out[3 * n] = kv.first[0];
      out[3 * n + 1] = kv.first[1];
      out[3 * n + 2] = kv.first[2];
    }
    ++n;
  }
  return n;
}

int khr_download_block(khr_ctx* c, int32_t bx, int32_t by, int32_t bz, float* distance, float* weight,
                       uint8_t* color_rgba, uint64_t* last_observed, uint64_t* last_occupied, uint8_t* voxel_flags,
                       uint32_t* sem_label, float* likelihoods, uint8_t* block_flags) {
  if (!c) return fail(KHR_EINVAL, "null ctx");
  int rc = ensureHostIndex(c);
  if (rc) return rc;
  auto it = c->host_index.find({bx, by, bz});
  if (it == c->host_index.end()) return fail(KHR_ENOTFOUND, "block (%d,%d,%d) not allocated", bx, by, bz);
  const size_t slot = it->second, nv = c->p.nvox;
  const DevMap& m = c->m;
  auto D = [&](void* dst, const void* src, size_t bytes) { return hipMemcpyAsync(dst, src, bytes, hipMemcpyDeviceToHost, c->stream); };
  if (distance) HIP_TRY(D(distance, m.dist + slot * nv, nv * 4));
  if (weight) HIP_TRY(D(weight, m.weight + slot * nv, nv * 4));
  if (color_rgba) HIP_TRY(D(color_rgba, m.color + slot * nv, nv * 4));
  std::vector<uint8_t> raw_flags;
  if (voxel_flags || (last_occupied && c->cfg.with_tracking)) {
    raw_flags.resize(nv);
    HIP_TRY(D(raw_flags.data(), m.vflags + slot * nv, nv));
  }
  std::vector<uint64_t> obs_words;
  if (last_observed) {
    if (c->cfg.with_tracking) {
      HIP_TRY(D(last_observed, m.last_obs + slot * nv, nv * 8));
      obs_words.resize(2 * (nv / 64));
      HIP_TRY(D(obs_words.data(), m.obs + slot * (nv / 64), (nv / 64) * 16));
    } else std::memset(last_observed, 0, nv * 8);
  }
  if (last_occupied) {
    if (c->cfg.with_tracking) HIP_TRY(D(last_occupied, m.last_occ + slot * nv, nv * 8));
    else std::memset(last_occupied, 0, nv * 8);
  }
  if (sem_label) {
    if (c->cfg.with_semantics) HIP_TRY(D(sem_label, m.sem_label + slot * nv, nv * 4));
    else std::memset(sem_label, 0, nv * 4);
  }
  std::vector<float> lik_vm;
  if (likelihoods && c->cfg.with_semantics) {
    lik_vm.resize(nv * c->p.KS);
    HIP_TRY(D(lik_vm.data(), m.lik + slot * nv * c->p.KS, nv * c->p.KS * 4));
  }
  uint32_t bf = 0;
  if (block_flags) HIP_TRY(D(&bf, m.blk_flags + slot, 4));
  HIP_TRY(hipStreamSynchronize(c->stream));
  if (block_flags) *block_flags = static_cast<uint8_t>(bf & 0xfu);
  for (size_t w = 0; w < obs_words.size() / 2; ++w)
    for (int b = 0; b < 64; ++b)
      if ((obs_words[2 * w] >> b) & 1ull) last_observed[64 * w + b] = obs_words[2 * w + 1];
  if (last_occupied && c->cfg.with_tracking)
    for (size_t i = 0; i < nv; ++i)
      if (raw_flags[i] & VOX_OCC) last_occupied[i] = c->last_track_stamp;
  if (voxel_flags)
    for (size_t i = 0; i < nv; ++i) voxel_flags[i] = raw_flags[i] & VOX_PUBLIC_MASK;
  if (likelihoods && c->cfg.with_semantics)
    for (size_t i = 0; i < nv; ++i)
      for (int k = 0; k < c->p.K; ++k) likelihoods[static_cast<size_t>(k) * nv + i] = lik_vm[i * c->p.KS + k];
  if (likelihoods && c->cfg.with_semantics) {
    std::vector<uint8_t> fl(nv);
    const uint8_t* f = voxel_flags;
    if (!f) {
      HIP_TRY(hipMemcpy(fl.data(), m.vflags + slot * nv, nv, hipMemcpyDeviceToHost));
      f = fl.data();
    }
    for (size_t i = 0; i < nv; ++i)
      if (!(f[i] & VOX_SEM_VALID))
        for (int k = 0; k < c->p.K; ++k) likelihoods[static_cast<size_t>(k) * nv + i] = 0.f;
  }
  return KHR_OK;
}

int khr_slice_voxel_z(float height, float voxel_size, int32_t voxels_per_side, int64_t* voxel_z) {
  if (!voxel_z || !(voxel_size > 0.f) || voxels_per_side < 1 || !std::isfinite(height)) return fail(KHR_EINVAL, "bad argument");
  const float bs = voxel_size * static_cast<float>(voxels_per_side), bs_inv = 1.f / bs, vs_inv = 1.f / voxel_size;
  const float fb = std::floor(height * bs_inv);
  if (!(std::fabs(fb) < 1e15f)) return fail(KHR_EINVAL, "slice height %g is out of range", static_cast<double>(height));
  const int64_t bz = static_cast<int64_t>(fb);
  const float origin = static_cast<float>(bz) * bs;
  const int64_t v = static_cast<int64_t>(std::floor((height - origin) * vs_inv));
  *voxel_z = bz * voxels_per_side + v;
  return KHR_OK;
}

struct SliceLayout {
  size_t xy, pos, dist, weight, obs, flags, bytes;
  SliceLayout(size_t cap, size_t np) {
    auto al = [](size_t b) { return (b + 255) / 256 * 256; };
    xy = 256;
    pos = xy + al(cap * 8);
    dist = pos + al(cap * np * 12);
    weight = dist + al(cap * np * 4);
    obs = weight + al(cap * np * 4);
    flags = obs + al(cap * np * 8);
    bytes = flags + al(cap * np);
  }
};

static int ensureSortKeys(khr_ctx* c) {
  if (c->d_slice_keys) return KHR_OK;
  const uint32_t sort_len = slicePadded(c->m.capacity);
  if (c->d_slice_keys.alloc(sort_len) || c->d_slice_count.alloc(1)) {
    c->d_slice_keys.reset();
    return fail(KHR_ENOMEM, "sort keys (%u words)", sort_len);
  }
  return KHR_OK;
}
static int sortKeys(khr_ctx* c) {
  const uint32_t sort_len = slicePadded(c->m.capacity);
  hipLaunchKernelGGL(k_slice_sort_tile, dim3(std::max(1u, sort_len / kSliceSortTile)), dim3(kSliceSortThreads), 0, c->stream,
                     c->d_slice_keys, c->d_slice_count, 0u);
  HIP_TRY(hipGetLastError());
  for (uint32_t k = 2 * kSliceSortTile; k <= sort_len; k <<= 1) {
    for (uint32_t j = k / 2; j >= kSliceSortTile; j >>= 1) {
      hipLaunchKernelGGL(k_slice_sort_step, dim3(std::min(gridFor(sort_len / 2), 1024)), dim3(256), 0, c->stream, c->d_slice_keys,
                         c->d_slice_count, k, j);
      HIP_TRY(hipGetLastError());
    }
    hipLaunchKernelGGL(k_slice_sort_tile, dim3(sort_len / kSliceSortTile), dim3(kSliceSortThreads), 0, c->stream, c->d_slice_keys,
                       c->d_slice_count, k);
    HIP_TRY(hipGetLastError());
  }
// ... 1846 lines not shown
```

Baseline: 4158.

## Finish motion-detector cluster numbering on device and queue gated tail work

Adds a single-block kernel that checks the component records, merges nearby components and numbers clusters on the GPU, then publishes the result to pinned host memory. The comp_finals and paint kernels, plus a speculative integrate, are queued behind it and gated by a device verdict word. The host no longer waits for the records, numbers them on the CPU and only then launches the tail. When the verdict says the host must handle the case, the gated kernels exit early and the queued integrate timers are discarded, at the cost of more complex control flow and some extra kernel launches.

Result: no change. 4164 (median of 3 runs) (+0.2%).

```diff
diff --git a/include/khronos_amd.h b/include/khronos_amd.h
--- a/include/khronos_amd.h
+++ b/include/khronos_amd.h
@@ -114,6 +114,7 @@
   uint64_t n_md_host_walks;
   uint64_t n_md_prelaunched;
   uint64_t n_md_prelaunch_repeats;
+  uint64_t n_md_device_finishes;
 } khr_stats;
 
 typedef struct khr_cluster {
diff --git a/khronos_amd/capi.py b/khronos_amd/capi.py
--- a/khronos_amd/capi.py
+++ b/khronos_amd/capi.py
@@ -143,7 +143,7 @@
         "n_tracking_processed_blocks", "n_fuse_items", "n_seed_waits", "n_seed_waits_late", "seed_wait_max_us")] + [
         ("seed_wait_hist", C.c_uint64 * 8)] + [(n, C.c_uint64) for n in (
         "seed_wait_late_us", "seed_wait_late_frame", "seed_wait_late_state", "n_md_device_merges", "n_md_host_walks",
-        "n_md_prelaunched", "n_md_prelaunch_repeats")]
+        "n_md_prelaunched", "n_md_prelaunch_repeats", "n_md_device_finishes")]
 
 
 EXPORTS = [
diff --git a/khronos_amd/csrc/khr_kernels_aux.h b/khronos_amd/csrc/khr_kernels_aux.h
--- a/khronos_amd/csrc/khr_kernels_aux.h
+++ b/khronos_amd/csrc/khr_kernels_aux.h
@@ -165,7 +165,8 @@
 }
 
 __global__ __launch_bounds__(256) void k_md_clear(uint64_t* __restrict__ keys, uint32_t* __restrict__ counts, uint32_t tsize,
-                                                 uint32_t* __restrict__ n4, int32_t* __restrict__ aabb) {
+                                                 uint32_t* __restrict__ n4, int32_t* __restrict__ aabb, uint32_t* __restrict__ verdict,
+                                                 const volatile uint32_t* __restrict__ seed_px_host) {
   const uint32_t stride = gridDim.x * blockDim.x;
   const uint32_t t0 = blockIdx.x * blockDim.x + threadIdx.x;
   ulonglong2* k2 = reinterpret_cast<ulonglong2*>(keys);
@@ -175,6 +176,8 @@
   if (t0 < 4) n4[t0] = 0u;
   if (t0 < 6) aabb[t0] = t0 < 3 ? INT32_MAX : INT32_MIN;
   if (t0 == 7) aabb[7] = 0;
+  if (t0 == 8) *verdict = mdh::kMdPending;
+  if (t0 == 64) verdict[sizeof(mdh::MdFinish) / 4] = *seed_px_host;
 }
 
 __global__ __launch_bounds__(256) void k_md_seed_insert(const uint64_t* __restrict__ keys, int n, VoxTable seeds,
@@ -617,6 +620,80 @@
   }
 }
 
+struct NumberArgs {
+  uint32_t force;
+  uint32_t device_merge, global_components, pre_px, mask, full_mask, list_cap, lds_max;
+  float sep;
+  int min_size, max_size;
+};
+__global__ __launch_bounds__(256) void k_md_number_publish(const uint32_t* __restrict__ src, NumberArgs a, int32_t* __restrict__ comp_final,
+                                                          uint32_t* __restrict__ fin, volatile uint32_t* __restrict__ dst_host,
+                                                          volatile uint32_t* __restrict__ fin_host, volatile uint32_t* __restrict__ ticket_host,
+                                                          uint32_t ticket, uint32_t* __restrict__ counters_to_zero) {
+  constexpr uint32_t N = mdh::kNumberMax, kRecWords = sizeof(CompAcc) / 4, kFinWords = sizeof(mdh::MdFinish) / 4;
+  __shared__ CompAcc comp[N];
+  __shared__ mdh::NumberWork w;
+  __shared__ mdh::MdFinish out;
+  __shared__ int32_t ids[N];
+  const uint32_t S = src[0], B = src[1], R = src[2], overflow = src[3];
+  const uint32_t seed_px = fin[kFinWords];
+  uint32_t verdict = a.force;
+  if (!verdict) {
+    if (overflow) verdict = a.mask < a.full_mask ? mdh::kMdHostTableFull : mdh::kMdHostOverflow;
+    else if (S > a.list_cap || B > a.list_cap) verdict = mdh::kMdHostListCap;
+    else if (seed_px > a.pre_px) verdict = mdh::kMdHostPrePx;
+    else if (S > a.lds_max && !a.global_components) verdict = mdh::kMdHostLdsShort;
+    else if (R > N) verdict = mdh::kMdHostManyComps;
+  }
+  const uint32_t n_recs = min(R, N);
+  if (threadIdx.x < 4) dst_host[threadIdx.x] = src[threadIdx.x];
+  for (uint32_t i = threadIdx.x; i < n_recs * kRecWords; i += blockDim.x) {
+    const uint32_t word = src[4 + i];
+    reinterpret_cast<uint32_t*>(comp)[i] = word;
+    dst_host[4 + i] = word;
+  }
+  __syncthreads();
+  int near = 0;
+  if (!verdict) {
+    for (uint32_t p = threadIdx.x; p < n_recs * N; p += blockDim.x) {
+      const uint32_t i = p / N, j = p % N;
+      if (i < j && j < n_recs && mdh::pairMayMerge(comp, i, j, a.sep)) near = 1;
+    }
+    if (threadIdx.x < n_recs) w.order[mdh::clusterRank(comp, n_recs, threadIdx.x)] = threadIdx.x;
+  }
+  const bool may_merge = __syncthreads_or(near) != 0;
+  if (!verdict && may_merge && !a.device_merge) verdict = mdh::kMdHostMergeOff;
+  if (threadIdx.x == 0) {
+    uint32_t n_kept = 0;
+    if (!verdict) {
+      if (may_merge) mdh::groupsFromRowsN(comp, n_recs, w.group);
+      else for (uint32_t r = 0; r < n_recs; ++r) w.group[r] = r;
+      n_kept = mdh::numberClustersN(w.order, w.group, n_recs, [&](uint32_t r) { return comp[r].n_pixels; }, a.min_size, a.max_size, w.gpx, w.gid,
+                                    ids, out.kept_id, out.kept_px);
+    }
+    out.verdict = verdict;
+    out.n_kept = n_kept;
+    out.max_id = n_kept ? out.kept_id[n_kept - 1] : 0u;
+    out.merged = !verdict && may_merge ? 1u : 0u;
+  }
+  __syncthreads();
+  if (!verdict && threadIdx.x < n_recs) comp_final[threadIdx.x] = ids[threadIdx.x];
+  const uint32_t n_kept = out.n_kept;
+  for (uint32_t i = threadIdx.x; i < kFinWords; i += blockDim.x)
+    if (i < 4u + n_kept || (i >= 4u + N && i < 4u + N + 2u * n_kept)) {
+      const uint32_t word = reinterpret_cast<const uint32_t*>(&out)[i];
+      fin[i] = word;
+      fin_host[i] = word;
+    }
+  __threadfence_system();
+  __syncthreads();
+  if (threadIdx.x < 4) counters_to_zero[threadIdx.x] = 0u;
+  if (threadIdx.x == 0) {
+    *ticket_host = ticket;
+    __threadfence_system();
+  }
+}
+
 constexpr int kCompInline = 64;
 struct CompFinals {
   int32_t id[kCompInline];
@@ -624,7 +701,9 @@
 __global__ __launch_bounds__(256) void k_md_comp_finals(const uint32_t* __restrict__ adj, const uint32_t* __restrict__ n_seeds, uint32_t cap,
                                                        int nn, const uint32_t* __restrict__ parent, const uint32_t* __restrict__ root_idx,
                                                        const int32_t* __restrict__ comp_final, CompFinals inl, int32_t* __restrict__ seed_final,
-                                                       int32_t* __restrict__ bnd_final, int32_t* __restrict__ bnd_deg) {
+                                                       int32_t* __restrict__ bnd_final, int32_t* __restrict__ bnd_deg,
+                                                       const uint32_t* __restrict__ fin_gate) {
+  if (fin_gate != nullptr && (fin_gate[0] != 0u || fin_gate[1] == 0u)) return;
   const uint32_t ns = min(*n_seeds, cap);
   for (uint32_t i = blockIdx.x * blockDim.x + threadIdx.x; i < ns * nn; i += gridDim.x * blockDim.x) {
     const uint32_t s = i / nn, j = i % nn;
@@ -669,7 +748,9 @@
 __global__ __launch_bounds__(256) void k_md_paint(const uint64_t* __restrict__ keys, int n, VoxTable seeds, VoxTable bnd,
                                                  const int32_t* __restrict__ seed_final,
                                                  const int32_t* __restrict__ bnd_final, int32_t* __restrict__ dyn,
-                                                 const int32_t* __restrict__ bnd_deg, uint8_t* __restrict__ dyn_weight) {
+                                                 const int32_t* __restrict__ bnd_deg, uint8_t* __restrict__ dyn_weight,
+                                                 const uint32_t* __restrict__ fin_gate) {
+  if (fin_gate != nullptr && (fin_gate[0] != 0u || fin_gate[1] == 0u)) return;
   const int i = blockIdx.x * blockDim.x + threadIdx.x;
   if (i >= n) return;
   const uint64_t k = keys[i];
diff --git a/khronos_amd/csrc/khr_md_host.h b/khronos_amd/csrc/khr_md_host.h
--- a/khronos_amd/csrc/khr_md_host.h
+++ b/khronos_amd/csrc/khr_md_host.h
@@ -6,6 +6,12 @@
 #include <utility>
 #include <vector>
 
+#if defined(__HIPCC__)
+#define KHR_MD_HD __host__ __device__
+#else
+#define KHR_MD_HD
+#endif
+
 namespace khr {
 
 struct CompAcc {
@@ -22,79 +28,147 @@
   return Vox{{static_cast<int64_t>(key & 0x1fffffu) - (1 << 20), static_cast<int64_t>((key >> 21) & 0x1fffffu) - (1 << 20),
               static_cast<int64_t>((key >> 42) & 0x1fffffu) - (1 << 20)}};
 }
-inline bool closerThan(int64_t n2, float sep) { return static_cast<float>(static_cast<int64_t>(std::sqrt(static_cast<double>(n2)))) < sep; }
+KHR_MD_HD inline bool closerThan(int64_t n2, float sep) { return static_cast<float>(static_cast<int64_t>(std::sqrt(static_cast<double>(n2)))) < sep; }
 template <class A, class B>
-inline bool boxesCloserThan(const A& a, const B& b, float sep) {
+KHR_MD_HD inline bool boxesCloserThan(const A& a, const B& b, float sep) {
   int64_t gap2 = 0;
   for (int d = 0; d < 3; ++d) {
-    const int64_t gp = std::max<int64_t>(0, std::max(static_cast<int64_t>(a.lo[d]) - b.hi[d], static_cast<int64_t>(b.lo[d]) - a.hi[d]));
+    const int64_t ab = static_cast<int64_t>(a.lo[d]) - b.hi[d], ba = static_cast<int64_t>(b.lo[d]) - a.hi[d];
+    const int64_t far = ab > ba ? ab : ba, gp = far > 0 ? far : 0;
     gap2 += gp * gp;
   }
   return closerThan(gap2, sep);
 }
 
-inline std::vector<uint32_t> clusterOrder(const CompAcc* comp, uint32_t R) {
-  std::vector<uint32_t> order(R);
-  std::iota(order.begin(), order.end(), 0u);
-  std::sort(order.begin(), order.end(), [&](uint32_t a, uint32_t b) { return comp[a].min_key < comp[b].min_key; });
-  return order;
-}
-
-inline bool mayMerge(const CompAcc* comp, uint32_t R, float sep) {
+constexpr uint32_t kNumberMax = 64;
+
+KHR_MD_HD inline uint32_t clusterRank(const CompAcc* comp, uint32_t R, uint32_t i) {
+  const unsigned long long ki = comp[i].min_key;
+  uint32_t rank = 0;
+  for (uint32_t j = 0; j < R; ++j) rank += (comp[j].min_key < ki || (comp[j].min_key == ki && j < i)) ? 1u : 0u;
+  return rank;
+}
+KHR_MD_HD inline void clusterOrderN(const CompAcc* comp, uint32_t R, uint32_t* order) {
+  for (uint32_t i = 0; i < R; ++i) order[clusterRank(comp, R, i)] = i;
+}
+
+KHR_MD_HD inline bool pairMayMerge(const CompAcc* comp, uint32_t i, uint32_t j, float sep) { return boxesCloserThan(comp[i], comp[j], sep); }
+KHR_MD_HD inline bool mayMergeN(const CompAcc* comp, uint32_t R, float sep) {
   for (uint32_t i = 0; i < R; ++i)
     for (uint32_t j = i + 1; j < R; ++j)
-      if (boxesCloserThan(comp[i], comp[j], sep)) return true;
+      if (pairMayMerge(comp, i, j, sep)) return true;
   return false;
 }
 
-struct Groups {
-  std::vector<uint32_t> rep;
-  explicit Groups(uint32_t n) : rep(n) { std::iota(rep.begin(), rep.end(), 0u); }
-  uint32_t find(uint32_t x) {
-    while (rep[x] != x) x = rep[x] = rep[rep[x]];
-    return x;
-  }
-  void unite(uint32_t a, uint32_t b) {
-    a = find(a), b = find(b);
-    if (a != b) rep[std::max(a, b)] = std::min(a, b);
-  }
-  std::vector<uint32_t> labels() {
-    for (uint32_t i = 0; i < rep.size(); ++i) rep[i] = find(i);
-    return rep;
-  }
-};
-
-inline std::vector<uint32_t> groupsFromRows(const CompAcc* comp, uint32_t R) {
-  Groups g(R);
+KHR_MD_HD inline uint32_t groupFind(uint32_t* rep, uint32_t x) {
+  while (rep[x] != x) x = rep[x] = rep[rep[x]];
+  return x;
+}
+KHR_MD_HD inline void groupUnite(uint32_t* rep, uint32_t a, uint32_t b) {
+  a = groupFind(rep, a), b = groupFind(rep, b);
+  if (a != b) rep[a > b ? a : b] = a > b ? b : a;
+}
+KHR_MD_HD inline unsigned long long overlapRow(const CompAcc& a) { return (static_cast<unsigned long long>(a.pad) << 32) | a.root; }
+
+KHR_MD_HD inline void groupsFromRowsN(const CompAcc* comp, uint32_t R, uint32_t* group) {
+  for (uint32_t i = 0; i < R; ++i) group[i] = i;
   for (uint32_t i = 0; i < R && i < 64; ++i) {
-    unsigned long long row = ((static_cast<unsigned long long>(comp[i].pad) << 32) | comp[i].root) & ~(1ull << i);
+    unsigned long long row = overlapRow(comp[i]) & ~(1ull << i);
     for (; row; row &= row - 1ull) {
       const uint32_t j = static_cast<uint32_t>(__builtin_ctzll(row));
-      if (j < R) g.unite(i, j);
-    }
-  }
-  return g.labels();
-}
-
-using Kept = std::vector<std::pair<int, uint64_t>>;
+      if (j < R) groupUnite(group, i, j);
+    }
+  }
+  for (uint32_t i = 0; i < R; ++i) group[i] = groupFind(group, i);
+}
+
 template <class Px>
-inline Kept numberClusters(const uint32_t* order, const uint32_t* group, uint32_t R, Px px, int min_size, int max_size, std::vector<int32_t>* id_out) {
-  Kept kept;
-  id_out->assign(R, 0);
-  std::vector<uint64_t> gpx(R, 0);
-  std::vector<int32_t> gid(R, -1);
+KHR_MD_HD inline uint32_t numberClustersN(const uint32_t* order, const uint32_t* group, uint32_t R, Px px, int min_size, int max_size,
+                                          unsigned long long* gpx, int32_t* gid, int32_t* id_out, uint32_t* kept_id, unsigned long long* kept_px) {
+  for (uint32_t r = 0; r < R; ++r) { gpx[r] = 0; gid[r] = -1; }
   for (uint32_t r = 0; r < R; ++r) gpx[group[r]] += px(r);
+  uint32_t n_kept = 0;
   int id = 1;
   for (uint32_t k = 0; k < R; ++k) {
     const uint32_t r = order[k], g = group[r];
     if (gid[g] < 0) {
       const int size = static_cast<int>(gpx[g]);
       gid[g] = size < min_size || size > max_size ? 0 : id;
-      if (gid[g]) kept.emplace_back(id, gpx[g]);
-      if (gid[g] && id < 255) ++id;
-    }
-    (*id_out)[r] = gid[g];
-  }
+      if (gid[g]) {
+        kept_id[n_kept] = static_cast<uint32_t>(id);
+        kept_px[n_kept++] = gpx[g];
+        if (id < 255) ++id;
+      }
+    }
+    id_out[r] = gid[g];
+  }
+  return n_kept;
+}
+
+enum MdVerdict : uint32_t {
+  kMdFinal = 0,
+  kMdHostForced = 1,
+  kMdHostWalk = 2,
+  kMdHostManyComps = 3,
+  kMdHostMergeOff = 4,
+  kMdHostOverflow = 5,
+  kMdHostListCap = 6,
+  kMdHostPrePx = 7,
+  kMdHostTableFull = 8,
+  kMdHostLdsShort = 9,
+  kMdPending = 0xffffffffu,
+};
+struct MdFinish {
+  uint32_t verdict, n_kept, max_id, merged;
+  uint32_t kept_id[kNumberMax];
+  unsigned long long kept_px[kNumberMax];
+};
+struct NumberWork {
+  uint32_t order[kNumberMax], group[kNumberMax];
+  int32_t gid[kNumberMax];
+  unsigned long long gpx[kNumberMax];
+};
+
+inline std::vector<uint32_t> clusterOrder(const CompAcc* comp, uint32_t R) {
+  std::vector<uint32_t> order(R);
+  if (R <= kNumberMax) {
+    clusterOrderN(comp, R, order.data());
+    return order;
+  }
+  std::iota(order.begin(), order.end(), 0u);
+  std::sort(order.begin(), order.end(), [&](uint32_t a, uint32_t b) { return comp[a].min_key < comp[b].min_key; });
+  return order;
+}
+
+inline bool mayMerge(const CompAcc* comp, uint32_t R, float sep) { return mayMergeN(comp, R, sep); }
+
+struct Groups {
+  std::vector<uint32_t> rep;
+  explicit Groups(uint32_t n) : rep(n) { std::iota(rep.begin(), rep.end(), 0u); }
+  uint32_t find(uint32_t x) { return groupFind(rep.data(), x); }
+  void unite(uint32_t a, uint32_t b) { groupUnite(rep.data(), a, b); }
+  std::vector<uint32_t> labels() {
+    for (uint32_t i = 0; i < rep.size(); ++i) rep[i] = find(i);
+    return rep;
+  }
+};
+
+inline std::vector<uint32_t> groupsFromRows(const CompAcc* comp, uint32_t R) {
+  std::vector<uint32_t> group(R);
+  groupsFromRowsN(comp, R, group.data());
+  return group;
+}
+
+using Kept = std::vector<std::pair<int, uint64_t>>;
+template <class Px>
+inline Kept numberClusters(const uint32_t* order, const uint32_t* group, uint32_t R, Px px, int min_size, int max_size, std::vector<int32_t>* id_out) {
+  id_out->assign(R, 0);
+  std::vector<unsigned long long> gpx(R), kept_px(R);
+  std::vector<int32_t> gid(R);
+  std::vector<uint32_t> kept_id(R);
+  const uint32_t n = numberClustersN(order, group, R, px, min_size, max_size, gpx.data(), gid.data(), id_out->data(), kept_id.data(), kept_px.data());
+  Kept kept(n);
+  for (uint32_t i = 0; i < n; ++i) kept[i] = {static_cast<int>(kept_id[i]), static_cast<uint64_t>(kept_px[i])};
   return kept;
 }
 
diff --git a/khronos_amd/csrc/khronos_amd.hip b/khronos_amd/csrc/khronos_amd.hip
--- a/khronos_amd/csrc/khronos_amd.hip
+++ b/khronos_amd/csrc/khronos_amd.hip
@@ -276,6 +276,9 @@
   bool md_seed_run = false;
   uint32_t md_prev_seed_px = 0;
   uint64_t n_md_prelaunched = 0, n_md_prelaunch_repeats = 0;
+  uint64_t n_md_device_finishes = 0;
+  uint32_t* d_md_fin = nullptr;
+  PinnedBuf<uint32_t> h_md_fin;
   uint32_t md_last_seeds = 0;
   uint32_t* d_md_edges = nullptr;
   uint32_t* d_md_scratch4 = nullptr;
@@ -918,6 +921,8 @@
     KHR_CHAIN(devAlloc(c, &c->d_md_comp_acc, c->md_list_cap, false));
     KHR_CHAIN(devAlloc(c, &c->d_md_comp_final, kCompCap));
     KHR_CHAIN(c->h_md_head.alloc(16 + sizeof(CompAcc) * kCompCap));
+    KHR_CHAIN(devAlloc(c, &c->d_md_fin, sizeof(mdh::MdFinish) / 4 + 4));
+    KHR_CHAIN(c->h_md_fin.alloc(sizeof(mdh::MdFinish) / 4));
     KHR_CHAIN(devAlloc(c, &c->d_md_scratch4, 16));
     c->md_host_walk = std::getenv("KHR_MD_HOST_WALK") != nullptr;
     if (const char* e = std::getenv("KHR_MD_LDS_MAX")) c->md_lds_max = std::min<uint32_t>(kCompLds, static_cast<uint32_t>(std::atoi(e)));
@@ -2144,6 +2149,15 @@
   }
 }
 
+static int seedPublishNow(khr_ctx* c) {
+  if (c->seed_by_ticket && c->seed_publish_pending) {
+    hipLaunchKernelGGL(k_publish_seed, dim3(1), dim3(1), 0, c->stream, c->m, c->h_pinned.dev() + 2, c->seed_ticket);
+    HIP_TRY(hipGetLastError());
+    c->seed_publish_pending = false;
+  }
+  return KHR_OK;
+}
+
 static int waitSeedCount(khr_ctx* c) {
   const auto t_wait0 = std::chrono::steady_clock::now();
   if (!c->seed_by_ticket) {
@@ -2151,11 +2165,7 @@
     seedWaitDone(c, t_wait0, true);
     return KHR_OK;
   }
-  if (c->seed_publish_pending) {
-    hipLaunchKernelGGL(k_publish_seed, dim3(1), dim3(1), 0, c->stream, c->m, c->h_pinned.dev() + 2, c->seed_ticket);
-    HIP_TRY(hipGetLastError());
-    c->seed_publish_pending = false;
-  }
+  KHR_TRY(seedPublishNow(c));
   volatile uint32_t* hp = c->h_pinned;
   uint64_t spins = 0;
   while (hp[3] != c->seed_ticket) {
@@ -2199,7 +2209,7 @@
 }
 
 struct MdHooks {
-  bool no_device_merge, no_predict, no_prelaunch;
+  bool no_device_merge, no_predict, no_prelaunch, no_device_finish;
   uint32_t table_log2, prelaunch_px;
 };
 static MdHooks mdHooks() {
@@ -2208,6 +2218,7 @@
   h.no_device_merge = no_device_merge;
   h.no_predict = std::getenv("KHR_MD_NO_PREDICT") != nullptr;
   h.no_prelaunch = std::getenv("KHR_MD_NO_PRELAUNCH") != nullptr;
+  h.no_device_finish = std::getenv("KHR_MD_NO_DEVICE_FINISH") != nullptr;
   if (const char* e = std::getenv("KHR_MD_TABLE_LOG2")) h.table_log2 = static_cast<uint32_t>(std::min(30, std::max(4, std::atoi(e))));
   if (const char* e = std::getenv("KHR_MD_PRELAUNCH_PX")) h.prelaunch_px = static_cast<uint32_t>(std::max(1, std::atoi(e)));
   return h;
@@ -2224,7 +2235,13 @@
 
 struct MdTables { VoxTable seeds, bnd, near; };
 struct MdHead { uint32_t S, B, R, overflow; };
-static int mdLaunchChain(khr_ctx* c, int n, uint32_t seed_pixels, uint32_t mask, bool global_components, bool device_merge, MdTables* t) {
+struct MdTail {
+  std::function<int()> queue_behind;
+  bool queued = false;
+  bool device_finished = false;
+};
+static int mdLaunchChain(khr_ctx* c, int n, uint32_t seed_pixels, uint32_t mask, bool global_components, bool device_merge, MdTables* t,
+                         const MdHooks& hooks, FrameSlot* tail) {
   const uint32_t cap = c->md_list_cap;
   const int nn = c->cfg.md_neighbor_connectivity;
   CompAcc* d_comp_out = reinterpret_cast<CompAcc*>(reinterpret_cast<uint8_t*>(c->d_md_n) + 16);
@@ -2234,7 +2251,8 @@
   const VoxTable bnd = t->bnd = VoxTable{c->d_md_keys + tsize, c->d_md_counts + tsize, c->d_md_ids + tsize, mask};
   const VoxTable near = t->near = VoxTable{c->d_md_keys + 2 * tsize, c->d_md_counts + 2 * tsize, c->d_md_ids + 2 * tsize, mask};
   int32_t* const d_box = reinterpret_cast<int32_t*>(c->d_md_scratch4) + 8;
-  hipLaunchKernelGGL(k_md_clear, dim3(1024), dim3(256), 0, c->stream, c->d_md_keys, c->d_md_counts, static_cast<uint32_t>(tsize), c->d_md_n, d_box);
+  hipLaunchKernelGGL(k_md_clear, dim3(1024), dim3(256), 0, c->stream, c->d_md_keys, c->d_md_counts, static_cast<uint32_t>(tsize), c->d_md_n, d_box, c->d_md_fin,
+                     c->h_pinned.dev() + (c->seed_by_ticket ? 2 : 0));
   hipLaunchKernelGGL(k_md_seed_insert, dim3(gridFor(n)), dim3(256), 0, c->stream, c->d_keys, n, seeds, c->d_md_n + 3);
   hipLaunchKernelGGL(k_md_compact, dim3(gridFor(tsize)), dim3(256), 0, c->stream, seeds, c->d_md_seed_keys, c->d_md_seed_counts, c->d_md_n, cap, nullptr);
   hipLaunchKernelGGL(k_md_near_insert, dim3(256), dim3(256), 0, c->stream, c->d_md_seed_keys, c->d_md_n, cap, nn, near, c->d_md_n + 3, d_box);
@@ -2264,13 +2282,27 @@
   }
   HIP_TRY(hipGetLastError());
   if (++c->md_head_ticket == 0) ++c->md_head_ticket;
-  hipLaunchKernelGGL(k_publish, dim3(1), dim3(1024), 0, c->stream, c->d_md_n, reinterpret_cast<uint32_t*>(c->h_md_head.dev()),
-                     static_cast<uint32_t>(sizeof(CompAcc) / 4), kCompHead, c->h_pinned.dev() + 8, c->md_head_ticket, c->d_md_scratch4);
+  NumberArgs na{};
+  na.force = !tail || hooks.no_device_finish ? mdh::kMdHostForced : c->md_host_walk ? mdh::kMdHostWalk : mdh::kMdFinal;
+  na.device_merge = device_merge ? 1u : 0u;
+  na.global_components = global_components ? 1u : 0u;
+  na.pre_px = seed_pixels, na.mask = mask, na.full_mask = c->md_mask, na.list_cap = cap, na.lds_max = c->md_lds_max;
+  na.sep = c->cfg.md_min_separation_distance;
+  na.min_size = c->cfg.md_min_cluster_size, na.max_size = c->cfg.md_max_cluster_size;
+  static_assert(kCompHead == mdh::kNumberMax && kCompInline == static_cast<int>(mdh::kNumberMax), "the records that travel with the head are the ones the device numbers");
+  hipLaunchKernelGGL(k_md_number_publish, dim3(1), dim3(256), 0, c->stream, c->d_md_n, na, c->d_md_comp_final, c->d_md_fin,
+                     reinterpret_cast<uint32_t*>(c->h_md_head.dev()), c->h_md_fin.dev(), c->h_pinned.dev() + 8, c->md_head_ticket, c->d_md_scratch4);
+  if (tail) {
+    hipLaunchKernelGGL(k_md_comp_finals, dim3(1024), dim3(256), 0, c->stream, c->d_md_adj, c->d_md_n, cap, nn, c->d_md_parent, c->d_md_rootidx,
+                       c->d_md_comp_final, CompFinals{}, c->d_md_seed_final, c->d_md_bnd_final, c->d_md_bnd_deg, c->d_md_fin);
+    hipLaunchKernelGGL(k_md_paint, dim3(gridFor(n)), dim3(256), 0, c->stream, c->d_keys, n, seeds, bnd, c->d_md_seed_final, c->d_md_bnd_final,
+                       tail->dyn, c->d_md_bnd_deg, tail->dynw, c->d_md_fin);
+  }
   HIP_TRY(hipGetLastError());
   return KHR_OK;
 }
 
-static int mdRunChain(khr_ctx* c, FrameSlot& s, const MdHooks& hooks, bool device_merge, MdTables* t, MdHead* head) {
+static int mdRunChain(khr_ctx* c, FrameSlot& s, const MdHooks& hooks, bool device_merge, MdTables* t, MdHead* head, MdTail* tail) {
   const int n = s.sensor.width * s.sensor.height;
   bool with_global = c->md_host_walk || 2u * c->md_last_seeds > c->md_lds_max || c->md_lds_max < kCompLds;
   if (hooks.no_predict) with_global = false;
@@ -2278,13 +2310,20 @@
   if (mdQueuesAhead(c, hooks)) {
     pre_px = hooks.prelaunch_px ? hooks.prelaunch_px : std::min<uint32_t>(c->md_list_cap, std::max<uint32_t>(4096u, 2u * c->md_prev_seed_px));
     pre_mask = mdMaskFor(c, hooks, pre_px);
-    KHR_TRY(mdLaunchChain(c, n, pre_px, pre_mask, with_global, device_merge, t));
+    KHR_TRY(seedPublishNow(c));
+    KHR_TRY(mdLaunchChain(c, n, pre_px, pre_mask, with_global, device_merge, t, hooks, &s));
+    if (tail->queue_behind) KHR_TRY(tail->queue_behind());
+    tail->queued = true;
     ++c->n_md_prelaunched;
   }
+  const bool forced = hooks.no_device_finish || c->md_host_walk;
   KHR_TRY(waitSeedCount(c));
   s.clusters.clear();
   c->md_seed_run = c->h_pinned[0] != 0;
-  if (c->h_pinned[0] == 0) return 0;
+  if (c->h_pinned[0] == 0) {
+    tail->device_finished = tail->queued && !forced;
+    return 0;
+  }
   c->md_prev_seed_px = c->h_pinned[0];
   s.dyn_clean = false;
   bool chain_queued = pre_px != 0 && c->h_pinned[0] <= pre_px;
@@ -2292,9 +2331,21 @@
   uint32_t mask = chain_queued ? pre_mask : mdMaskFor(c, hooks, c->h_pinned[0]);
   const uint32_t* cnt = reinterpret_cast<const uint32_t*>(c->h_md_head.get());
   for (int attempt = 0;; ++attempt) {
-    if (!chain_queued) KHR_TRY(mdLaunchChain(c, n, c->h_pinned[0], mask, with_global, device_merge, t));
+    const bool first_chain = !chain_queued && !tail->queued;
+    if (!chain_queued) KHR_TRY(mdLaunchChain(c, n, c->h_pinned[0], mask, with_global, device_merge, t, hooks, first_chain ? &s : nullptr));
+    if (first_chain) {
+      if (tail->queue_behind) KHR_TRY(tail->queue_behind());
+      tail->queued = true;
+    }
+    const bool has_tail = chain_queued || first_chain;
     chain_queued = false;
     KHR_TRY(waitTicket(c, 8, c->md_head_ticket, "the motion detector's component records"));
+    if (has_tail && static_cast<volatile const uint32_t*>(c->h_md_fin.get())[0] == mdh::kMdFinal) {
+      *head = MdHead{cnt[0], cnt[1], cnt[2], cnt[3]};
+      c->md_last_seeds = head->S;
+      tail->device_finished = true;
+      return 2;
+    }
     const bool table_full = cnt[3] && mask < c->md_mask;
     const bool lds_short = !table_full && cnt[0] > c->md_lds_max && !with_global;
     if (attempt == 2 || !(table_full || lds_short)) break;
@@ -2312,7 +2363,7 @@
 static int mdPaintAndList(khr_ctx* c, FrameSlot& s, const MdTables& t, const mdh::Kept& kept, int* deferred_summary) {
   const int n = s.sensor.width * s.sensor.height;
   hipLaunchKernelGGL(k_md_paint, dim3(gridFor(n)), dim3(256), 0, c->stream, c->d_keys, n, t.seeds, t.bnd, c->d_md_seed_final,
-                     c->d_md_bnd_final, s.dyn, c->d_md_bnd_deg, s.dynw);
+                     c->d_md_bnd_final, s.dyn, c->d_md_bnd_deg, s.dynw, static_cast<const uint32_t*>(nullptr));
   s.dyn_clean = false, s.dynw_valid = true;
   HIP_TRY(hipGetLastError());
   if (deferred_summary) *deferred_summary = kept.back().first;
@@ -2344,7 +2395,8 @@
     fin_dev = c->d_md_comp_final;
   }
   hipLaunchKernelGGL(k_md_comp_finals, dim3(1024), dim3(256), 0, c->stream, c->d_md_adj, c->d_md_n, c->md_list_cap, c->cfg.md_neighbor_connectivity,
-                     c->d_md_parent, c->d_md_rootidx, fin_dev, inl, c->d_md_seed_final, c->d_md_bnd_final, c->d_md_bnd_deg);
+                     c->d_md_parent, c->d_md_rootidx, fin_dev, inl, c->d_md_seed_final, c->d_md_bnd_final, c->d_md_bnd_deg,
+                     static_cast<const uint32_t*>(nullptr));
   return mdPaintAndList(c, s, t, kept, deferred_summary);
 }
 
@@ -2383,7 +2435,7 @@
   return mdPaintAndList(c, s, t, kept, deferred_summary);
 }
 
-static int motionFinish(khr_ctx* c, FrameSlot& s, int* deferred_summary = nullptr) {
+static int motionFinish(khr_ctx* c, FrameSlot& s, int* deferred_summary = nullptr, MdTail* tail = nullptr) {
   if (deferred_summary) *deferred_summary = -1;
   if (!c->cfg.with_tracking) return 0;
   const MdHooks hooks = mdHooks();
@@ -2391,9 +2443,28 @@
   const bool device_merge = !hooks.no_device_merge && !c->md_host_walk && sep > 0.f && sep <= 2.f;
   MdTables t{};
   MdHead head{};
-  const int rc = mdRunChain(c, s, hooks, device_merge, &t, &head);
+  MdTail own_tail;
+  if (!tail) tail = &own_tail;
+  const int rc = mdRunChain(c, s, hooks, device_merge, &t, &head, tail);
   if (rc <= 0) return rc;
   c->stats.n_seeds = head.S;
+  if (rc == 2) {
+    const mdh::MdFinish* fin = reinterpret_cast<const mdh::MdFinish*>(c->h_md_fin.get());
+    ++c->n_md_device_finishes;
+    if (fin->merged) ++c->n_md_device_merges;
+    const uint32_t n_kept = std::min<uint32_t>(fin->n_kept, mdh::kNumberMax);
+    if (n_kept == 0) return 0;
+    s.dyn_clean = false, s.dynw_valid = true;
+    if (deferred_summary) *deferred_summary = static_cast<int>(fin->max_id);
+    else KHR_TRY(clusterSummaryLaunch(c, s, static_cast<int>(fin->max_id)));
+    s.clusters.assign(n_kept, khr_cluster{});
+    for (uint32_t i = 0; i < n_kept; ++i) {
+      s.clusters[i].id = static_cast<int32_t>(fin->kept_id[i]);
+      s.clusters[i].num_pixels_listed = fin->kept_px[i];
+      s.clusters[i].semantic_id = -1;
+    }
+    return static_cast<int>(n_kept);
+  }
   if (head.R <= kCompCap && !c->md_host_walk) {
     if (head.R > kCompHead) {
       HIP_TRY(hipMemcpyAsync(c->h_md_head, c->d_md_n, 16 + sizeof(CompAcc) * head.R, hipMemcpyDeviceToHost, c->stream));
@@ -3618,8 +3689,20 @@
   }
   bool have_seeds = false;
   int summary_pending = -1;
+  MdTail tail;
+  size_t tail_timer = static_cast<size_t>(-1), tail_end = 0;
   if (motion) {
-    const int nc = motionFinish(c, s, &summary_pending);
+    tail.queue_behind = [&]() {
+      const size_t n_pending = c->pending.size();
+      const bool clean = s.dyn_clean;
+      s.dyn_clean = false;
+      const int rcu = integrateUpdate(c, s, f, 1, 1, -1, defer_fold, nullptr, c->d_md_fin);
+      s.dyn_clean = clean;
+      if (c->pending.size() > n_pending) tail_timer = n_pending;
+      tail_end = c->pending.size();
+      return rcu;
+    };
+    const int nc = motionFinish(c, s, &summary_pending, &tail);
     if (nc < 0) return nc;
     if (n_clusters) *n_clusters = nc;
     have_seeds = c->cfg.with_tracking && c->h_pinned[0] != 0;
@@ -3627,7 +3710,9 @@
   HT("pf_motion_done");
   if (speculated && have_seeds && spec_timer != static_cast<size_t>(-1))
     for (size_t i = spec_timer; i < spec_end && i < c->pending.size(); ++i) c->pending[i].which = -1;
-  if (!speculated || have_seeds) {
+  if (tail.queued && !tail.device_finished && tail_timer != static_cast<size_t>(-1))
+    for (size_t i = tail_timer; i < tail_end && i < c->pending.size(); ++i) c->pending[i].which = -1;
+  if (!((speculated && !have_seeds) || tail.device_finished)) {
     rc = integrateUpdate(c, s, f, 1, motion ? 1 : 0, -1, defer_fold);
     if (rc) return rc;
   }
@@ -3798,6 +3883,7 @@
   s.n_md_host_walks = c->n_md_host_walks;
   s.n_md_prelaunched = c->n_md_prelaunched;
   s.n_md_prelaunch_repeats = c->n_md_prelaunch_repeats;
+  s.n_md_device_finishes = c->n_md_device_finishes;
   s.band_overflow = 0;
   s.n_tracking_processed_blocks = c->h_counters[c->ef_cur ? C_N_PROC2 : C_N_PROC];
   s.cum_updated_voxels = st[S_CUM_UPD] + cur_upd;
```
